# chairclr/PathTracing

Measured on AMD Instinct MI355X. Metric: Mrays/s, higher is better.
Workload: dtype f32

## Files before the change

include/ptrt.h:

```cpp
#ifndef PTRT_H
#define PTRT_H
#include <stddef.h>
#include <stdint.h>
#ifdef __cplusplus
extern "C" {
#endif

#define PTRT_ABI_VERSION 2

typedef int32_t pt_status;
enum {
    PT_OK = 0,
    PT_ERR_INVALID_ARGUMENT = 1,
    PT_ERR_NO_DEVICE = 2,
    PT_ERR_HIP = 3,
    PT_ERR_OUT_OF_MEMORY = 4,
    PT_ERR_NOT_COMMITTED = 5,
    PT_ERR_UNSUPPORTED = 6,
    PT_ERR_INTERNAL = 7
};

typedef struct pt_context pt_context;
typedef struct pt_scene pt_scene;

// ... 9 lines not shown
    PT_FLAG_EXTEND_SIMPLE = 8u,
    PT_FLAG_BUCKET_SPECULAR = 32u,
    PT_FLAG_SPLIT_KERNELS = 64u,
    PT_FLAG_EXTEND_POOL = 128u,
    PT_FLAG_ACCUMULATE = 16u,
    PT_FLAG_NEXT_EVENT = 256u,
    PT_FLAG_NEXT_EVENT_SPHERES = 512u
};
enum {
    PT_BVH_WIDTH_DEFAULT = 0,
    PT_BVH_WIDTH_2 = 2,
    PT_BVH_WIDTH_4 = 4,
    PT_BVH_WIDTH_4Q = 68,
    PT_BVH_WIDTH_8Q = 72,
    PT_BVH_WIDTH_8O = 73,
    PT_BVH_BUILD_LBVH = 0x100
};

typedef struct {
    int32_t device_ordinal;
    void *stream;
    uint32_t flags;
    uint32_t reserved;
} pt_device_desc;

typedef struct { uint32_t kind; float albedo[3]; float emission[3]; float roughness; float ior; uint32_t pad[3]; } pt_material;
#define PT_IOR_MIN 9.5367431640625e-07f
#define PT_IOR_MAX 1048576.0f

typedef struct { float origin[3], forward[3], right[3], up[3]; float scale, cx, cy; uint32_t jitter; } pt_camera;

typedef struct {
    uint32_t width, height;
    uint32_t spp;
    uint32_t max_depth;
    uint32_t rr_start;
    uint32_t seed;
    uint32_t sample_offset;
    uint32_t mode;
    float ray_eps;
    uint32_t rank, nranks;
    uint32_t tile_size;
    uint32_t flags;
    uint32_t streams;
    uint32_t pad[2];
} pt_render_params;

typedef struct {
    uint64_t rays;
    uint64_t paths;
    uint64_t node_visits, tri_tests, sphere_tests;
    uint32_t iterations;
    uint32_t extend_launches;
    double gpu_ms;
    double extend_ms;
    double shade_ms;
    double other_ms;
    uint64_t reserved[4];
} pt_stats;

typedef struct {
    uint32_t width;
    uint32_t n_nodes;
    uint32_t n_tris;
    uint32_t max_depth;
    uint64_t node_bytes;
    uint64_t tri_bytes;
    double build_ms;
    float sah_cost;
    uint32_t stack_need;
} pt_bvh_info;

typedef struct {
    uint32_t bounces;
    uint32_t loops;
    uint32_t finish_below;
    uint32_t packed_chunk;
    float compact_below;
    float sparse_below;
    uint32_t sticky_samples;
    uint32_t lag;
    uint32_t extend_kernel;
    uint32_t readback;
} pt_tuning;

pt_status pt_context_create(const pt_device_desc *desc, pt_context **out);
void pt_context_destroy(pt_context *ctx);
const char *pt_last_error(const pt_context *ctx);
pt_status pt_context_get_tuning(const pt_context *ctx, pt_tuning *out);
pt_status pt_context_set_tuning(pt_context *ctx, const pt_tuning *tuning);
uint32_t pt_abi_version(void);

pt_status pt_scene_create(pt_context *ctx, pt_scene **out);
void pt_scene_destroy(pt_scene *scene);
pt_status pt_scene_set_triangles(pt_scene *s, const float *verts9, const uint32_t *material_ids, uint64_t count);
pt_status pt_scene_set_spheres(pt_scene *s, const float *cxyzr, const uint32_t *material_ids, uint64_t count);
pt_status pt_scene_set_materials(pt_scene *s, const pt_material *mats, uint64_t count);
pt_status pt_scene_set_camera(pt_scene *s, const pt_camera *cam);
pt_status pt_scene_set_sky(pt_scene *s, const float rgb[3]);
pt_status pt_scene_set_environment(pt_scene *s, const float *rgb, uint32_t n);
typedef struct pt_environment_info { uint32_t n, lit; uint64_t device_bytes; double total; } pt_environment_info;
pt_status pt_scene_environment_info(const pt_scene *s, pt_environment_info *out);
pt_status pt_scene_environment_read(const pt_scene *s, float *texels4, float *mcdf, float *ccdf, uint64_t n_texels);
typedef struct pt_lens {
    float radius;
    float focus_distance;
    uint32_t flags;
    uint32_t pad[5];
} pt_lens;
pt_status pt_scene_set_lens(pt_scene *s, const pt_lens *lens);
pt_status pt_scene_get_lens(const pt_scene *s, pt_lens *out);
#define PT_MAX_TEXTURES 64u
#define PT_NO_TEXTURE 0xFFFFFFFFu
enum { PT_TEXTURE_NEAREST = 1u };
pt_status pt_scene_set_triangle_uvs(pt_scene *s, const float *uv6, uint64_t count);
pt_status pt_scene_set_texture(pt_scene *s, uint32_t index, const float *rgb, uint32_t width, uint32_t height, uint32_t flags);
pt_status pt_scene_set_material_textures(pt_scene *s, const uint32_t *texture_of_material, uint64_t count);
typedef struct pt_texture_info { uint32_t width, height, flags, materials; uint64_t device_bytes; } pt_texture_info;
pt_status pt_scene_texture_info(const pt_scene *s, uint32_t index, pt_texture_info *out);
pt_status pt_scene_commit(pt_scene *s, uint32_t bvh_width);
pt_status pt_scene_bvh_info(const pt_scene *s, pt_bvh_info *out);
pt_status pt_scene_bvh_read(const pt_scene *s, void *nodes, uint64_t node_bytes, void *tris48, uint64_t tri_bytes);

pt_status pt_render(pt_context *ctx, const pt_scene *scene, const pt_render_params *params, pt_stats *stats);

enum {
    PT_TRACE_OCCLUSION = 1u,
    PT_TRACE_COUNT_VISITS = 2u,
    PT_TRACE_HOST_MEMORY = 4u
};
pt_status pt_trace_rays(pt_context *ctx, const pt_scene *scene, const void *rays, void *hits, uint64_t n_rays,
                        uint32_t flags, pt_stats *stats);

enum { PT_GATHER_HOST_MEMORY = 1u };
typedef struct pt_gather_params {
    uint32_t samples;
    uint32_t seed;
    uint32_t sample_offset;
    uint32_t point_offset;
    float max_distance;
    float ray_eps;
    uint32_t flags;
    uint32_t pad;
} pt_gather_params;
pt_status pt_gather(pt_context *ctx, const pt_scene *scene, const void *points, void *out, uint64_t n_points,
                    const pt_gather_params *gp, pt_stats *stats);

enum {
    PT_GATHER_PATHS_NEXT_EVENT = 4u,
    PT_GATHER_PATHS_SPHERE_LIGHTS = 16u
};
typedef struct pt_gather_path_params {
    uint32_t max_depth;
    uint32_t rr_start;
    uint32_t flags;
    uint32_t pad[5];
} pt_gather_path_params;
pt_status pt_gather_paths(pt_context *ctx, const pt_scene *scene, const void *points, void *out, uint64_t n_points,
                          const pt_gather_params *gp, const pt_gather_path_params *pp, pt_stats *stats);

enum {
    PT_UPDATE_HOST_MEMORY = 1u
};
pt_status pt_scene_update_triangles(pt_scene *s, const void *verts9, uint64_t count, uint32_t flags, pt_stats *stats);
pt_status pt_scene_update_spheres(pt_scene *s, const float *cxyzr, uint64_t count);

// ... 99 lines not shown
```

pathtracing_amd/_native.py:

```python
import ctypes as C
import os

_HERE = os.path.dirname(os.path.abspath(__file__))
LIB_PATH = os.environ.get("PTRT_LIB") or os.path.join(_HERE, "libptrt.so")

if not os.path.exists(LIB_PATH):
    raise ImportError(
        f"{LIB_PATH} not found: build it with `make -C pathtracing_amd/csrc` (hipcc --offload-arch=gfx950) "
        "or `python -c 'import __graft_entry__ as g; g.build()'`. libptrt has no CPU fallback."
    )

try:
    import torch
except ImportError:
    torch = None

lib = C.CDLL(LIB_PATH)

PT_OK, PT_ERR_INVALID_ARGUMENT, PT_ERR_NO_DEVICE, PT_ERR_HIP, PT_ERR_OUT_OF_MEMORY, PT_ERR_NOT_COMMITTED, \
    PT_ERR_UNSUPPORTED, PT_ERR_INTERNAL = range(8)
PT_REFERENCE_SPHERE, PT_PATH_TRACE = 0, 1
PT_LAMBERT, PT_METAL, PT_DIELECTRIC = 0, 1, 2
PT_IOR_MIN, PT_IOR_MAX = 2.0 ** -20, 2.0 ** 20
PT_FLAG_PROFILE_KERNELS, PT_FLAG_COUNT_VISITS, PT_FLAG_EXTEND_PACKED, PT_FLAG_EXTEND_SIMPLE, PT_FLAG_ACCUMULATE, PT_FLAG_BUCKET_SPECULAR = 1, 2, 4, 8, 16, 32
PT_FLAG_SPLIT_KERNELS = 64
PT_FLAG_EXTEND_POOL = 128
PT_FLAG_NEXT_EVENT = 256
PT_FLAG_NEXT_EVENT_SPHERES = 512
PT_SCENE_CORNELL, PT_SCENE_CORNELL_GLASS, PT_SCENE_TRIANGLE_SOUP, PT_SCENE_CORNELL_TESS = 0, 1, 2, 3
PT_BVH_WIDTH_2, PT_BVH_WIDTH_4, PT_BVH_WIDTH_4Q, PT_BVH_WIDTH_8Q, PT_BVH_WIDTH_8O, PT_BVH_BUILD_LBVH = 2, 4, 68, 72, 73, 0x100
PT_COMM_FORCE_RCCL, PT_COMM_COPY_EXCHANGE = 1, 2
PT_TRACE_OCCLUSION, PT_TRACE_COUNT_VISITS, PT_TRACE_HOST_MEMORY = 1, 2, 4
PT_UPDATE_HOST_MEMORY = 1
PT_GATHER_HOST_MEMORY = 1
PT_MAX_TEXTURES, PT_NO_TEXTURE, PT_TEXTURE_NEAREST = 64, 0xFFFFFFFF, 1
PT_GATHER_PATHS_NEXT_EVENT = 4
PT_GATHER_PATHS_SPHERE_LIGHTS = 16
PT_DENOISE_GUIDES_ONLY, PT_DENOISE_NO_EDGE_STOPS = 1, 2
PT_TEMPORAL_RESET, PT_TEMPORAL_MATCH_IDS = 1, 2
PT_TEMPORAL_MOTION = 8
PT_DISPLAY_FRAME, PT_DISPLAY_DENOISED, PT_DISPLAY_TEMPORAL = 0, 1, 2
PT_TONE_CLAMP, PT_TONE_REINHARD, PT_TONE_ACES = 0, 1, 2
PT_DISPLAY_AUTO_EXPOSURE, PT_DISPLAY_LINEAR, PT_DISPLAY_RESET_ADAPTATION = 1, 2, 4


class pt_device_desc(C.Structure):
    _fields_ = [("device_ordinal", C.c_int32), ("stream", C.c_void_p), ("flags", C.c_uint32), ("reserved", C.c_uint32)]


class pt_material(C.Structure):
    _fields_ = [("kind", C.c_uint32), ("albedo", C.c_float * 3), ("emission", C.c_float * 3),
                ("roughness", C.c_float), ("ior", C.c_float), ("pad", C.c_uint32 * 3)]


class pt_camera(C.Structure):
    _fields_ = [("origin", C.c_float * 3), ("forward", C.c_float * 3), ("right", C.c_float * 3), ("up", C.c_float * 3),
                ("scale", C.c_float), ("cx", C.c_float), ("cy", C.c_float), ("jitter", C.c_uint32)]


class pt_render_params(C.Structure):
    _fields_ = [("width", C.c_uint32), ("height", C.c_uint32), ("spp", C.c_uint32), ("max_depth", C.c_uint32),
                ("rr_start", C.c_uint32), ("seed", C.c_uint32), ("sample_offset", C.c_uint32), ("mode", C.c_uint32),
                ("ray_eps", C.c_float), ("rank", C.c_uint32), ("nranks", C.c_uint32), ("tile_size", C.c_uint32),
                ("flags", C.c_uint32), ("streams", C.c_uint32), ("pad", C.c_uint32 * 2)]


class pt_stats(C.Structure):
    _fields_ = [("rays", C.c_uint64), ("paths", C.c_uint64), ("node_visits", C.c_uint64), ("tri_tests", C.c_uint64),
                ("sphere_tests", C.c_uint64), ("iterations", C.c_uint32), ("extend_launches", C.c_uint32),
                ("gpu_ms", C.c_double), ("extend_ms", C.c_double), ("shade_ms", C.c_double), ("other_ms", C.c_double),
                ("reserved", C.c_uint64 * 4)]


class pt_bvh_info(C.Structure):
    _fields_ = [("width", C.c_uint32), ("n_nodes", C.c_uint32), ("n_tris", C.c_uint32), ("max_depth", C.c_uint32),
                ("node_bytes", C.c_uint64), ("tri_bytes", C.c_uint64), ("build_ms", C.c_double),
                ("sah_cost", C.c_float), ("stack_need", C.c_uint32)]


class pt_tuning(C.Structure):
    _fields_ = [("bounces", C.c_uint32), ("loops", C.c_uint32), ("finish_below", C.c_uint32), ("packed_chunk", C.c_uint32),
                ("compact_below", C.c_float), ("sparse_below", C.c_float), ("sticky_samples", C.c_uint32), ("lag", C.c_uint32),
                ("extend_kernel", C.c_uint32), ("readback", C.c_uint32)]


class pt_tile_layout(C.Structure):
    _fields_ = [("tile_size", C.c_uint32), ("tiles_x", C.c_uint32), ("tiles_y", C.c_uint32), ("n_tiles", C.c_uint32),
                ("tiles_mine", C.c_uint32), ("tiles_per_rank", C.c_uint32), ("floats_per_tile", C.c_uint64)]


class pt_denoise_params(C.Structure):
    _fields_ = [("iterations", C.c_uint32), ("sigma_color", C.c_float), ("sigma_normal", C.c_float), ("sigma_depth", C.c_float),
                ("sigma_albedo", C.c_float), ("flags", C.c_uint32), ("pad", C.c_uint32 * 2)]


class pt_temporal_params(C.Structure):
    _fields_ = [("max_history", C.c_uint32), ("plane_tolerance", C.c_float), ("normal_min", C.c_float), ("flags", C.c_uint32),
                ("pad", C.c_uint32 * 4)]


class pt_display_params(C.Structure):
    _fields_ = [("source", C.c_uint32), ("curve", C.c_uint32), ("exposure", C.c_float), ("white", C.c_float), ("key", C.c_float),
                ("adapt", C.c_float), ("trim_low", C.c_uint32), ("trim_high", C.c_uint32), ("flags", C.c_uint32), ("pad", C.c_uint32)]


class pt_display_info(C.Structure):
    _fields_ = [("exposure", C.c_float), ("metered", C.c_float), ("log_average", C.c_float), ("adapted", C.c_uint32),
                ("counted", C.c_uint64), ("used", C.c_uint64)]


class pt_environment_info(C.Structure):
    _fields_ = [("n", C.c_uint32), ("lit", C.c_uint32), ("device_bytes", C.c_uint64), ("total", C.c_double)]


class pt_gather_params(C.Structure):
    _fields_ = [("samples", C.c_uint32), ("seed", C.c_uint32), ("sample_offset", C.c_uint32), ("point_offset", C.c_uint32),
                ("max_distance", C.c_float), ("ray_eps", C.c_float), ("flags", C.c_uint32), ("pad", C.c_uint32)]


class pt_gather_path_params(C.Structure):
    _fields_ = [("max_depth", C.c_uint32), ("rr_start", C.c_uint32), ("flags", C.c_uint32), ("pad", C.c_uint32 * 5)]


class pt_lens(C.Structure):
    _fields_ = [("radius", C.c_float), ("focus_distance", C.c_float), ("flags", C.c_uint32), ("pad", C.c_uint32 * 5)]


class pt_texture_info(C.Structure):
    _fields_ = [("width", C.c_uint32), ("height", C.c_uint32), ("flags", C.c_uint32), ("materials", C.c_uint32), ("device_bytes", C.c_uint64)]


class pt_scene_counts(C.Structure):
    _fields_ = [("n_tris", C.c_uint64), ("n_spheres", C.c_uint64), ("n_mats", C.c_uint64)]


assert C.sizeof(pt_material) == 48 and C.sizeof(pt_camera) == 64 and C.sizeof(pt_render_params) == 64 and C.sizeof(pt_tuning) == 40
assert C.sizeof(pt_denoise_params) == 32 and C.sizeof(pt_temporal_params) == 32
assert C.sizeof(pt_display_params) == 40 and C.sizeof(pt_display_info) == 32 and C.sizeof(pt_environment_info) == 24
assert C.sizeof(pt_gather_params) == 32 and C.sizeof(pt_lens) == 32 and C.sizeof(pt_texture_info) == 24

_vp, _u32, _u64, _st = C.c_void_p, C.c_uint32, C.c_uint64, C.c_int32
_P = C.POINTER

SYMBOLS = {
    "pt_abi_version": (_u32, []),
    "pt_context_create": (_st, [_P(pt_device_desc), _P(_vp)]),
    "pt_context_destroy": (None, [_vp]),
    "pt_last_error": (C.c_char_p, [_vp]),
    "pt_context_get_tuning": (_st, [_vp, _P(pt_tuning)]),
    "pt_context_set_tuning": (_st, [_vp, _P(pt_tuning)]),
    "pt_scene_create": (_st, [_vp, _P(_vp)]),
    "pt_scene_destroy": (None, [_vp]),
    "pt_scene_set_triangles": (_st, [_vp, _vp, _vp, _u64]),
    "pt_scene_set_spheres": (_st, [_vp, _vp, _vp, _u64]),
    "pt_scene_set_materials": (_st, [_vp, _vp, _u64]),
    "pt_scene_set_camera": (_st, [_vp, _P(pt_camera)]),
    "pt_scene_set_sky": (_st, [_vp, _P(C.c_float * 3)]),
    "pt_scene_set_environment": (_st, [_vp, _vp, _u32]),
    "pt_scene_environment_info": (_st, [_vp, _P(pt_environment_info)]),
    "pt_scene_environment_read": (_st, [_vp, _vp, _vp, _vp, _u64]),
    "pt_scene_set_lens": (_st, [_vp, _P(pt_lens)]),
    "pt_scene_get_lens": (_st, [_vp, _P(pt_lens)]),
    "pt_scene_set_triangle_uvs": (_st, [_vp, _vp, _u64]),
    "pt_scene_set_texture": (_st, [_vp, _u32, _vp, _u32, _u32, _u32]),
    "pt_scene_set_material_textures": (_st, [_vp, _vp, _u64]),
    "pt_scene_texture_info": (_st, [_vp, _u32, _P(pt_texture_info)]),
    "pt_scene_commit": (_st, [_vp, _u32]),
    "pt_scene_bvh_info": (_st, [_vp, _P(pt_bvh_info)]),
    "pt_scene_bvh_read": (_st, [_vp, _vp, _u64, _vp, _u64]),
    "pt_render": (_st, [_vp, _vp, _P(pt_render_params), _P(pt_stats)]),
    "pt_trace_rays": (_st, [_vp, _vp, _vp, _vp, _u64, _u32, _P(pt_stats)]),
    "pt_gather": (_st, [_vp, _vp, _vp, _vp, _u64, _P(pt_gather_params), _P(pt_stats)]),
    "pt_gather_paths": (_st, [_vp, _vp, _vp, _vp, _u64, _P(pt_gather_params), _P(pt_gather_path_params), _P(pt_stats)]),
    "pt_scene_update_triangles": (_st, [_vp, _vp, _u64, _u32, _P(pt_stats)]),
    "pt_scene_update_spheres": (_st, [_vp, _vp, _u64]),
    "pt_denoise": (_st, [_vp, _vp, _P(pt_denoise_params), _P(pt_stats)]),
    "pt_denoised_read": (_st, [_vp, _vp, _u64]),
    "pt_denoised_device_ptr": (_st, [_vp, _P(_vp), _P(_u64)]),
    "pt_guides_read": (_st, [_vp, _vp, _u64]),
    "pt_denoise_temporal": (_st, [_vp, _vp, _P(pt_temporal_params), _P(pt_denoise_params), _P(pt_stats)]),
    "pt_temporal_read": (_st, [_vp, _vp, _u64]),
    "pt_temporal_device_ptr": (_st, [_vp, _P(_vp), _P(_u64)]),
    "pt_temporal_history_read": (_st, [_vp, _vp, _u64]),
    "pt_display": (_st, [_vp, _P(pt_display_params), _P(pt_stats)]),
    "pt_display_read": (_st, [_vp, _vp, _u64]),
    "pt_display_device_ptr": (_st, [_vp, _P(_vp), _P(_u64)]),
    "pt_display_info_read": (_st, [_vp, _P(pt_display_info)]),
    "pt_display_histogram_read": (_st, [_vp, _vp, _u64]),
    "pt_framebuffer_read": (_st, [_vp, _vp, _u64]),
    "pt_framebuffer_read_rgba8": (_st, [_vp, _vp, _u64]),
    "pt_framebuffer_read_srgb8": (_st, [_vp, _vp, _u64]),
    "pt_framebuffer_device_ptr": (_st, [_vp, _P(_vp), _P(_u64)]),
    "pt_tile_layout_query": (_st, [_P(pt_render_params), _P(pt_tile_layout)]),
    "pt_tiles_device_ptr": (_st, [_vp, _P(_vp), _P(_u64)]),
    "pt_assemble_tiles": (_st, [_vp, _P(pt_render_params), _vp, _u64]),
    "pt_comm_create": (_st, [_P(_vp), _u32, _u32, _u32, _P(_vp)]),
    "pt_comm_destroy": (None, [_vp]),
    "pt_comm_render": (_st, [_vp, _P(_vp), _P(pt_render_params), _P(pt_stats)]),
    "pt_comm_stage_tiles": (_st, [_vp, _u32]),
    "pt_comm_assemble": (_st, [_vp, _P(pt_render_params)]),
    "pt_scenegen": (_st, [_u32, _u32, _u32, _u32, _u32, _P(pt_scene_counts), _vp, _vp, _vp, _vp, _vp, _P(pt_camera), _vp]),
}

for _name, (_res, _args) in SYMBOLS.items():
    _f = getattr(lib, _name)
    _f.restype = _res
    _f.argtypes = _args

INTERNAL_SYMBOLS = {
    "pt_internal_lbvh_binary": (_st, [_vp, _vp, _u64, _vp, _vp, _vp, _vp, _vp, _vp]),
}
for _name, (_res, _args) in INTERNAL_SYMBOLS.items():
    _f = getattr(lib, _name)
    _f.restype = _res
    _f.argtypes = _args

PTRT_ABI_VERSION = 2
if lib.pt_abi_version() != PTRT_ABI_VERSION:
    raise ImportError(f"{LIB_PATH} has ABI version {lib.pt_abi_version()}, this binding expects {PTRT_ABI_VERSION}: rebuild libptrt.so")
# ... 1 lines not shown
```

pathtracing_amd/csrc/api.cpp:

```cpp
#include "context.h"
#include <hip/hip_runtime.h>
#include <cmath>
#include <cstdarg>
#include <cstdio>
#include <cstring>
#include <new>
#include <string>

using namespace ptrt;

namespace {
thread_local std::string g_err;
}

namespace ptrt {
pt_status layout_of(const pt_render_params *p, pt_tile_layout *o)
{
    if (!p || !o) return PT_ERR_INVALID_ARGUMENT;
    if (p->width == 0 || p->height == 0 || p->width > 32768 || p->height > 32768) return PT_ERR_INVALID_ARGUMENT;
    if (p->tile_size != 0 && p->tile_size != kTile) return PT_ERR_UNSUPPORTED;
    const uint32_t nr = p->nranks ? p->nranks : 1u;
    if (p->rank >= nr) return PT_ERR_INVALID_ARGUMENT;
    o->tile_size = kTile;
    o->tiles_x = (p->width + kTile - 1) / kTile;
// ... 22 lines not shown
pt_status check_device_array(pt_context *c, const void *p, uint64_t bytes, const char *what, const char *who, const char *host_flag)
{
    hipPointerAttribute_t at;
    if (hipPointerGetAttributes(&at, p) != hipSuccess || (at.type != hipMemoryTypeDevice && !at.isManaged) || at.device != c->device) {
        (void)hipGetLastError();
        return fail(c, PT_ERR_INVALID_ARGUMENT, "%s: %s is not device memory of the context's device %d (host arrays: %s)", who, what, c->device, host_flag);
    }
    hipDeviceptr_t base = nullptr; size_t size = 0;
    if (hipMemGetAddressRange(&base, &size, (hipDeviceptr_t)p) != hipSuccess) { (void)hipGetLastError(); return PT_OK; }
    if ((const char *)p + bytes > (const char *)base + size)
        return fail(c, PT_ERR_INVALID_ARGUMENT, "%s: %s holds %llu bytes from the pointer on, the call needs %llu", who, what,
                    (unsigned long long)((const char *)base + size - (const char *)p), (unsigned long long)bytes);
    return PT_OK;
}
pt_status copy_out(pt_context *c, void *dst, const void *src, uint64_t need, size_t elem, uint64_t have, const char *unit)
{
    if (have < need) return fail(c, PT_ERR_INVALID_ARGUMENT, "buffer too small: need %llu %s", (unsigned long long)need, unit);
    HIP_TRY(c, hipSetDevice(c->device));
    HIP_TRY(c, hipMemcpyAsync(dst, src, need * elem, hipMemcpyDeviceToHost, c->stream));
    HIP_TRY(c, hipStreamSynchronize(c->stream));
    return PT_OK;
}
}

extern "C" {

uint32_t pt_abi_version(void) { return PTRT_ABI_VERSION; }

const char *pt_last_error(const pt_context *ctx) { return ctx ? ctx->err.c_str() : g_err.c_str(); }

pt_status pt_context_create(const pt_device_desc *desc, pt_context **out)
{
    if (!out) return fail(nullptr, PT_ERR_INVALID_ARGUMENT, "pt_context_create: out is NULL");
    *out = nullptr;
    const int dev = desc ? desc->device_ordinal : 0;
    int ndev = 0;
    hipError_t e = hipGetDeviceCount(&ndev);
    if (e != hipSuccess || ndev <= 0)
        return fail(nullptr, PT_ERR_NO_DEVICE, "no HIP device visible (%s); libptrt has no CPU backend",
                    e == hipSuccess ? "device count 0" : hipGetErrorString(e));
    if (dev < 0 || dev >= ndev) return fail(nullptr, PT_ERR_INVALID_ARGUMENT, "device ordinal %d out of range [0,%d)", dev, ndev);
    hipDeviceProp_t prop;
    HIP_TRY(nullptr, hipGetDeviceProperties(&prop, dev));
    if (std::strncmp(prop.gcnArchName, "gfx950", 6) != 0)
        return fail(nullptr, PT_ERR_NO_DEVICE, "device %d is %s; libptrt ships gfx950 (MI355X) code objects only", dev, prop.gcnArchName);
    HIP_TRY(nullptr, hipSetDevice(dev));
    pt_context *c = new (std::nothrow) pt_context();
    if (!c) return fail(nullptr, PT_ERR_OUT_OF_MEMORY, "host allocation failed");
    c->device = dev;
    if (desc && desc->stream) c->stream.borrow((hipStream_t)desc->stream);
    else if ((e = c->stream.create()) != hipSuccess) { delete c; return fail(nullptr, PT_ERR_HIP, "hipStreamCreate: %s", hipGetErrorString(e)); }
    bool ok = c->sizes.alloc() == hipSuccess;
    if (ok && !c->sizes.can_map()) c->tuning.readback = 1u;
    for (uint32_t g = 0; ok && g < kMaxGroups; ++g) ok = c->group_stream[g].create() == hipSuccess && c->ev_join[g].create(false) == hipSuccess;
    ok = ok && c->ev_fork.create(false) == hipSuccess && c->ev_start.create() == hipSuccess && c->ev_stop.create() == hipSuccess;
    ok = ok && c->sizes.create_events() == hipSuccess;
    for (auto &ev : c->ev_probe) ok = ok && ev.create() == hipSuccess;
    for (auto &ev : c->query.ev) ok = ok && ev.create() == hipSuccess;
    ok = ok && c->counters.ensure(kCntTotalWords) == hipSuccess;
    if (!ok) { delete c; return fail(nullptr, PT_ERR_HIP, "context resource creation failed"); }
    *out = c;
    return PT_OK;
}

pt_status pt_context_get_tuning(const pt_context *c, pt_tuning *o)
{
    if (!c || !o) return fail(nullptr, PT_ERR_INVALID_ARGUMENT, "pt_context_get_tuning: NULL argument");
    *o = c->tuning;
    return PT_OK;
}

pt_status pt_context_set_tuning(pt_context *c, const pt_tuning *t)
{
    if (!c || !t) return fail(c, PT_ERR_INVALID_ARGUMENT, "pt_context_set_tuning: NULL argument");
    if (t->bounces > 64) return fail(c, PT_ERR_INVALID_ARGUMENT, "tuning: bounces must be 0 (default) or 1..64");
    if (t->loops != 0 && t->loops != 1 && t->loops != 2 && t->loops != 4) return fail(c, PT_ERR_INVALID_ARGUMENT, "tuning: loops must be 0 (default), 1, 2 or 4");
    if (t->packed_chunk != 0 && (t->packed_chunk < 64 || t->packed_chunk > (1u << 20))) return fail(c, PT_ERR_INVALID_ARGUMENT, "tuning: packed_chunk must be 0 (default) or 64..2^20");
    if (t->lag != 0 && (t->lag < 2 || t->lag > kLag)) return fail(c, PT_ERR_INVALID_ARGUMENT, "tuning: lag must be 0 (default) or 2..%u", kLag);
    if (!(t->compact_below >= 0.f && t->compact_below <= 2.f) || !(t->sparse_below >= 0.f && t->sparse_below <= 1.f))
        return fail(c, PT_ERR_INVALID_ARGUMENT, "tuning: compact_below must be in [0,2], sparse_below in [0,1]");
    if (t->extend_kernel > kExtendKernelLast) return fail(c, PT_ERR_INVALID_ARGUMENT, "tuning: extend_kernel must be 0 (probed), 1 (one ray per lane), 2 (lane-packing) or 3 (pooled)");
    if (t->readback > 1) return fail(c, PT_ERR_INVALID_ARGUMENT, "tuning: readback must be 0 (mapped store) or 1 (copy per launch)");
    if (t->readback == 0 && !c->sizes.can_map()) return fail(c, PT_ERR_UNSUPPORTED, "tuning: readback 0 needs host-mapped pinned memory, which this platform did not provide");
    c->tuning = *t;
    return PT_OK;
}

void pt_context_destroy(pt_context *c)
{
    if (!c) return;
    (void)hipSetDevice(c->device);
    context_drain(c);
    delete c;
}

pt_status pt_tile_layout_query(const pt_render_params *p, pt_tile_layout *o)
{
    pt_status st = layout_of(p, o);
    if (st != PT_OK) return fail(nullptr, st, "invalid render params for tile layout");
    return PT_OK;
}

pt_status pt_framebuffer_read(pt_context *c, float *rgba, uint64_t n_floats)
{
    if (!c || !rgba) return fail(c, PT_ERR_INVALID_ARGUMENT, "NULL argument");
    if (!c->out.readable()) return fail(c, PT_ERR_NOT_COMMITTED, "no assembled frame (render with nranks == 1 or call pt_assemble_tiles)");
    return copy_out(c, rgba, c->out.fb.p, c->out.pixels() * 4, sizeof(float), n_floats, "floats");
}

pt_status pt_framebuffer_read_rgba8(pt_context *c, uint8_t *rgba8, uint64_t n_bytes)
{
    if (!c || !rgba8) return fail(c, PT_ERR_INVALID_ARGUMENT, "NULL argument");
    if (!c->out.readable()) return fail(c, PT_ERR_NOT_COMMITTED, "no assembled frame");
    return copy_out(c, rgba8, c->out.fb8.p, c->out.pixels() * 4, 1, n_bytes, "bytes");
}

pt_status pt_framebuffer_read_srgb8(pt_context *c, uint8_t *rgba8, uint64_t n_bytes)
{
    pt_status st = pt_framebuffer_read_rgba8(c, rgba8, n_bytes);
    if (st != PT_OK) return st;
    uint8_t lut[256];
    for (int q = 0; q < 256; ++q) {
        const double l = q / 255.0, e = l <= 0.0031308 ? 12.92 * l : 1.055 * std::pow(l, 1.0 / 2.4) - 0.055;
        lut[q] = (uint8_t)std::floor(255.0 * e + 0.5);
    }
    const uint64_t n = c->out.pixels() * 4;
    for (uint64_t i = 0; i < n; ++i) if ((i & 3u) != 3u) rgba8[i] = lut[rgba8[i]];
    return PT_OK;
}

pt_status pt_framebuffer_device_ptr(pt_context *c, void **dptr, uint64_t *n_floats)
{
    if (!c || !dptr) return fail(c, PT_ERR_INVALID_ARGUMENT, "NULL argument");
    if (!c->out.readable()) return fail(c, PT_ERR_NOT_COMMITTED, "no assembled frame");
    *dptr = c->out.fb.p;
    if (n_floats) *n_floats = c->out.pixels() * 4;
    return PT_OK;
}

pt_status pt_tiles_device_ptr(pt_context *c, void **dptr, uint64_t *n_floats)
{
    if (!c || !dptr) return fail(c, PT_ERR_INVALID_ARGUMENT, "NULL argument");
    if (!c->out.tile_slots()) return fail(c, PT_ERR_NOT_COMMITTED, "no path-traced frame yet");
    *dptr = c->out.tiles.p;
    if (n_floats) *n_floats = (uint64_t)c->out.tile_slots() * 4;
    return PT_OK;
}

pt_status pt_assemble_tiles(pt_context *c, const pt_render_params *p, const void *gathered, uint64_t n_floats)
{
    if (!c || !p || !gathered) return fail(c, PT_ERR_INVALID_ARGUMENT, "NULL argument");
    pt_tile_layout lay;
    pt_status st = layout_of(p, &lay);
    if (st != PT_OK) return fail(c, st, "pt_assemble_tiles: bad params");
    if (p->spp == 0) return fail(c, PT_ERR_INVALID_ARGUMENT, "spp == 0");
    const uint32_t nranks = p->nranks ? p->nranks : 1u;
    const uint64_t per_rank = (uint64_t)lay.tiles_per_rank * kTilePixels;
    if (n_floats < per_rank * nranks * 4) return fail(c, PT_ERR_INVALID_ARGUMENT, "gathered buffer too small: need %llu floats", (unsigned long long)(per_rank * nranks * 4));
    HIP_TRY(c, hipSetDevice(c->device));
    c->out.replace();
    HIP_TRY(c, c->out.resize(p->width, p->height));
    HIP_TRY(c, launch_assemble(c->stream, (const float4 *)gathered, nranks, (uint32_t)per_rank, p->width, p->height, lay.tiles_x, lay.n_tiles,
                               1.0f / (float)(((p->flags & PT_FLAG_ACCUMULATE) ? (uint64_t)p->sample_offset : 0u) + p->spp), c->out.fb.p, c->out.fb8.p));
    HIP_TRY(c, hipStreamSynchronize(c->stream));
    c->out.complete(FrameOutputs::Holds::path_traced);
    return PT_OK;
// ... 4 lines not shown
```

pathtracing_amd/csrc/context.h:

```cpp
#pragma once
#include "ptrt_internal.h"
#include "device_owner.h"
#include <algorithm>
#include <cstring>
#include <string>
#include <vector>

namespace ptrt {

pt_status fail(pt_context *ctx, pt_status code, const char *fmt, ...);
#define HIP_TRY(ctx, expr)                                                                          \
    do { hipError_t _e = (expr);                                                                    \
         if (_e != hipSuccess)                                                                      \
             return fail(ctx, _e == hipErrorOutOfMemory ? PT_ERR_OUT_OF_MEMORY : PT_ERR_HIP,        \
                         "%s failed: %s (%s:%d)", #expr, hipGetErrorString(_e), __FILE__, __LINE__); \
    } while (0)

void context_drain(pt_context *c);

template <typename Call> pt_status drained_on_failure(pt_context *c, Call call)
{
    const pt_status st = call();
    if (st != PT_OK && c) { (void)hipSetDevice(context_device(c)); context_drain(c); }
    return st;
// ... 141 lines not shown
    bool valid_ = false;
};

class Accumulation {
public:
    struct Key { uint32_t w, h, rank, nranks, streams, seed; bool nee; bool spheres = false; };
    enum class Refusal { none, other_frame, other_estimator, other_light_set, wrong_offset };
    Refusal continues(const Key &k, uint32_t sample_offset) const
    {
        if (spp == 0 || key.w != k.w || key.h != k.h || key.rank != k.rank || key.nranks != k.nranks || key.streams != k.streams || key.seed != k.seed)
            return Refusal::other_frame;
        if (key.nee != k.nee) return Refusal::other_estimator;
        if (key.spheres != k.spheres) return Refusal::other_light_set;
        return sample_offset != spp ? Refusal::wrong_offset : Refusal::none;
    }
    uint64_t samples() const { return spp; }
    bool next_event() const { return key.nee; }
    bool sphere_lights() const { return key.spheres; }
    void begin() { spp = 0; }
    void complete(const Key &k, uint64_t total_spp) { key = k; spp = total_spp; }

private:
    Key key{};
    uint64_t spp = 0;
};

class QueueSizes {
public:
    struct Sizes { uint32_t longest; uint64_t alive, traced; };
    hipError_t alloc()
    {
        const hipError_t e = h_counts.alloc(kTemplateOffset + kRingWords);
        if (e == hipSuccess && h_ring.alloc(kLag * kShards, true) == hipSuccess) std::memset(h_ring.p, 0, sizeof(uint4) * kLag * kShards);
        else if (e == hipSuccess) (void)hipGetLastError();
        return e;
    }
    hipError_t create_events()
    {
        for (auto &row : ev_lag) for (auto &ev : row) if (const hipError_t e = ev.create(false)) return e;
        return hipSuccess;
    }
    bool can_map() const { return h_ring.d != nullptr; }
    uint4 *begin(bool mapped) { mapped_ = mapped; return mapped ? h_ring.d : nullptr; }
    uint32_t *frame_end() const { return h_counts.p + kFinalOffset; }
    uint32_t *template_sizes() const { return h_counts.p + kTemplateOffset; }

    hipError_t post(hipStream_t stream, uint32_t g, uint32_t it, const uint32_t *lines, uint32_t n_shards)
    {
        const uint32_t ring = it % kLag;
        if (!mapped_) {
            const hipError_t e = hipMemcpyAsync(copied(g, ring), lines, sizeof(uint32_t) * n_shards * kCounterStride, hipMemcpyDeviceToHost, stream);
            if (e != hipSuccess) return e;
        }
        return hipEventRecord(ev_lag[g][ring], stream);
    }
    hipError_t wait(uint32_t g, uint32_t old_it, uint32_t first_shard, uint32_t n_shards, Sizes &out)
    {
        const hipError_t e = hipEventSynchronize(ev_lag[g][(mapped_ ? old_it + 1u : old_it) % kLag]);
        if (e != hipSuccess) return e;
        const volatile uint32_t *h_old = mapped_ ? (const volatile uint32_t *)(h_ring.p + (size_t)(old_it % kLag) * kShards + first_shard)
                                                 : copied(g, old_it % kLag);
        const uint32_t line = mapped_ ? 4u : kCounterStride;
        out = Sizes{ 0u, 0u, 0u };
        for (uint32_t sh = 0; sh < n_shards; ++sh) {
            out.longest = std::max(out.longest, (uint32_t)h_old[sh * line]);
            out.alive += h_old[sh * line + 1];
            out.traced += (uint64_t)h_old[sh * line + 2] | ((uint64_t)h_old[sh * line + 3] << 32);
        }
        return hipSuccess;
    }

private:
    static constexpr size_t kFinalOffset = (size_t)kMaxGroups * kLag * kRingWords;
    static constexpr size_t kTemplateOffset = kFinalOffset + kCntTotalWords;
    uint32_t *copied(uint32_t g, uint32_t ring) const { return h_counts.p + ((size_t)g * kLag + ring) * kRingWords; }
    Pinned<uint32_t> h_counts;
    Pinned<uint4> h_ring;
    Event ev_lag[kMaxGroups][kLag];
    bool mapped_ = false;
};

class FrameTemplate {
public:
    struct Key { uint32_t w, h, rank, nranks, streams, first_spp, offset, n_slots, shard_cap, pad; const void *q, *acc;
                 bool operator==(const Key &o) const { return std::memcmp(this, &o, sizeof *this) == 0; } };
    hipError_t reserve(size_t q_entries)
    {
        const hipError_t e = q_init.ensure(q_entries);
        return e != hipSuccess ? e : cnt_init.ensure(kCntTotalWords);
    }
    pt_status build_if_differs(pt_context *c, hipStream_t q, Key key, const Pipeline &pipe, const DeviceScene &ds, const PathState &ps,
                               const FrameParams &fp, const QueueSizes &sizes);
    void frame_ran(bool accumulate_or_full_state) { if (accumulate_or_full_state && key_.first_spp < key_.streams) valid = false; }
    const uint32_t *counters() const { return cnt_init.p; }
    uint32_t *first_queue() const { return q_init.p; }
    uint32_t first_bound() const { return bound; }

private:
    DevBuf<uint32_t> q_init, cnt_init;
    Key key_{};
    bool valid = false;
    uint32_t bound = 0;
};

class Queries {
public:
    DevBuf<float4> rays, hits;
    Event ev[2];
    struct Counts { uint32_t error; uint64_t node_visits, tri_tests, sphere_tests; };
    pt_status setup(pt_context *c, uint32_t overflow, uint64_t n_rays, PathState &ps);
    pt_status launch(pt_context *c, const DeviceScene &ds, const PathState &ps, const float4 *rays, float4 *hits, uint64_t n_rays, bool occlusion, bool count);
    pt_status finish(pt_context *c, Counts &out);

private:
    DevBuf<uint32_t> cnt;
    DevBuf<int32_t> ovf;
};

}

struct pt_context {
    int device = 0;
    ptrt::Stream stream;
    std::string err;
    ptrt::DevBuf<float4> ray_o, ray_d, thr, acc;
    ptrt::DevBuf<float4> nee_ext, nee_rad;
    ptrt::DevBuf<float2> hit;
    ptrt::DevBuf<uint32_t> sd, q_ext0, q_ext1, q_metal, q_dielectric, counters;
    ptrt::DevBuf<int32_t> stack_ovf;
    ptrt::Accumulation sums;
    ptrt::FrameTemplate start;
    ptrt::QueueSizes sizes;
    ptrt::Stream group_stream[ptrt::kMaxGroups];
    ptrt::Event ev_fork, ev_join[ptrt::kMaxGroups];
    pt_tuning tuning = {
        0,
        0,
        4096,
        0,
        0.9f,
        0.f,
        32,
        0,
        0,
        0,
    };
    ptrt::Event ev_start, ev_stop;
    ptrt::Event ev_probe[4];
    std::vector<ptrt::Event> ev_pool;
    ptrt::FrameOutputs out;
    ptrt::TemporalHistory history;
    ptrt::DisplayAdaptation adaptation;
    ptrt::Queries query;
};
```

pathtracing_amd/csrc/frame.cpp:

```cpp
#include "scene.h"
#include <hip/hip_runtime.h>
#include <algorithm>
#include <cmath>
#include <cstdio>
#include <cstdlib>
#include <cstring>
#include <vector>

using namespace ptrt;

namespace {

uint32_t host_pcg(uint32_t x)
{
    uint32_t s = x * 747796405u + 2891336453u;
    uint32_t w = ((s >> ((s >> 28) + 4u)) ^ s) * 277803737u;
    return (w >> 22) ^ w;
}

uint32_t faster(double rate_simple, double rate_packed) { return rate_packed > 1.10 * rate_simple ? EXT_PACKED : EXT_SIMPLE; }
struct ExtendFrame {
    ExtendChoice &mem;
    bool undecided;
    uint32_t frame_kernel, kernel;
    bool mixed = false;
    uint64_t probe_n[2] = { 0, 0 };
    ExtendFrame(ExtendChoice &m, const Pipeline &p) : mem(m),
        undecided(p.forced == 0u && m.kernel == 0u && !p.instrumented()),
        frame_kernel((undecided && m.rate_simple > 0.0 && m.rate_packed == 0.0) ? EXT_PACKED : EXT_SIMPLE),
        kernel(p.forced ? p.forced : m.kernel ? m.kernel : (undecided && frame_kernel == EXT_SIMPLE) ? 0u : frame_kernel) {}
    bool probing(uint32_t g, uint32_t it) const { return g == 0u && kernel == 0u && (it == 2u || it == 3u); }
    uint32_t bounces(uint32_t g, uint32_t it, int k, uint32_t simple) const { return k != EXT_PACKED ? simple : probing(g, it) ? 8u : 64u; }
    hipError_t observe(uint32_t g, uint32_t it, uint64_t traced, uint32_t loop_slots, const Event *ev)
    {
        if (!probing(g, it)) return hipSuccess;
        probe_n[it - 2u] = traced;
        if (it == 2u) return hipSuccess;
        float ms_simple = 0.f, ms_packed = 0.f; hipError_t e = hipEventElapsedTime(&ms_simple, ev[0], ev[1]);
        if (e != hipSuccess || (e = hipEventElapsedTime(&ms_packed, ev[2], ev[3])) != hipSuccess) return e;
        const uint64_t enough = (uint64_t)loop_slots / 8u;
        if (probe_n[0] < enough || probe_n[1] < enough) {
            kernel = EXT_SIMPLE; mixed = probe_n[1] >= enough / 8u;
        } else kernel = mem.kernel = faster(probe_n[0] / std::max((double)ms_simple, 1e-6), probe_n[1] / std::max((double)ms_packed, 1e-6));
        return hipSuccess;
    }
    void frame_done(uint64_t rays, double gpu_ms, bool cold)
    {
        if (!undecided || mem.kernel != 0u || cold) return;
        if (mixed || rays < (1u << 20) || !(gpu_ms > 0.0)) { if (++mem.misses >= 3u) mem.kernel = EXT_SIMPLE; return; }
        (frame_kernel == EXT_PACKED ? mem.rate_packed : mem.rate_simple) = (double)rays / gpu_ms;
        if (mem.rate_simple > 0.0 && mem.rate_packed > 0.0) mem.kernel = faster(mem.rate_simple, mem.rate_packed);
    }
};

hipEvent_t pool_event(pt_context *c, size_t i)
{
    while (c->ev_pool.size() <= i) {
        Event e;
        if (e.create() != hipSuccess) return nullptr;
        c->ev_pool.push_back(std::move(e));
    }
    return c->ev_pool[i];
}

bool scene_pixels(const pt_scene *s, const pt_camera &cam, uint32_t W, uint32_t H, FrameParams &fp)
{
    fp.scene_x0 = fp.scene_y0 = 0u; fp.scene_x1 = fp.scene_y1 = ~0u;
    Box tb;
    if (!s->tree.root_bound(tb)) return false;
    double lo[3], hi[3], o[3], big = 0.0;
    for (int k = 0; k < 3; ++k) { lo[k] = tb.lo[k]; hi[k] = tb.hi[k]; o[k] = cam.origin[k]; big = std::max(big, std::fabs(o[k])); }
    for (size_t i = 0; i < s->sph_mat.size(); ++i) {
        const float *sp = &s->spheres[i * 4];
        const double r = sp[3], dx = sp[0] - o[0], dy = sp[1] - o[1], dz = sp[2] - o[2], reach = std::sqrt(dx * dx + dy * dy + dz * dz) + r;
        const double rr = std::sqrt(r * r + std::ldexp(reach * reach, -16));
        for (int k = 0; k < 3; ++k) { lo[k] = std::min(lo[k], sp[k] - rr); hi[k] = std::max(hi[k], sp[k] + rr); }
    }
    if (!(lo[0] <= hi[0])) { fp.scene_x0 = fp.scene_x1 = fp.scene_y0 = fp.scene_y1 = ~0u; return true; }
    for (int k = 0; k < 3; ++k) big = std::max(big, std::max(std::fabs(lo[k]), std::fabs(hi[k])));
    if (!(big < 1e15)) return false;
    for (int k = 0; k < 3; ++k) { lo[k] -= 1e-4 * big; hi[k] += 1e-4 * big; }
    const double R[3] = { cam.right[0], cam.right[1], cam.right[2] }, U[3] = { cam.up[0], cam.up[1], cam.up[2] }, F[3] = { cam.forward[0], cam.forward[1], cam.forward[2] };
    auto cross = [](const double *a, const double *b, double *c) { c[0] = a[1] * b[2] - a[2] * b[1]; c[1] = a[2] * b[0] - a[0] * b[2]; c[2] = a[0] * b[1] - a[1] * b[0]; };
    auto dot = [](const double *a, const double *b) { return a[0] * b[0] + a[1] * b[1] + a[2] * b[2]; };
    double UF[3], FR[3], RU[3];
    cross(U, F, UF); cross(F, R, FR); cross(R, U, RU);
    const double det = dot(R, UF), scale = cam.scale;
    if (!(std::fabs(det) > 1e-6 * std::sqrt(dot(R, R) * dot(U, U) * dot(F, F))) || !(scale > 0.0) || !std::isfinite(scale)) return false;
    double x0 = INFINITY, x1 = -INFINITY, y0 = INFINITY, y1 = -INFINITY;
    for (int i = 0; i < 8; ++i) {
        const double v[3] = { ((i & 1) ? hi[0] : lo[0]) - o[0], ((i & 2) ? hi[1] : lo[1]) - o[1], ((i & 4) ? hi[2] : lo[2]) - o[2] };
        const double a = dot(v, UF) / det, b = dot(v, FR) / det, c = dot(v, RU) / det;
        if (!(c > 1e-4 * (std::fabs(a) + std::fabs(b) + std::fabs(c)))) return false;
        const double px = (a / c + cam.cx) / scale, py = (b / c + cam.cy) / scale;
        x0 = std::min(x0, px); x1 = std::max(x1, px); y0 = std::min(y0, py); y1 = std::max(y1, py);
    }
    const double mx = 1.0 + 1e-4 * ((double)W + std::fabs(cam.cx / scale)), my = 1.0 + 1e-4 * ((double)H + std::fabs(cam.cy / scale));
    x0 -= mx; x1 += mx; y0 -= my; y1 += my;
    if (!std::isfinite(x0) || !std::isfinite(x1) || !std::isfinite(y0) || !std::isfinite(y1)) return false;
    auto px_of = [](double v, uint32_t n) { return (uint32_t)std::min(std::max(v, 0.0), (double)n); };
    fp.scene_x0 = px_of(std::floor(x0), W); fp.scene_x1 = px_of(std::ceil(x1), W);
    fp.scene_y0 = px_of(std::floor(y0), H); fp.scene_y1 = px_of(std::ceil(y1), H);
    if (fp.scene_x0 == 0u && fp.scene_x1 >= W && fp.scene_y0 == 0u && fp.scene_y1 >= H) { fp.scene_x1 = fp.scene_y1 = ~0u; return false; }
    return true;
}

uint64_t scene_pixels_code(const FrameParams &fp)
{
    if (fp.scene_x0 >= fp.scene_x1 || fp.scene_y0 >= fp.scene_y1) return ~0ull;
    if (fp.width > 0xFFFFu || fp.height > 0xFFFFu) return 0ull;
    return (uint64_t)fp.scene_x0 | (uint64_t)fp.scene_x1 << 16 | (uint64_t)fp.scene_y0 << 32 | (uint64_t)fp.scene_y1 << 48;
}

bool lens_basis(const pt_camera &cam, const pt_lens &lens, LensArgs &out)
{
    auto dot = [](const float *a) { return std::fma(a[2], a[2], std::fma(a[1], a[1], a[0] * a[0])); };
    const float dr = dot(cam.right), du = dot(cam.up);
    if (dr == 0.0f || du == 0.0f) return false;
    const float ru = lens.radius * (1.0f / std::sqrt(dr)), rv = lens.radius * (1.0f / std::sqrt(du));
    for (int k = 0; k < 3; ++k) {
        out.u[k] = cam.right[k] * ru; out.v[k] = cam.up[k] * rv;
        if (!std::isfinite(out.u[k]) || !std::isfinite(out.v[k])) return false;
    }
    out.focus = lens.focus_distance; out.pad = 0u;
    return true;
}

bool lens_in_domain(const pt_camera &cam, const pt_lens &lens, uint32_t W, uint32_t H)
{
    const double r[3] = { cam.right[0], cam.right[1], cam.right[2] }, u[3] = { cam.up[0], cam.up[1], cam.up[2] }, f[3] = { cam.forward[0], cam.forward[1], cam.forward[2] };
    auto dot = [](const double *a, const double *b) { return a[0] * b[0] + a[1] * b[1] + a[2] * b[2]; };
    const double n[3] = { r[1] * u[2] - r[2] * u[1], r[2] * u[0] - r[0] * u[2], r[0] * u[1] - r[1] * u[0] };
    const double nn = std::sqrt(dot(n, n)), lr = std::sqrt(dot(r, r)), lu = std::sqrt(dot(u, u)), F = lens.focus_distance, R = lens.radius;
    if (!(nn > 0x1p-6 * lr * lu)) return false;
    const double scale = cam.scale, cx = cam.cx, cy = cam.cy, tw = (double)W * std::fabs(scale) + std::fabs(cx), th = (double)H * std::fabs(scale) + std::fabs(cy);
    const double ax = -cx, bx = (double)W * scale - cx, ay = -cy, by = (double)H * scale - cy;
    const double sxs[2] = { std::min(ax, bx) - std::ldexp(tw, -22), std::max(ax, bx) + std::ldexp(tw, -22) };
    const double sys[2] = { std::min(ay, by) - std::ldexp(th, -22), std::max(ay, by) + std::ldexp(th, -22) };
    double vmax = 0.0;
    for (int i = 0; i < 4; ++i) {
        const double sx = sxs[i & 1], sy = sys[i >> 1];
        const double v[3] = { f[0] + sx * r[0] + sy * u[0], f[1] + sx * r[1] + sy * u[1], f[2] + sx * r[2] + sy * u[2] };
        const double len = std::sqrt(dot(v, v));
        if (!std::isfinite(len)) return false;
        vmax = std::max(vmax, len);
    }
    const double hi = F * vmax + R * std::sqrt(1.0 + std::fabs(dot(r, u)) / (lr * lu));
    const double S = std::sqrt(dot(f, f)) + (std::max(std::fabs(ax), std::fabs(bx)) + tw) * lr + (std::max(std::fabs(ay), std::fabs(by)) + th) * lu;
    const double lo = F * (std::fabs(dot(f, n)) / nn - std::ldexp(S, -11));
    return lo >= 0x1p-60 && hi * hi <= 0x1p127;
}

struct Frame {
    uint32_t nranks, streams, pixel_slots, n_slots, shard_cap, samples_per_stream, lag, n_loops, packed_chunk, default_bounces;
    Pipeline pipe;
    bool accumulate, mapped, compact;
    NeeArgs nee_args; EnvArgs env_args; LensArgs lens_args;
    SphArgs sph_args;
    TexArgs tex_args;
    bool sky;
    Accumulation::Key sums_key;
    size_t q_entries; uint64_t total_spp, allocs_before;
    PathState ps; FrameParams fp;
    uint32_t iters; uint64_t slot_launches; size_t n_events;
    std::vector<uint64_t> trace_alive, trace_rays;
};

}

pt_status FrameTemplate::build_if_differs(pt_context *c, hipStream_t q, Key key, const Pipeline &pipe, const DeviceScene &ds, const PathState &ps,
                                          const FrameParams &fp, const QueueSizes &sizes)
{
    key.q = q_init.p;
    if (valid && key == key_) return PT_OK;
    valid = false; HIP_TRY(c, hipMemsetAsync(cnt_init.p, 0, sizeof(uint32_t) * kCntTotalWords, q));
    PathState pt = ps; pt.counters = cnt_init.p; pt.q_ext[0] = q_init.p;
    const bool dense = key.first_spp < key.streams;
    HIP_TRY(c, launch_generate(q, ds, pt, fp, pipe.generate_mode(dense)));
    bound = key.shard_cap;
    if (dense) {
        uint32_t *h = sizes.template_sizes();
        HIP_TRY(c, hipMemcpyAsync(h, cnt_init.p, sizeof(uint32_t) * kShards * kCounterStride, hipMemcpyDeviceToHost, q));
        HIP_TRY(c, hipStreamSynchronize(q));
        bound = 0;
        for (uint32_t sh = 0; sh < kShards; ++sh) bound = std::max(bound, h[cnt_ext_index(0, sh)]);
    }
    key_ = key; valid = true;
    return PT_OK;
}

static PipelineDecode decode_frame(const pt_context *c, const pt_scene *s, const pt_render_params *p)
{
    return decode_pipeline(p->flags, c->tuning.extend_kernel, s->env.present(), s->has_specular, s->lens.radius > 0.f, s->n_sph_lights != 0u, s->textures.textured());
}
static Accumulation::Key sums_key_of(const pt_render_params *p)
{
    return Accumulation::Key{ p->width, p->height, p->rank, p->nranks ? p->nranks : 1u, p->streams ? p->streams : 1u, p->seed,
                              (p->flags & PT_FLAG_NEXT_EVENT) != 0, (p->flags & PT_FLAG_NEXT_EVENT_SPHERES) != 0 };
}
static pt_status other_light_set(pt_context *c)
{
    return fail(c, PT_ERR_INVALID_ARGUMENT, "PT_FLAG_ACCUMULATE: the sums so far were made %s PT_FLAG_NEXT_EVENT_SPHERES", c->sums.sphere_lights() ? "with" : "without");
}

static pt_status plan_frame(pt_context *c, const pt_scene *s, const pt_render_params *p, const pt_tile_layout &lay, Frame &f)
{
    if (!s) return fail(c, PT_ERR_INVALID_ARGUMENT, "pt_render: scene is NULL");
    if (s->ctx != c) return fail(c, PT_ERR_INVALID_ARGUMENT, "scene belongs to another context");
    if (!s->committed) return fail(c, PT_ERR_NOT_COMMITTED, "scene not committed");
    if (p->spp == 0 || p->spp >= (1u << 24)) return fail(c, PT_ERR_INVALID_ARGUMENT, "spp must be in [1, 2^24)");
    if (p->max_depth == 0 || p->max_depth > 255) return fail(c, PT_ERR_INVALID_ARGUMENT, "max_depth must be in [1,255]");
    if (!std::isfinite(p->ray_eps) || p->ray_eps < 0.f) return fail(c, PT_ERR_INVALID_ARGUMENT, "ray_eps must be finite and >= 0");
    if (p->streams > 64) return fail(c, PT_ERR_INVALID_ARGUMENT, "streams must be in [0,64]");
    const pt_tuning &t = c->tuning;
    f.nranks = p->nranks ? p->nranks : 1u; f.streams = p->streams ? p->streams : 1u;
    f.pixel_slots = lay.tiles_per_rank * kTilePixels;
    const uint64_t slots64 = (uint64_t)f.pixel_slots * f.streams;
    if (slots64 >= (1ull << 28)) return fail(c, PT_ERR_UNSUPPORTED, "frame too large: %llu slots (pixels of this rank x streams), limit 2^28", (unsigned long long)slots64);
    f.n_slots = (uint32_t)slots64;
    const uint32_t groups = (f.n_slots + (1u << kShardGroupShift) - 1u) >> kShardGroupShift, shard_cap = ((groups + kShards - 1) / kShards) << kShardGroupShift;
    f.shard_cap = shard_cap; f.q_entries = (size_t)kShards * shard_cap;
    f.samples_per_stream = (p->spp + f.streams - 1u) / f.streams;
    const PipelineDecode d = decode_frame(c, s, p);
    if (d.status != PT_OK) return fail(c, d.status, "%s", d.message);
    const Pipeline &pipe = f.pipe = d.pipeline;
    if (pipe.lens && !lens_basis(s->ds.cam, s->lens, f.lens_args))
        return fail(c, PT_ERR_INVALID_ARGUMENT, "pt_render through a lens: the camera's right or up has length 0, or the aperture's axes are not finite");
    f.mapped = t.readback == 0u;
    f.packed_chunk = t.packed_chunk >= 64u ? t.packed_chunk : (f.streams >= 4u ? 256u : 128u);
    const uint32_t v34 = p->max_depth * 3u / 4u; f.default_bounces = std::min(12u, std::max(4u, v34 > 2u ? v34 - 2u : 0u));
    if (pipe.nee) f.default_bounces *= 2u;
    f.lag = t.lag ? t.lag : (f.samples_per_stream <= 2u ? 2u : 3u) + (f.mapped ? 1u : 0u);
    f.accumulate = (p->flags & PT_FLAG_ACCUMULATE) != 0;
    f.sums_key = sums_key_of(p);
    if (f.accumulate)
        switch (c->sums.continues(f.sums_key, p->sample_offset)) {
        case Accumulation::Refusal::other_frame:
            return fail(c, PT_ERR_INVALID_ARGUMENT, "PT_FLAG_ACCUMULATE needs a previous frame with the same size, rank, nranks, streams and seed");
        case Accumulation::Refusal::other_estimator:
            return fail(c, PT_ERR_INVALID_ARGUMENT, "PT_FLAG_ACCUMULATE: the sums so far were made %s PT_FLAG_NEXT_EVENT", c->sums.next_event() ? "with" : "without");
        case Accumulation::Refusal::other_light_set: return other_light_set(c);
        case Accumulation::Refusal::wrong_offset:
            return fail(c, PT_ERR_INVALID_ARGUMENT, "PT_FLAG_ACCUMULATE: sample_offset must be %llu (samples so far)", (unsigned long long)c->sums.samples());
        case Accumulation::Refusal::none: break;
        }
    f.total_spp = (f.accumulate ? c->sums.samples() : 0u) + p->spp; c->sums.begin();
    f.allocs_before = g_device_allocs;
    HIP_TRY(c, c->ray_o.ensure(f.n_slots)); HIP_TRY(c, c->ray_d.ensure(f.n_slots)); HIP_TRY(c, c->thr.ensure(f.n_slots));
    HIP_TRY(c, c->acc.ensure(f.n_slots)); HIP_TRY(c, c->out.tiles.ensure(f.pixel_slots)); HIP_TRY(c, c->sd.ensure(f.n_slots));
    HIP_TRY(c, c->q_ext0.ensure(f.q_entries)); HIP_TRY(c, c->q_ext1.ensure(f.q_entries));
    if (pipe.split) { HIP_TRY(c, c->hit.ensure(f.n_slots)); HIP_TRY(c, c->q_metal.ensure(f.q_entries)); HIP_TRY(c, c->q_dielectric.ensure(f.q_entries)); }
    if (!pipe.full_state()) HIP_TRY(c, c->start.reserve(f.q_entries));
    const uint32_t ovf = s->tree.stack_overflow();
    if (ovf) HIP_TRY(c, c->stack_ovf.ensure((size_t)ovf * f.q_entries));
    if (pipe.nee) {
        HIP_TRY(c, c->nee_ext.ensure(f.n_slots)); HIP_TRY(c, c->nee_rad.ensure(f.n_slots));
        f.nee_args = NeeArgs{ s->d_lights.p, s->d_cdf.p, s->d_pa.p, s->n_lights, c->nee_ext.p, c->nee_rad.p };
        if (pipe.sph) {
            f.nee_args = NeeArgs{ s->d_jlights.p, s->d_jcdf.p, s->d_jpa.p, s->n_lights + s->n_sph_lights, c->nee_ext.p, c->nee_rad.p };
            f.sph_args = SphArgs{ s->d_sph_pmf.p, s->n_lights, 0u };
        }
    }
    if (pipe.env) f.env_args = s->env.args(pipe.nee && s->env.lit() && (s->n_lights || pipe.sph) ? 0.5f : 1.0f);
    if (pipe.tex) f.tex_args = s->textures.args();
    if (f.nranks == 1) HIP_TRY(c, c->out.resize(p->width, p->height));
    PathState &ps = f.ps;
    ps.ray_o = c->ray_o.p; ps.ray_d = c->ray_d.p; ps.thr = c->thr.p; ps.sd = c->sd.p; ps.acc = c->acc.p; ps.q_ext[0] = c->q_ext0.p; ps.q_ext[1] = c->q_ext1.p;
    if (pipe.split) { ps.hit = c->hit.p; ps.q_bucket[B_METAL] = c->q_metal.p; ps.q_bucket[B_DIELECTRIC] = c->q_dielectric.p; }
    ps.counters = c->counters.p; ps.stack_ovf = c->stack_ovf.p; ps.stack_ovf_entries = ovf; ps.n_slots = f.n_slots; ps.shard_cap = f.shard_cap;
    ps.shard_base = 0; ps.shard_count = kShards; ps.compact_below = t.compact_below; ps.finish_below = t.finish_below; ps.sparse_below = t.sparse_below;
    ps.repack_sticky = (f.samples_per_stream <= t.sticky_samples && t.compact_below > 0.f) ? 1u : 0u;
    ps.host_ring = c->sizes.begin(f.mapped); ps.ring_slots = kLag;
    f.compact = pipe.forces_compact(ps.repack_sticky != 0u, f.samples_per_stream);
    FrameParams &fp = f.fp;
    fp.width = p->width; fp.height = p->height; fp.spp = p->spp; fp.max_depth = p->max_depth; fp.rr_start = p->rr_start;
    fp.seed_hashed = host_pcg(p->seed); fp.sample_offset = p->sample_offset; fp.ray_eps = p->ray_eps;
    fp.rank = p->rank; fp.nranks = f.nranks; fp.tiles_x = lay.tiles_x; fp.n_tiles = lay.n_tiles; fp.streams = f.streams; fp.slots_per_stream = f.pixel_slots;
    div_magic(f.streams, fp.streams_magic, fp.streams_shift); div_magic(lay.tiles_x, fp.tiles_x_magic, fp.tiles_x_shift);
    fp.offset_mod = p->sample_offset % f.streams; fp.accumulate = f.accumulate ? 1u : 0u;
    fp.scene_x0 = fp.scene_y0 = 0u; fp.scene_x1 = fp.scene_y1 = ~0u;
    f.sky = pipe.resolves_sky() && scene_pixels(s, s->ds.cam, p->width, p->height, fp);
    return PT_OK;
}

static pt_status start_frame(pt_context *c, const pt_scene *s, const pt_render_params *p, const Frame &f)
{
    hipStream_t q = c->stream; const bool full_state = f.pipe.full_state();
    if (full_state) {
        HIP_TRY(c, hipMemsetAsync(c->counters.p, 0, sizeof(uint32_t) * kCntTotalWords, q));
        HIP_TRY(c, hipEventRecord(c->ev_start, q));
        HIP_TRY(c, launch_generate(q, s->ds, f.ps, f.fp, f.pipe.generate_mode(false)));
    } else {
        HIP_TRY(c, hipEventRecord(c->ev_start, q));
        FrameTemplate::Key key{};
        key.w = p->width; key.h = p->height; key.rank = p->rank; key.nranks = f.nranks; key.streams = f.streams; key.first_spp = std::min(p->spp, f.streams);
        key.offset = f.fp.offset_mod; key.n_slots = f.n_slots; key.shard_cap = f.shard_cap; key.acc = c->acc.p;
        const pt_status st = c->start.build_if_differs(c, q, key, f.pipe, s->ds, f.ps, f.fp, c->sizes);
        if (st != PT_OK) return st;
        HIP_TRY(c, hipMemcpyAsync(c->counters.p, c->start.counters(), sizeof(uint32_t) * kCntTotalWords, hipMemcpyDeviceToDevice, q));
        if (f.sky) HIP_TRY(c, launch_sky_pixels(q, s->ds, f.ps, f.fp));
    }
    c->start.frame_ran(f.accumulate || full_state);
    return PT_OK;
}

static pt_status run_loops(pt_context *c, const pt_scene *s, const pt_render_params *p, Frame &f, ExtendFrame &x)
{
    hipStream_t q = c->stream; const Pipeline &pipe = f.pipe; const bool full_state = pipe.full_state();
    const uint32_t n_loops = f.n_loops, per_group = kShards / n_loops;
    struct Loop { hipStream_t stream; uint32_t base, bound, iters; bool done; } loops[kMaxGroups];
    HIP_TRY(c, hipEventRecord(c->ev_fork, q));
    for (uint32_t g = 0; g < n_loops; ++g) {
        loops[g] = Loop{ n_loops == 1 ? q : c->group_stream[g], g * per_group, full_state ? f.shard_cap : c->start.first_bound(), 0u, false };
        if (loops[g].stream != q) HIP_TRY(c, hipStreamWaitEvent(loops[g].stream, c->ev_fork, 0));
    }
    const uint64_t max_iters = (uint64_t)p->spp * p->max_depth * (pipe.nee ? 2u : 1u) + kLag + 2;
    const bool trace = pipe.profile && getenv("PTRT_TRACE") != nullptr;
    for (uint32_t live = n_loops; live > 0;) {
        for (uint32_t g = 0; g < n_loops; ++g) {
            Loop &L = loops[g];
            if (L.done) continue;
            if (L.iters >= max_iters) return fail(c, PT_ERR_INTERNAL, "wavefront loop did not drain after %u iterations", L.iters);
            const uint32_t it = L.iters; PathState pg = f.ps; pg.shard_base = L.base; pg.shard_count = per_group;
            if (it == 0u && !full_state) pg.q_ext[0] = c->start.first_queue();
            if (x.kernel == 0u) pg.finish_below = 0u;
            hipEvent_t e0 = nullptr, e1 = nullptr, e2 = nullptr;
            if (pipe.profile) {
                e0 = pool_event(c, f.n_events++); e1 = pool_event(c, f.n_events++); e2 = pool_event(c, f.n_events++);
                if (!e0 || !e1 || !e2) return fail(c, PT_ERR_HIP, "hipEventCreate failed");
                HIP_TRY(c, hipEventRecord(e0, L.stream));
            }
            const bool probing = x.probing(g, it); const ExtendKernel kernel = pipe.kernel_for(x.kernel, probing ? it : 0u);
            if (probing) HIP_TRY(c, hipEventRecord(c->ev_probe[(it - 2u) * 2u], L.stream));
            const ExtendLaunch launch{ it, L.bound, kernel, pipe.fuse(), pipe.count, f.compact, f.packed_chunk,
                                       c->tuning.bounces ? c->tuning.bounces : x.bounces(g, it, kernel, f.default_bounces),
                                       pipe.nee ? &f.nee_args : nullptr, pipe.env ? &f.env_args : nullptr, pipe.lens ? &f.lens_args : nullptr,
                                       pipe.sph ? &f.sph_args : nullptr, pipe.tex ? &f.tex_args : nullptr };
            HIP_TRY(c, launch_extend(L.stream, s->ds, pg, f.fp, launch));
            if (pipe.profile) HIP_TRY(c, hipEventRecord(e1, L.stream));
            if (pipe.bucket) {
                HIP_TRY(c, launch_shade(L.stream, s->ds, pg, f.fp, it, L.bound, SHADE_QUEUE, true));
                HIP_TRY(c, launch_shade(L.stream, s->ds, pg, f.fp, it, L.bound, SHADE_BUCKETS, true));
            } else if (pipe.split) HIP_TRY(c, launch_shade(L.stream, s->ds, pg, f.fp, it, L.bound, pipe.shade, f.compact));
            if (probing) HIP_TRY(c, hipEventRecord(c->ev_probe[(it - 2u) * 2u + 1u], L.stream));
            if (pipe.profile) HIP_TRY(c, hipEventRecord(e2, L.stream));
            HIP_TRY(c, c->sizes.post(L.stream, g, it, c->counters.p + cnt_ext_index((it + 1u) % 3u, L.base), per_group));
            f.iters = std::max(f.iters, ++L.iters);
            if (L.iters < f.lag) continue;
            const uint32_t old_iter = L.iters - f.lag;
            QueueSizes::Sizes left;
            HIP_TRY(c, c->sizes.wait(g, old_iter, L.base, per_group, left));
            const uint64_t total = left.alive, traced = left.traced;
            L.bound = left.longest;
            if (trace) {
                f.trace_alive.resize(std::max<size_t>(f.trace_alive.size(), old_iter + 1), 0); f.trace_rays.resize(f.trace_alive.size(), 0);
                f.trace_alive[old_iter] += total; f.trace_rays[old_iter] += traced;
            }
            f.slot_launches += total;
            if (total == 0) { L.done = true; --live; }
            HIP_TRY(c, x.observe(g, old_iter, traced, f.n_slots / n_loops, c->ev_probe));
        }
    }
    for (uint32_t g = 0; g < n_loops; ++g)
        if (loops[g].stream != q) { HIP_TRY(c, hipEventRecord(c->ev_join[g], loops[g].stream)); HIP_TRY(c, hipStreamWaitEvent(q, c->ev_join[g], 0)); }
    return PT_OK;
}

static pt_status finish_frame(pt_context *c, const pt_render_params *p, const Frame &f, ExtendFrame &x, pt_stats *stats)
{
    hipStream_t q = c->stream; const FrameParams &fp = f.fp;
    HIP_TRY(c, launch_reduce_streams(q, c->acc.p, c->out.tiles.p, f.pixel_slots, f.streams));
    if (f.nranks == 1)
        HIP_TRY(c, launch_assemble(q, c->out.tiles.p, 1, f.pixel_slots, p->width, p->height, fp.tiles_x, fp.n_tiles, 1.0f / (float)f.total_spp, c->out.fb.p, c->out.fb8.p));
    HIP_TRY(c, hipEventRecord(c->ev_stop, q));
    HIP_TRY(c, hipMemcpyAsync(c->sizes.frame_end(), c->counters.p, sizeof(uint32_t) * kCntTotalWords, hipMemcpyDeviceToHost, q));
    HIP_TRY(c, hipStreamSynchronize(q));
    pt_stats out{}; const CounterView hc{ c->sizes.frame_end(), 0u };
    if (hc.error()) return fail(c, PT_ERR_INTERNAL, "device error flag 0x%x (1 = traversal stack overflow, 2 = step limit)", hc.error());
    for (uint32_t sh = 0; sh < kShards; ++sh) {
        if (hc.word(cnt_alive_index(0, sh)) || hc.word(cnt_alive_index(1, sh)) || hc.word(cnt_alive_index(2, sh))) return fail(c, PT_ERR_INTERNAL, "extend queue of shard %u not empty at frame end", sh);
        out.rays += hc.u64(cnt_rays_index(sh));
    }
    float ms = 0.f; HIP_TRY(c, hipEventElapsedTime(&ms, c->ev_start, c->ev_stop)); out.gpu_ms = ms;
    out.node_visits = hc.u64(kCntNodes); out.tri_tests = hc.u64(kCntTris); out.sphere_tests = hc.u64(kCntSph);
    out.reserved[3] = (hc.u64(kCntWaveNodeIters) & 0xFFFFFFFFFFull) | (hc.u64(kCntWaveNodeIters + 2) << 40);
    if (f.sky) out.reserved[3] = scene_pixels_code(fp);
    if (f.pipe.count && getenv("PTRT_TRACE")) {
        const double slots = 64.0 * (double)hc.u64(kCntWaveNodeIters), v = (double)out.node_visits, lf = (double)hc.u64(kCntIdleLeaf), dn = (double)hc.u64(kCntIdleDone);
        if (slots > 0) fprintf(stderr, "ptrt: node-loop lane-slots %.3g: visiting %.1f %%, waiting at a leaf %.1f %%, ray finished %.1f %%, no ray %.1f %%\n", slots,
                               100 * v / slots, 100 * lf / slots, 100 * dn / slots, 100 * (slots - v - lf - dn) / slots);
    }
    out.iterations = f.iters; out.extend_launches = f.iters;
    x.frame_done(out.rays, out.gpu_ms, g_device_allocs != f.allocs_before);
    out.reserved[0] = x.kernel ? x.kernel : (uint32_t)EXT_SIMPLE;
    out.reserved[1] = hc.word(kCntCompactions);
    uint64_t px = 0, scene_px = 0;
    for (uint32_t t = p->rank; t < fp.n_tiles; t += f.nranks) {
        const uint32_t tx = t % fp.tiles_x, ty = t / fp.tiles_x;
        const uint32_t xa = tx * kTile, ya = ty * kTile, xb = xa + std::min(kTile, p->width - xa), yb = ya + std::min(kTile, p->height - ya);
        px += (uint64_t)(xb - xa) * (yb - ya);
        const int64_t ix = (int64_t)std::min(xb, fp.scene_x1) - (int64_t)std::max(xa, fp.scene_x0), iy = (int64_t)std::min(yb, fp.scene_y1) - (int64_t)std::max(ya, fp.scene_y0);
        scene_px += (uint64_t)(std::max<int64_t>(ix, 0) * std::max<int64_t>(iy, 0));
    }
    out.paths = px * p->spp;
    out.rays += (px - scene_px) * p->spp;
    out.reserved[2] = f.slot_launches + px * std::min(f.streams, p->spp);
    if (f.pipe.profile) {
        const bool trace = getenv("PTRT_TRACE") != nullptr;
        for (size_t i = 0; i + 2 < f.n_events; i += 3) {
            float a = 0.f, b = 0.f; HIP_TRY(c, hipEventElapsedTime(&a, c->ev_pool[i], c->ev_pool[i + 1]));
            HIP_TRY(c, hipEventElapsedTime(&b, c->ev_pool[i + 1], c->ev_pool[i + 2]));
            out.extend_ms += a; out.shade_ms += b;
            if (trace) fprintf(stderr, "ptrt: iteration %3zu  rays %10llu  alive after %10llu  extend %8.3f ms  shade %8.3f ms\n", i / 3,
                               (unsigned long long)(i / 3 < f.trace_rays.size() ? f.trace_rays[i / 3] : 0),
                               (unsigned long long)(i / 3 < f.trace_alive.size() ? f.trace_alive[i / 3] : 0), a, b);
        }
        out.other_ms = out.gpu_ms - out.extend_ms - out.shade_ms;
        if (trace && f.sky) fprintf(stderr, "ptrt: sky pixels x [%u, %u) y [%u, %u) excepted: %llu of %llu pixels, %llu rays resolved at frame start\n", fp.scene_x0,
                                    fp.scene_x1, fp.scene_y0, fp.scene_y1, (unsigned long long)(px - scene_px), (unsigned long long)px, (unsigned long long)((px - scene_px) * p->spp));
    }
    c->out.tiles_hold(f.pixel_slots); c->sums.complete(f.sums_key, f.total_spp);
    if (f.nranks == 1) c->out.complete(FrameOutputs::Holds::path_traced);
    if (stats) *stats = out;
    return PT_OK;
}

static pt_status render_frame(pt_context *c, const pt_scene *s, const pt_render_params *p, pt_stats *stats)
{
    if (!c || !p) return fail(c, PT_ERR_INVALID_ARGUMENT, "pt_render: NULL argument");
    pt_tile_layout lay; pt_status st = layout_of(p, &lay);
    if (st != PT_OK) return fail(c, st, "pt_render: bad width/height/rank/nranks/tile_size");
    HIP_TRY(c, hipSetDevice(c->device));
    c->out.replace();
    if (p->mode == PT_REFERENCE_SPHERE) {
        HIP_TRY(c, c->out.resize(p->width, p->height));
        HIP_TRY(c, hipEventRecord(c->ev_start, c->stream));
        HIP_TRY(c, launch_reference_sphere(c->stream, p->width, p->height, c->out.fb.p, c->out.fb8.p));
        HIP_TRY(c, hipEventRecord(c->ev_stop, c->stream));
        HIP_TRY(c, hipStreamSynchronize(c->stream));
        float ms = 0.f; HIP_TRY(c, hipEventElapsedTime(&ms, c->ev_start, c->ev_stop));
        pt_stats out{};
        out.gpu_ms = ms; out.other_ms = ms; out.rays = out.paths = (uint64_t)p->width * p->height; out.iterations = 1;
        c->out.complete(FrameOutputs::Holds::reference_sphere); if (stats) *stats = out;
        return PT_OK;
    }
    if (p->mode != PT_PATH_TRACE) return fail(c, PT_ERR_INVALID_ARGUMENT, "unknown mode %u", p->mode);
    Frame f{};
    if ((st = plan_frame(c, s, p, lay, f)) != PT_OK) return st;
    ExtendFrame x(s->cache.ext, f.pipe);
    f.n_loops = f.pipe.single_loop(x.kernel == 0u) ? 1u : c->tuning.loops ? c->tuning.loops : 2u;
    if ((st = start_frame(c, s, p, f)) != PT_OK || (st = run_loops(c, s, p, f, x)) != PT_OK) return st;
    return finish_frame(c, p, f, x, stats);
}

extern "C" pt_status pt_render(pt_context *c, const pt_scene *s, const pt_render_params *p, pt_stats *stats)
{
    if (c && s && p && p->mode == PT_PATH_TRACE && s->ctx == c && s->committed && s->lens.radius > 0.f && !lens_in_domain(s->ds.cam, s->lens, p->width, p->height))
        return fail(c, PT_ERR_INVALID_ARGUMENT, "pt_render through a lens: the lens (radius %g, focus_distance %g) is outside its domain for this camera and a %u x %u image "
                    "(docs/SPEC.md 3.1: focus_distance * |v| + radius too large, focus_distance * forward's part off the plane of right and up too small, or no such plane)",
                    (double)s->lens.radius, (double)s->lens.focus_distance, p->width, p->height);
    if (c && s && p && p->mode == PT_PATH_TRACE && s->ctx == c && s->committed) {
        if (p->flags & PT_FLAG_NEXT_EVENT_SPHERES) {
            const PipelineDecode d = decode_frame(c, s, p);
            if (d.status != PT_OK) return fail(c, d.status, "%s", d.message);
        }
        if ((p->flags & PT_FLAG_ACCUMULATE) && c->sums.continues(sums_key_of(p), p->sample_offset) == Accumulation::Refusal::other_light_set) return other_light_set(c);
    }
    const pt_status st = drained_on_failure(c, [&] { return render_frame(c, s, p, stats); });
    if (st != PT_OK && c) { c->sums.begin(); c->out.lost(); }
    return st;
}
```

pathtracing_amd/csrc/kernels.hip:

```cpp
#include "ptrt_internal.h"
#include "pt_device.h"
#include "texture_device.h"
#include <algorithm>
#include <cstdlib>
#include <type_traits>

using namespace ptd;

namespace ptrt {

PT_DEV uint32_t lane_prefix(uint64_t m) { return __builtin_amdgcn_mbcnt_hi((uint32_t)(m >> 32), __builtin_amdgcn_mbcnt_lo((uint32_t)m, 0u)); }
PT_DEV uint32_t lane_id() { return lane_prefix(~0ull); }

typedef const float4 __attribute__((address_space(4))) *uniform_f4;
PT_DEV uniform_f4 as_uniform(const float4 *p) { return (uniform_f4)(uintptr_t)p; }
PT_DEV float4 uniform_load(uniform_f4 p, uint32_t i) { return make_float4(p[i].x, p[i].y, p[i].z, p[i].w); }
PT_DEV uint32_t spheres_test(const float4 *spheres, uint32_t n_spheres, uint32_t first_id, V3 o, V3 d, Hit &h)
{
    const uniform_f4 sp = as_uniform(spheres);
    for (uint32_t j = 0; j < n_spheres; j += 4u) {
        const float4 s0 = uniform_load(sp, j), s1 = uniform_load(sp, j + 1u), s2 = uniform_load(sp, j + 2u), s3 = uniform_load(sp, j + 3u);
        sphere_test(s0, first_id + j, o, d, h);
        if (j + 1u < n_spheres) sphere_test(s1, first_id + j + 1u, o, d, h);
        if (j + 2u < n_spheres) sphere_test(s2, first_id + j + 2u, o, d, h);
        if (j + 3u < n_spheres) sphere_test(s3, first_id + j + 3u, o, d, h);
    }
    return n_spheres;
}
struct HotScene {
    const float4 *__restrict__ nodes, *__restrict__ tris, *__restrict__ spheres;
    uint32_t n_spheres, n_tris, n_nodes;
};
PT_DEV HotScene hot_scene(const DeviceScene &sc) { return HotScene{ sc.nodes, sc.tris, sc.spheres, sc.n_spheres, sc.n_tris, sc.n_nodes }; }
PT_DEV uint32_t spheres_test(const HotScene &g, V3 o, V3 d, Hit &h) { return spheres_test(g.spheres, g.n_spheres, g.n_tris, o, d, h); }

PT_DEV void wave_push(uint32_t *counter, uint32_t *queue, bool pred, uint32_t value)
{
    const uint64_t m = __ballot(pred);
    if (m == 0) return;
    const uint32_t prefix = lane_prefix(m);
    const int leader = __ffsll((long long)m) - 1;
    uint32_t base = 0;
    if ((int)lane_id() == leader) base = atomicAdd(counter, (uint32_t)__popcll(m));
    base = __shfl(base, leader, 64);
    if (pred) queue[base + prefix] = value;
}

struct ExtArgs {
    DeviceScene sc; PathState ps; FrameParams fp;
    uint32_t it, compact, bounces, chunk;
};
template <typename T>
PT_DEV T &at(T *base, uint32_t i) { return *reinterpret_cast<T *>(reinterpret_cast<char *>(base) + (size_t)(i * (uint32_t)sizeof(T))); }

template <bool NEE, bool ENV> struct ExtArgsT { ExtArgs x; };
template <> struct ExtArgsT<true, false> { ExtArgs x; NeeArgs nee; };
template <> struct ExtArgsT<false, true> { ExtArgs x; EnvArgs env; };
template <> struct ExtArgsT<true, true> { ExtArgs x; NeeArgs nee; EnvArgs env; };
static_assert(sizeof(ExtArgsT<false, false>) == sizeof(ExtArgs) && __builtin_offsetof(ExtArgsT<true, false>, nee) == sizeof(ExtArgs) &&
              __builtin_offsetof(ExtArgsT<false, true>, env) == sizeof(ExtArgs) && __builtin_offsetof(ExtArgsT<true, true>, nee) == sizeof(ExtArgs) &&
              __builtin_offsetof(ExtArgsT<true, true>, env) == sizeof(ExtArgs) + sizeof(NeeArgs), "each block directly behind the one before it");
template <bool NEE, bool ENV>
PT_DEV const ExtArgsT<NEE, ENV> &kernargs()
{
    auto p = __builtin_amdgcn_kernarg_segment_ptr();
    asm volatile("" : "+s"(p));
    return *(const ExtArgsT<NEE, ENV> *)p;
}
PT_DEV const ExtArgs &cold() { return kernargs<false, false>().x; }
template <bool NEE, bool ENV> struct ExtLensArgsT { ExtArgsT<NEE, ENV> a; LensArgs lens; };
static_assert(__builtin_offsetof(ExtLensArgsT<false, false>, lens) == sizeof(ExtArgsT<false, false>) && __builtin_offsetof(ExtLensArgsT<true, false>, lens) == sizeof(ExtArgsT<true, false>) &&
              __builtin_offsetof(ExtLensArgsT<false, true>, lens) == sizeof(ExtArgsT<false, true>) && __builtin_offsetof(ExtLensArgsT<true, true>, lens) == sizeof(ExtArgsT<true, true>) &&
              __builtin_offsetof(ExtLensArgsT<true, true>, a) == 0, "the lens block directly behind the others, which stay where every instantiation reads them");
template <bool NEE, bool ENV>
PT_DEV const LensArgs &lens_args()
{
    auto p = __builtin_amdgcn_kernarg_segment_ptr();
    asm volatile("" : "+s"(p));
    return ((const ExtLensArgsT<NEE, ENV> *)p)->lens;
}
template <bool NEE, bool ENV> PT_DEV const ExtArgs &ext_of(const ExtArgsT<NEE, ENV> &t) { return t.x; }
template <bool NEE, bool ENV> PT_DEV const ExtArgs &ext_of(const ExtLensArgsT<NEE, ENV> &t) { return t.a.x; }
template <bool ENV, bool LENS> struct ExtSphArgsT { std::conditional_t<LENS, ExtLensArgsT<true, ENV>, ExtArgsT<true, ENV>> a; SphArgs sph; };
static_assert(__builtin_offsetof(ExtSphArgsT<false, false>, sph) == sizeof(ExtArgsT<true, false>) && __builtin_offsetof(ExtSphArgsT<true, false>, sph) == sizeof(ExtArgsT<true, true>) &&
              __builtin_offsetof(ExtSphArgsT<false, true>, sph) == sizeof(ExtLensArgsT<true, false>) && __builtin_offsetof(ExtSphArgsT<true, true>, sph) == sizeof(ExtLensArgsT<true, true>) &&
              __builtin_offsetof(ExtSphArgsT<true, true>, a) == 0, "the sphere block directly behind the others, which stay where every instantiation reads them");
template <bool ENV, bool LENS>
PT_DEV const SphArgs &sph_args()
{
    auto p = __builtin_amdgcn_kernarg_segment_ptr();
    asm volatile("" : "+s"(p));
    return ((const ExtSphArgsT<ENV, LENS> *)p)->sph;
}
template <bool ENV, bool LENS> PT_DEV const ExtArgs &ext_of(const ExtSphArgsT<ENV, LENS> &t) { return ext_of(t.a); }
template <bool NEE, bool ENV> struct ExtTexArgsT { ExtArgsT<NEE, ENV> a; TexArgs tex; };
static_assert(__builtin_offsetof(ExtTexArgsT<false, false>, tex) == sizeof(ExtArgsT<false, false>) && __builtin_offsetof(ExtTexArgsT<true, false>, tex) == sizeof(ExtArgsT<true, false>) &&
              __builtin_offsetof(ExtTexArgsT<false, true>, tex) == sizeof(ExtArgsT<false, true>) && __builtin_offsetof(ExtTexArgsT<true, true>, tex) == sizeof(ExtArgsT<true, true>) &&
              __builtin_offsetof(ExtTexArgsT<true, true>, a) == 0, "the texture block directly behind the others, which stay where every instantiation reads them");
template <bool NEE, bool ENV>
PT_DEV const TexArgs &tex_args()
{
    auto p = __builtin_amdgcn_kernarg_segment_ptr();
    asm volatile("" : "+s"(p));
    return ((const ExtTexArgsT<NEE, ENV> *)p)->tex;
}
template <bool NEE, bool ENV> PT_DEV const ExtArgs &ext_of(const ExtTexArgsT<NEE, ENV> &t) { return t.a.x; }

PT_DEV uint32_t slot_stream(uint32_t slot, const FrameParams &fp)
{
    const uint32_t g = slot >> 6;
    return g - div_by(g, fp.streams_magic, fp.streams_shift) * fp.streams;
}
PT_DEV uint32_t slot_pixel_slot(uint32_t slot, const FrameParams &fp)
{
    return (div_by(slot >> 6, fp.streams_magic, fp.streams_shift) << 6) | (slot & 63u);
}
PT_DEV size_t slot_of(uint32_t pixel_slot, uint32_t stream, uint32_t streams)
{
    return (((size_t)(pixel_slot >> 6) * streams + stream) << 6) | (pixel_slot & 63u);
}

PT_DEV void block_pos(const PathState &ps, uint32_t &shard, uint32_t &bx, uint32_t &nbx)
{
    const uint32_t sh = 31u - (uint32_t)__builtin_clz(ps.shard_count);
    shard = (blockIdx.x & (ps.shard_count - 1u)) + ps.shard_base; bx = blockIdx.x >> sh; nbx = gridDim.x >> sh;
}
static inline dim3 shard_grid(uint32_t blocks, uint32_t shard_count) { return dim3(blocks * shard_count); }

PT_DEV bool slot_pixel(uint32_t slot_all, const FrameParams &fp, uint32_t &x, uint32_t &y)
{
    const uint32_t slot = slot_pixel_slot(slot_all, fp);
    const uint32_t tl = slot >> (2 * kTileShift), inner = slot & (kTilePixels - 1);
    const uint32_t tile = fp.rank + fp.nranks * tl;
    if (tile >= fp.n_tiles) return false;
    const uint32_t ty = div_by(tile, fp.tiles_x_magic, fp.tiles_x_shift), tx = tile - ty * fp.tiles_x;
    const uint32_t blk = inner >> 6, ln = inner & 63u;
    x = (tx << kTileShift) + ((blk & 7u) << 3) + (ln & 7u);
    y = (ty << kTileShift) + ((blk >> 3) << 3) + (ln >> 3);
    return x < fp.width && y < fp.height;
}

PT_DEV Camera camera_of(const pt_camera &c)
{
    Camera k;
    k.origin[0] = c.origin[0]; k.origin[1] = c.origin[1]; k.origin[2] = c.origin[2];
    k.forward[0] = c.forward[0]; k.forward[1] = c.forward[1]; k.forward[2] = c.forward[2];
    k.right[0] = c.right[0]; k.right[1] = c.right[1]; k.right[2] = c.right[2];
    k.up[0] = c.up[0]; k.up[1] = c.up[1]; k.up[2] = c.up[2];
    k.scale = c.scale; k.cx = c.cx; k.cy = c.cy; k.jitter = c.jitter;
    return k;
}
PT_DEV void camera_ray_of(const pt_camera &c, uint32_t x, uint32_t y, uint32_t key, V3 &o, V3 &d) { camera_ray(camera_of(c), x, y, key, o, d); }
PT_DEV V3 camera_vec_of(const pt_camera &c, uint32_t x, uint32_t y, float jx, float jy) { return camera_vec(camera_of(c), x, y, jx, jy); }
PT_DEV void lens_ray_of(const pt_camera &c, const LensArgs &l, uint32_t x, uint32_t y, uint32_t key, V3 &o, V3 &d)
{
    lens_ray(camera_of(c), v3(l.u[0], l.u[1], l.u[2]), v3(l.v[0], l.v[1], l.v[2]), l.focus, x, y, key, o, d);
}

__global__ void __launch_bounds__(kBlock) k_reference_sphere(uint32_t w, uint32_t h, float4 *out_f, uint32_t *out8)
{
    const uint32_t x = blockIdx.x * 64u + threadIdx.x, y = blockIdx.y * 4u + threadIdx.y;
    if (x >= w || y >= h) return;
    const float4 c = ref_sphere_pixel(x, y);
    const size_t i = (size_t)y * w + x;
    out_f[i] = c;
    out8[i] = unorm8(c.x) | (unorm8(c.y) << 8) | (unorm8(c.z) << 16) | (unorm8(c.w) << 24);
}

template <int L>
PT_DEV constexpr int node_rows() { return (L == PT_BVH_WIDTH_4 || L == PT_BVH_WIDTH_8Q || L == PT_BVH_WIDTH_8O) ? 8 : 4; }
template <int L>
PT_DEV constexpr int fanout() { return L == PT_BVH_WIDTH_2 ? 2 : (L == PT_BVH_WIDTH_8Q || L == PT_BVH_WIDTH_8O) ? 8 : 4; }

template <int L, bool SLOT>
PT_DEV void visit_node_keys(const float4 *__restrict__ nd, float4 r0, float4 r1, float4 r2, float4 r3, const RaySetup &rs, float t_best,
                            uint32_t (&key)[fanout<L>()], int32_t (&ref)[fanout<L>()])
{
    constexpr int N = fanout<L>();
    if constexpr (L == PT_BVH_WIDTH_8Q) {
        const float4 r4 = nd[4], r5 = nd[5];
        const uint32_t eb = __float_as_uint(r0.w);
        const float sx = __uint_as_float((eb & 0xffu) << 23), sy = __uint_as_float(((eb >> 8) & 0xffu) << 23),
                    sz = __uint_as_float(((eb >> 16) & 0xffu) << 23);
        const uint32_t q[6][2] = { { __float_as_uint(r3.x), __float_as_uint(r3.y) }, { __float_as_uint(r3.z), __float_as_uint(r3.w) },
                                   { __float_as_uint(r4.x), __float_as_uint(r4.y) }, { __float_as_uint(r4.z), __float_as_uint(r4.w) },
                                   { __float_as_uint(r5.x), __float_as_uint(r5.y) }, { __float_as_uint(r5.z), __float_as_uint(r5.w) } };
        ref[0] = __float_as_int(r1.x); ref[1] = __float_as_int(r1.y); ref[2] = __float_as_int(r1.z); ref[3] = __float_as_int(r1.w);
        ref[4] = __float_as_int(r2.x); ref[5] = __float_as_int(r2.y); ref[6] = __float_as_int(r2.z); ref[7] = __float_as_int(r2.w);
        const bool ng[3] = { rs.inv.x < 0.f, rs.inv.y < 0.f, rs.inv.z < 0.f };
        const float qa[3] = { sx * rs.inv.x, sy * rs.inv.y, sz * rs.inv.z };
        const float qb[3] = { fma_(r0.x, rs.inv.x, rs.noi.x), fma_(r0.y, rs.inv.y, rs.noi.y), fma_(r0.z, rs.inv.z, rs.noi.z) };
        uint32_t qn[3][2], qf[3][2];
#pragma unroll
        for (int k = 0; k < 3; ++k)
#pragma unroll
            for (int w = 0; w < 2; ++w) { qn[k][w] = ng[k] ? q[3 + k][w] : q[k][w]; qf[k][w] = ng[k] ? q[k][w] : q[3 + k][w]; }
#pragma unroll
        for (int c = 0; c < 8; ++c) {
            const int w = c >> 2, sh = 8 * (c & 3);
            float tnk[3], tfk[3];
#pragma unroll
            for (int k = 0; k < 3; ++k) {
                tnk[k] = fma_((float)((qn[k][w] >> sh) & 0xffu), qa[k], qb[k]);
                tfk[k] = fma_((float)((qf[k][w] >> sh) & 0xffu), qa[k], qb[k]);
            }
            const float tn = fmax_(fmax_(tnk[0], tnk[1]), fmax_(tnk[2], 0.0f));
            const float tf = fmin_(fmin_(tfk[0], tfk[1]), fmin_(tfk[2], t_best)) * 1.0000004f;
            const bool hb = tn <= tf && ref[c] != PT_BVH_EMPTY;
            key[c] = hb ? ((__float_as_uint(tn) & ~7u) | (uint32_t)c) : 0xFFFFFFFFu;
        }
    } else if constexpr (L == PT_BVH_WIDTH_4Q) {
        const uint32_t eb = __float_as_uint(r0.w);
        const float sx = __uint_as_float((eb & 0xffu) << 23), sy = __uint_as_float(((eb >> 8) & 0xffu) << 23),
                    sz = __uint_as_float(((eb >> 16) & 0xffu) << 23);
        const uint32_t qlx = __float_as_uint(r2.x), qly = __float_as_uint(r2.y), qlz = __float_as_uint(r2.z),
                       qhx = __float_as_uint(r2.w), qhy = __float_as_uint(r3.x), qhz = __float_as_uint(r3.y);
        ref[0] = __float_as_int(r1.x); ref[1] = __float_as_int(r1.y); ref[2] = __float_as_int(r1.z); ref[3] = __float_as_int(r1.w);
        const bool ng[3] = { rs.inv.x < 0.f, rs.inv.y < 0.f, rs.inv.z < 0.f };
        const float qa[3] = { sx * rs.inv.x, sy * rs.inv.y, sz * rs.inv.z };
        const float qb[3] = { fma_(r0.x, rs.inv.x, rs.noi.x), fma_(r0.y, rs.inv.y, rs.noi.y), fma_(r0.z, rs.inv.z, rs.noi.z) };
        const uint32_t ql[3] = { qlx, qly, qlz }, qh[3] = { qhx, qhy, qhz };
        uint32_t qn[3], qf[3];
// ... 126 lines not shown
};
PT_DEV PathRegs path_none() { return PathRegs{ v3(0.f, 0.f, 0.f), v3(0.f, 0.f, 1.f), v3(0.f, 0.f, 0.f), 0u, 0u, 0u }; }
PT_DEV void path_load(const PathState &ps, uint32_t slot, PathRegs &r)
{
    const float4 O = at(ps.ray_o, slot), D = at(ps.ray_d, slot), TK = at(ps.thr, slot);
    const uint32_t sdv = at(ps.sd, slot);
    r.o = xyz(O); r.d = xyz(D); r.T = xyz(TK);
    r.key = __float_as_uint(TK.w); r.sample = sdv >> 8; r.depth = sdv & 255u;
}

enum : uint32_t { NEE_PENDING = 1u, NEE_END = 2u };
constexpr uint32_t NEE_LAMP_SHIFT = 8u;
PT_DEV bool shadow_reached_lamp(uint32_t flags, uint32_t ref, uint32_t n_tris) { return (flags >> NEE_LAMP_SHIFT) != 0u && ref - n_tris + 1u == flags >> NEE_LAMP_SHIFT; }
struct NeeRegs {
    float aux;
    uint32_t flags;
};
template <bool NEE = false>
PT_DEV void path_store(const PathState &ps, uint32_t slot, const PathRegs &r, const NeeRegs *nr = nullptr)
{
    at(ps.ray_o, slot) = make_float4(r.o.x, r.o.y, r.o.z, NEE ? __uint_as_float(nr->flags) : 0.f);
    at(ps.ray_d, slot) = make_float4(r.d.x, r.d.y, r.d.z, NEE ? nr->aux : 0.f);
    at(ps.thr, slot) = make_float4(r.T.x, r.T.y, r.T.z, __uint_as_float(r.key));
    at(ps.sd, slot) = (r.sample << 8) | r.depth;
}
constexpr float kInvPi = 0.318309873f;
PT_DEV float nan_to_zero(float w) { return w >= 0.0f ? w : 0.0f; }
PT_DEV float mis_weight(float q) { return nan_to_zero(1.0f / fma_(q, q, 1.0f)); }
PT_DEV float mis_weight_times_q(float q) { return nan_to_zero(q / fma_(q, q, 1.0f)); }
PT_DEV uint32_t pick_light(const float *cdf, uint32_t n, float u)
{
    uint32_t lo = 0, hi = n - 1u;
    while (lo < hi) {
        const uint32_t mid = (lo + hi) >> 1;
        if (u < cdf[mid]) hi = mid; else lo = mid + 1u;
    }
    return lo;
}
constexpr float kTwoPi = 6.28318548f;
struct SphCone { V3 oc; float d2, r2, omc; };
PT_DEV bool sphere_cone(V3 c, float r, V3 o, SphCone &k)
{
    k.oc = c - o; k.d2 = dot(k.oc, k.oc); k.r2 = r * r;
    if (!(k.d2 > k.r2)) return false;
    const float sin2 = k.r2 / k.d2, cosm = __builtin_sqrtf(fmax_(0.0f, 1.0f - sin2));
    k.omc = sin2 / (1.0f + cosm);
    return true;
}
PT_DEV float sphere_cone_pdf(float pm, float omc) { return pm * (1.0f / (kTwoPi * omc)); }
PT_DEV V3 sphere_cone_dir(const SphCone &k, float u1, float u2, float &thit)
{
    const float z = u1 * k.omc, cos_t = 1.0f - z, s2 = z * (2.0f - z), sin_t = __builtin_sqrtf(s2);
    float sn, cs;
    sincos2pi(u2, sn, cs);
    const float dist = __builtin_sqrtf(k.d2), inv = 1.0f / dist;
    const V3 w = v3(k.oc.x * inv, k.oc.y * inv, k.oc.z * inv);
    V3 tx, ty;
    basis(w, tx, ty);
    thit = dist * cos_t - __builtin_sqrtf(fmax_(0.0f, k.r2 - k.d2 * s2));
    return to_world(v3(sin_t * cs, sin_t * sn, cos_t), tx, ty, w);
}
PT_DEV V3 env_decode(float u, float v)
{
    const float z = (1.0f - __builtin_fabsf(u)) - __builtin_fabsf(v);
    float x = u, y = v;
    if (z < 0.0f) { x = (1.0f - __builtin_fabsf(v)) * __builtin_copysignf(1.0f, u); y = (1.0f - __builtin_fabsf(u)) * __builtin_copysignf(1.0f, v); }
    return normalize(v3(x, y, z));
}
PT_DEV uint32_t env_cell(float u, float nf, uint32_t n)
{
    const int i = (int)__builtin_floorf(fma_(u, 0.5f, 0.5f) * nf);
    return (uint32_t)min(max(i, 0), (int)n - 1);
}
PT_DEV uint32_t env_texel(const EnvArgs &e, V3 d, float &s)
{
    s = (__builtin_fabsf(d.x) + __builtin_fabsf(d.y)) + __builtin_fabsf(d.z);
    const float is = 1.0f / s, px = d.x * is, py = d.y * is;
    float u = px, v = py;
    if (d.z < 0.0f) { u = (1.0f - __builtin_fabsf(py)) * __builtin_copysignf(1.0f, px); v = (1.0f - __builtin_fabsf(px)) * __builtin_copysignf(1.0f, py); }
    return env_cell(v, e.nf, e.n) * e.n + env_cell(u, e.nf, e.n);
}
PT_DEV float env_pdf(const EnvArgs &e, float4 tx, float s) { return e.psel * (tx.w / ((s * s) * s)); }

PT_DEV uint32_t first_sample(uint32_t slot, const FrameParams &fp)
{
    const uint32_t v = slot_stream(slot, fp) + fp.streams - fp.offset_mod;
    return v >= fp.streams ? v - fp.streams : v;
}
template <bool RAY = true, bool LENS = false>
PT_DEV void camera_sample(const DeviceScene &sc, const FrameParams &fp, uint32_t x, uint32_t y, PathRegs &r, uint32_t &depth, const LensArgs *lens = nullptr)
{
    static_assert(RAY || !LENS, "a lens ray's origin and direction are made together");
    r.key = path_key(fp.seed_hashed, y * fp.width + x, fp.sample_offset + r.sample);
    if constexpr (LENS) lens_ray_of(sc.cam, *lens, x, y, r.key, r.o, r.d);
    else if constexpr (RAY) camera_ray_of(sc.cam, x, y, r.key, r.o, r.d);
    else r.o = v3(sc.cam.origin[0], sc.cam.origin[1], sc.cam.origin[2]);
    r.T = v3(1.f, 1.f, 1.f); depth = 0;
}
template <bool LENS = false>
PT_DEV void path_init(const DeviceScene &sc, const FrameParams &fp, uint32_t slot, PathRegs &r, const LensArgs *lens = nullptr)
{
    uint32_t x = 0, y = 0;
    slot_pixel(slot, fp, x, y);
    r.sample = first_sample(slot, fp);
    camera_sample<true, LENS>(sc, fp, x, y, r, r.depth, lens);
}
template <bool NEE = false, bool LENS = false>
PT_DEV void path_begin(uint32_t it, uint32_t slot, PathRegs &r, NeeRegs *nr = nullptr, const LensArgs *lens = nullptr)
{
    if (it == 0u) {
        path_init<LENS>(cold().sc, cold().fp, slot, r, lens);
        if (!cold().fp.accumulate) at(cold().ps.acc, slot) = make_float4(0.f, 0.f, 0.f, 0.f);
    } else {
        const PathState &ps = cold().ps;
        path_load(ps, slot, r);
        if constexpr (NEE) { nr->flags = __float_as_uint(at(ps.ray_o, slot).w); nr->aux = at(ps.ray_d, slot).w; }
    }
}
PT_DEV uint32_t queued_slot(uint32_t it, uint32_t slot)
{
    if (it == 0u && slot != kInvalidSlot) {
        uint32_t x = 0, y = 0;
        slot_pixel(slot, cold().fp, x, y);
        if (sky_pixel(cold().fp, x, y)) slot = kInvalidSlot;
    }
    return slot;
}

__global__ void __launch_bounds__(kBlock) k_generate(DeviceScene sc, PathState ps, FrameParams fp, uint32_t full)
{
    uint32_t shard, bx, nbx;
    block_pos(ps, shard, bx, nbx);
    const uint32_t j = bx * kBlock + threadIdx.x;
    const uint32_t t = j >> kShardGroupShift, rot = (shard + kShards - t % kShards) % kShards;
    const uint32_t slot = ((t * kShards + rot) << kShardGroupShift) | (j & ((1u << kShardGroupShift) - 1u));
    uint32_t x = 0, y = 0;
    const bool in_range = j < ps.shard_cap && slot < ps.n_slots;
    const uint32_t first = first_sample(slot, fp);
    const bool valid = in_range && first < fp.spp && slot_pixel(slot, fp, x, y);
    if (in_range && !fp.accumulate) ps.acc[slot] = make_float4(0.f, 0.f, 0.f, 0.f);
    if (valid && full == 1u) {
        PathRegs r;
        path_init(sc, fp, slot, r);
        path_store(ps, slot, r);
    }
    if (full == 2u) wave_push(&ps.counters[cnt_ext_index(0, shard)], ps.q_ext[0] + (size_t)shard * ps.shard_cap, valid, slot);
    else if (j < ps.shard_cap) ps.q_ext[0][(size_t)shard * ps.shard_cap + j] = valid ? slot : kInvalidSlot;
    const uint32_t n_alive = (uint32_t)__syncthreads_count(valid);
    if (threadIdx.x == 0) {
        if (n_alive) atomicAdd(&ps.counters[cnt_alive_index(0, shard)], n_alive);
        if (bx == 0 && full != 2u) ps.counters[cnt_ext_index(0, shard)] = ps.shard_cap;
    }
}

__global__ void __launch_bounds__(kBlock) k_sky_pixels(DeviceScene sc, PathState ps, FrameParams fp)
{
    const uint32_t slot = blockIdx.x * kBlock + threadIdx.x;
    uint32_t x = 0, y = 0;
    if (slot >= ps.n_slots || !slot_pixel(slot, fp, x, y) || !sky_pixel(fp, x, y)) return;
    const uint32_t first = first_sample(slot, fp);
    if (first >= fp.spp) return;
    float4 A = fp.accumulate ? ps.acc[slot] : make_float4(0.f, 0.f, 0.f, 0.f);
    for (uint32_t s = first; s < fp.spp; s += fp.streams) {
        A.x = fma_(1.0f, sc.sky[0], A.x); A.y = fma_(1.0f, sc.sky[1], A.y); A.z = fma_(1.0f, sc.sky[2], A.z);
        A.w += 1.0f;
    }
    ps.acc[slot] = A;
}

template <bool LENS = false>
PT_DEV bool next_sample(const DeviceScene &sc, const FrameParams &fp, uint32_t slot, PathRegs &r, uint32_t &depth, const LensArgs *lens = nullptr)
{
    uint32_t x = 0, y = 0;
    r.sample += fp.streams;
    if (!(r.sample < fp.spp)) return false;
    slot_pixel(slot, fp, x, y);
    camera_sample<true, LENS>(sc, fp, x, y, r, depth, lens);
    return true;
}

PT_DEV bool roulette_ends(const FrameParams &fp, uint32_t key, uint32_t depth, uint32_t bb, V3 &T)
{
    if (!(fmax_(T.x, fmax_(T.y, T.z)) > 0.0f)) return true;
    if (depth >= fp.rr_start) {
        const float qrr = fmin_(fmax_(T.x, fmax_(T.y, T.z)), 0.95f);
        if (!(u01(key, 7u + 4u * bb) < qrr)) return true;
        const float iq = 1.0f / qrr; T = v3(T.x * iq, T.y * iq, T.z * iq);
    }
    return false;
}
template <int MODE, bool NEE = false, bool ENV = false, bool LENS = false, bool SPH = false, bool TEX = false>
PT_DEV bool shade_one(const DeviceScene &sc, const PathState &ps, const FrameParams &fp, uint32_t slot, PathRegs &r, float t, uint32_t ref,
                      uint32_t b, uint32_t &defer, NeeRegs *nr = nullptr)
{
    V3 &o = r.o, &d = r.d, &T = r.T;
    uint32_t &key = r.key, &sample = r.sample;
    uint32_t depth = r.depth + 1u;
    float4 A = at(ps.acc, slot);
    bool touched = false, term = false, alive = false;
    constexpr bool SHARED = !NEE && MODE != SHADE_INLINE;
    static_assert(!LENS || !SHARED, "the shared end makes pinhole rays only");
    static_assert(!SPH || (NEE && MODE == SHADE_INLINE), "sphere lights: NEE with all-kinds shading");
    static_assert(!TEX || (MODE == SHADE_INLINE && !LENS && !SPH), "textures: all-kinds shading, pinhole, no sphere lights");
    bool lambert = false, regen = false;
    auto add = [&](V3 L) {
        touched = true;
        A.x = fma_(T.x, L.x, A.x); A.y = fma_(T.y, L.y, A.y); A.z = fma_(T.z, L.z, A.z);
    };

    if (ref == PT_MISS) {
        if constexpr (ENV) {
            const EnvArgs &ea = kernargs<NEE, true>().env;
            float s;
            const float4 tx = ea.texels[env_texel(ea, d, s)];
            V3 e = xyz(tx);
            if constexpr (NEE)
                if (ea.lit && nr->aux > 0.0f) {
                    const float w = mis_weight(env_pdf(ea, tx, s) / nr->aux);
                    e = v3(tx.x * w, tx.y * w, tx.z * w);
                }
            add(e);
        } else
        add(v3(sc.sky[0], sc.sky[1], sc.sky[2]));
        term = true;
    } else {
        const V3 P = madd(t, d, o);
        V3 ng;
        uint32_t mat;
        V3 texel = v3(1.0f, 1.0f, 1.0f);
        if (ref < sc.n_tris) {
            const float4 ts = sc.tris[(size_t)ref * 4 + 3];
            ng = xyz(ts);
            mat = __float_as_uint(ts.w);
            if constexpr (TEX) {
                const float4 *tr = sc.tris + (size_t)ref * 4;
                float u, v;
                tri_uv(tr[0], tr[1], tr[2], o, d, u, v);
                texel = tex_of_hit(tex_args<NEE, ENV>(), ref, u, v);
            }
        } else {
            const uint32_t j = ref - sc.n_tris;
            const float4 s = sc.spheres[j];
            const uint2 mi = sc.sph_mat[j];
            const float ir = __uint_as_float(mi.y);
            ng = v3((P.x - s.x) * ir, (P.y - s.y) * ir, (P.z - s.z) * ir);
            mat = mi.x;
        }
        const bool front = dot(ng, d) < 0.0f;
        const V3 n = front ? ng : neg(ng);
        float4 m0 = sc.mats[(size_t)mat * 3], m1 = sc.mats[(size_t)mat * 3 + 1];
        const float4 m2 = sc.mats[(size_t)mat * 3 + 2];
        asm volatile("" : "+v"(m0.x), "+v"(m1.x));
        const V3 alb = TEX ? v3(m0.y * texel.x, m0.z * texel.y, m0.w * texel.z) : v3(m0.y, m0.z, m0.w), emi = xyz(m1);
        const uint32_t kind = __float_as_uint(m0.x);
        if (MODE == SHADE_QUEUE && kind != (uint32_t)PT_LAMBERT) { defer = 1u + kind; return false; }
        if (emi.x != 0.0f || emi.y != 0.0f || emi.z != 0.0f) {
            if constexpr (NEE) {
                V3 e = emi;
                if (nr->aux > 0.0f && ref < sc.n_tris && (!ENV || kernargs<true, ENV>().nee.n_lights)) {
                    float pa = kernargs<true, ENV>().nee.pa[ref];
                    if constexpr (ENV) pa = pa * kernargs<NEE, true>().env.psel;
                    if (pa > 0.0f) {
                        const float pl = (pa * (t * t)) / __builtin_fabsf(dot(ng, d)), w = mis_weight(pl / nr->aux);
                        e = v3(emi.x * w, emi.y * w, emi.z * w);
                    }
                }
                if constexpr (SPH)
                    if (nr->aux > 0.0f && ref >= sc.n_tris) {
                        float pm = sph_args<ENV, LENS>().pmf[ref - sc.n_tris];
                        if constexpr (ENV) pm = pm * kernargs<NEE, true>().env.psel;
                        const float4 s = sc.spheres[ref - sc.n_tris];
                        SphCone k;
                        if (pm > 0.0f && sphere_cone(xyz(s), s.w, o, k)) {
                            const float w = mis_weight(sphere_cone_pdf(pm, k.omc) / nr->aux);
                            e = v3(emi.x * w, emi.y * w, emi.z * w);
                        }
                    }
                add(e);
            } else add(emi);
        }
        if (depth >= fp.max_depth) term = true;
// ... 25 lines not shown
                        if constexpr (ENV) return na.n_lights || kernargs<NEE, true>().env.lit;
                        else return na.n_lights;
                    };
                    if (!term) nr->aux = (bk == B_LAMBERT && lights()) ? dot(n, wi) * kInvPi : 0.0f;
                    if (bk == B_LAMBERT && lights()) {
                        float uc = 0.0f;
                        bool to_env = false;
                        if constexpr (ENV) {
                            uc = u01(key, 1024u + 3u * bb);
                            to_env = kernargs<NEE, true>().env.lit != 0u;
                            if (to_env && na.n_lights) { to_env = uc < 0.5f; uc = to_env ? uc * 2.0f : fma_(uc, 2.0f, -1.0f); }
                        }
                        if (ENV && to_env) {
                            const EnvArgs &ea = kernargs<NEE, true>().env;
                            const uint32_t j = pick_light(ea.mcdf, ea.n, uc), i = pick_light(ea.ccdf + (size_t)j * ea.n, ea.n, u01(key, 1025u + 3u * bb));
                            const float u = fma_((float)i + u01(key, 1026u + 3u * bb), ea.step, -1.0f), v = fma_((float)j + u01(key, 2048u + bb), ea.step, -1.0f);
                            const V3 wl = env_decode(u, v);
                            float s;
                            const float4 tx = ea.texels[env_texel(ea, wl, s)];
                            const float cs = dot(n, wl), pl = env_pdf(ea, tx, s);
                            if (cs > 0.0f && pl > 0.0f) {
                                const float f = mis_weight_times_q((cs * kInvPi) / pl);
                                at(na.rad, slot) = make_float4((ta.x * f) * tx.x, (ta.y * f) * tx.y, (ta.z * f) * tx.z, 0.0f);
                                if (!term) at(na.ext, slot) = make_float4(d.x, d.y, d.z, nr->aux);
                                nr->flags = NEE_PENDING | (term ? NEE_END : 0u);
                                nr->aux = __builtin_inff();
                                o = madd(fp.ray_eps, n, P); d = wl;
                                term = false;
                            }
                        } else {
                        const float4 *lr = na.lights + (size_t)pick_light(na.cdf, na.n_lights, ENV ? uc : u01(key, 1024u + 3u * bb)) * 4;
                        const float4 l0 = lr[0], l1 = lr[1], l2 = lr[2];
                        if (SPH && lr >= na.lights + (size_t)sph_args<ENV, LENS>().n_tri * 4) {
                            const V3 so = madd(fp.ray_eps, n, P);
                            SphCone k;
                            if (sphere_cone(xyz(l0), l1.x, so, k)) {
                                float thit, pm = l0.w;
                                const V3 sd = sphere_cone_dir(k, u01(key, 1025u + 3u * bb), u01(key, 1026u + 3u * bb), thit);
                                if constexpr (ENV) pm = pm * kernargs<NEE, true>().env.psel;
                                const float cs = dot(n, sd), pl = sphere_cone_pdf(pm, k.omc);
                                if (cs > 0.0f && pl > 0.0f) {
                                    const float4 l3 = lr[3];
                                    const float f = mis_weight_times_q((cs * kInvPi) / pl);
                                    at(na.rad, slot) = make_float4((ta.x * f) * l1.w, (ta.y * f) * l2.w, (ta.z * f) * l3.w, 0.0f);
                                    if (!term) at(na.ext, slot) = make_float4(d.x, d.y, d.z, nr->aux);
                                    nr->flags = NEE_PENDING | (term ? NEE_END : 0u) | (__float_as_uint(l1.y) << NEE_LAMP_SHIFT);
                                    nr->aux = thit * 0.9999f;
                                    o = so; d = sd;
                                    term = false;
                                }
                            }
                        } else {
                        const float su = __builtin_sqrtf(u01(key, 1025u + 3u * bb)), b1 = 1.0f - su, b2 = u01(key, 1026u + 3u * bb) * su;
                        const V3 x = v3(fma_(b2, l2.x, fma_(b1, l1.x, l0.x)), fma_(b2, l2.y, fma_(b1, l1.y, l0.y)), fma_(b2, l2.z, fma_(b1, l1.z, l0.z)));
                        const V3 so = madd(fp.ray_eps, n, P);
                        const V3 dl = x - so;
                        const float dist2 = dot(dl, dl), dist = __builtin_sqrtf(dist2), inv = 1.0f / dist;
                        const V3 sd = v3(dl.x * inv, dl.y * inv, dl.z * inv);
                        const float4 l3 = lr[3];
                        const float cs = dot(n, sd), cl = __builtin_fabsf(dot(xyz(l3), sd));
                        if (cs > 0.0f && cl > 0.0f) {
                            float pa = l0.w;
                            if constexpr (ENV) pa = pa * kernargs<NEE, true>().env.psel;
                            const float pl = (pa * dist2) / cl, f = mis_weight_times_q((cs * kInvPi) / pl);
                            at(na.rad, slot) = make_float4((ta.x * f) * l1.w, (ta.y * f) * l2.w, (ta.z * f) * l3.w, 0.0f);
                            if (!term) at(na.ext, slot) = make_float4(d.x, d.y, d.z, nr->aux);
                            nr->flags = NEE_PENDING | (term ? NEE_END : 0u);
                            nr->aux = dist * 0.9999f;
                            o = so; d = sd;
                            term = false;
                        }
                        }
                        }
                    }
                }
            }
        }
    }

    uint32_t x = 0, y = 0;
    if (term) {
        touched = true;
        A.w += 1.0f;
        sample += fp.streams;
        if (sample < fp.spp) {
            slot_pixel(slot, fp, x, y);
            if constexpr (LENS) camera_sample<true, true>(sc, fp, x, y, r, depth, &lens_args<NEE, ENV>());
            else
            camera_sample<!SHARED>(sc, fp, x, y, r, depth);
            regen = SHARED; alive = true;
        }
        if constexpr (NEE) nr->aux = 0.0f;
    } else alive = true;
    if (lambert || regen) {
        const uint32_t dim = regen ? 0u : 4u * depth;
        float u1 = u01(key, dim), u2 = u01(key, dim + 1u);
        V3 v;
        if (regen) {
            if (!sc.cam.jitter) u1 = u2 = 0.5f;
            v = camera_vec_of(sc.cam, x, y, u1, u2);
        } else v = lambert_vec(d, u1, u2);
        d = normalize(v);
    }
    if (touched) at(ps.acc, slot) = A;
    r.depth = depth;
    return alive;
}

template <bool LENS = false>
PT_DEV bool resolve_shadow(const DeviceScene &sc, const PathState &ps, const FrameParams &fp, const NeeArgs &na, uint32_t slot, PathRegs &r,
                           NeeRegs &nr, bool visible, const LensArgs *lens = nullptr)
{
    const bool end = (nr.flags & NEE_END) != 0u;
    bool alive = true;
    if (visible || end) {
        float4 A = at(ps.acc, slot);
        if (visible) { const float4 L = at(na.rad, slot); A.x = A.x + L.x; A.y = A.y + L.y; A.z = A.z + L.z; }
        if (end) { A.w += 1.0f; alive = next_sample<LENS>(sc, fp, slot, r, r.depth, lens); nr.aux = 0.0f; }
        at(ps.acc, slot) = A;
    }
    if (!end) { const float4 e = at(na.ext, slot); r.d = xyz(e); nr.aux = e.w; }
    nr.flags = 0u;
    return alive;
}

PT_DEV unsigned long long *traced_counter(const PathState &ps, uint32_t c, uint32_t shard)
{
    return reinterpret_cast<unsigned long long *>(ps.counters + cnt_traced_index(c, shard));
}
PT_DEV void fold_traced(const PathState &ps, uint32_t shard, uint32_t it, uint32_t n, uint32_t n_alive)
{
    *traced_counter(ps, (it + 2u) % 3u, shard) = 0ull;
    const unsigned long long traced = *traced_counter(ps, it % 3u, shard);
    *reinterpret_cast<unsigned long long *>(ps.counters + cnt_rays_index(shard)) += traced;
    if (ps.host_ring && it) ps.host_ring[((it - 1u) % ps.ring_slots) * kShards + shard] = make_uint4(n, n_alive, (uint32_t)traced, (uint32_t)(traced >> 32));
}

PT_DEV bool want_compact(const PathState &ps, uint32_t len, uint32_t n_alive, uint32_t prev_alive, bool sticky, bool forced)
{
    const uint32_t deaths = prev_alive > n_alive ? prev_alive - n_alive : 0u;
    const uint32_t predicted = n_alive > deaths ? n_alive - deaths : 0u;
    return forced || (sticky && len < ps.shard_cap) || (float)predicted < ps.compact_below * (float)len;
}

PT_DEV void queue_next(const PathState &ps, uint32_t shard, uint32_t cnext, uint32_t *q_next, uint32_t gid, uint32_t total, bool alive,
                       uint32_t slot, bool compact)
{
    if (compact) wave_push(&ps.counters[cnt_ext_index(cnext, shard)], q_next, alive, slot);
    else {
        if (gid < total) at(q_next, gid) = alive ? slot : kInvalidSlot;
        if (gid == 0) ps.counters[cnt_ext_index(cnext, shard)] = total;
    }
    const uint64_t m = __ballot(alive);
    if (m && lane_id() == 0u) atomicAdd(&ps.counters[cnt_alive_index(cnext, shard)], (uint32_t)__popcll(m));
}

#ifndef PT_EXT_WAVES
#define PT_EXT_WAVES(L, FUSE) (((L) == PT_BVH_WIDTH_4Q || (L) == PT_BVH_WIDTH_2) && (FUSE) != SHADE_INLINE ? 8 : 7)
#endif
#ifndef PT_EXT_WAVES_NEE
#define PT_EXT_WAVES_NEE(L, FUSE) ((FUSE) == SHADE_QUEUE && (L) != PT_BVH_WIDTH_8Q && (L) != PT_BVH_WIDTH_8O ? 7 : 6)
#endif
#define PT_EXT_WAVES_OF(L, FUSE, NEE) ((NEE) ? PT_EXT_WAVES_NEE(L, FUSE) : PT_EXT_WAVES(L, FUSE))
#ifndef PT_EXT_WAVES_ENV
#define PT_EXT_WAVES_ENV(L, NEE) ((NEE) ? 5 : (L) == PT_BVH_WIDTH_8O ? 6 : 7)
#endif
#define PT_EXT_WAVES_FOR(L, FUSE, NEE, ENV) ((ENV) ? PT_EXT_WAVES_ENV(L, NEE) : PT_EXT_WAVES_OF(L, FUSE, NEE))
#ifndef PT_EXT_WAVES_LENS
#define PT_EXT_WAVES_LENS(L, NEE, ENV) (!(NEE) && ((L) == PT_BVH_WIDTH_8Q || (L) == PT_BVH_WIDTH_8O) ? 6 : PT_EXT_WAVES_FOR(L, SHADE_INLINE, NEE, ENV))
#endif
#ifndef PT_EXT_WAVES_SPH
#define PT_EXT_WAVES_SPH(L, FUSE, ENV) ((FUSE) == 5  && (L) == PT_BVH_WIDTH_8O && !(ENV) ? 5 : PT_EXT_WAVES_FOR(L, SHADE_INLINE, true, ENV))
#endif
#ifndef PT_EXT_WAVES_TEX
#define PT_EXT_WAVES_TEX(L, NEE, ENV) (!(NEE) && !(ENV) && (L) == PT_BVH_WIDTH_8O ? 6 : PT_EXT_WAVES_FOR(L, SHADE_INLINE, NEE, ENV))
#endif
#define PT_EXT_WAVES_K(L, FUSE, NEE, ENV) ((FUSE) == 6  ? PT_EXT_WAVES_TEX(L, NEE, ENV) : (FUSE) >= 4  ? PT_EXT_WAVES_SPH(L, FUSE, ENV) : (FUSE) == 3  ? PT_EXT_WAVES_LENS(L, NEE, ENV) : PT_EXT_WAVES_FOR(L, FUSE, NEE, ENV))
struct StackCtx { int32_t *lds; uint32_t stride, tid, col; };
PT_DEV void push_slow(const StackCtx &k, uint32_t &sp, int32_t v)
{
    if (sp < kStackLds) k.lds[sp * k.stride + k.tid] = v;
    else {
        const PathState &ps = cold().ps;
        const uint32_t e = sp - kStackLds;
        if (e < ps.stack_ovf_entries) ps.stack_ovf[(size_t)e * ((size_t)kShards * ps.shard_cap) + k.col] = v;
        else { atomicOr(&ps.counters[kCntError], 1u); return; }
    }
    ++sp;
}
PT_DEV int32_t pop_slow(const StackCtx &k, uint32_t &sp)
{
    if (sp == 0) return PT_BVH_EMPTY;
    --sp;
    if (sp < kStackLds) return k.lds[sp * k.stride + k.tid];
    const PathState &ps = cold().ps;
    return ps.stack_ovf[(size_t)(sp - kStackLds) * ((size_t)kShards * ps.shard_cap) + k.col];
}
PT_DEV int32_t pop_lds(const StackCtx &k, uint32_t &sp)
{
    if (sp == 0) return PT_BVH_EMPTY;
    --sp;
    return k.lds[sp * k.stride + k.tid];
// ... 154 lines not shown
};
PT_DEV void flush_visit_counters(const PathState &ps, const VisitCounts &v)
{
    auto add = [&](uint32_t i, unsigned long long x) { atomicAdd(reinterpret_cast<unsigned long long *>(ps.counters + i), x); };
    if (v.wave_iters) add(kCntWaveNodeIters, v.wave_iters);
    if (v.wave_iters_late) add(kCntWaveNodeIters + 2, v.wave_iters_late);
    if (v.idle_leaf) add(kCntIdleLeaf, v.idle_leaf);
    if (v.idle_done) add(kCntIdleDone, v.idle_done);
    add(kCntNodes, v.nodes);
    add(kCntTris, v.tris);
    add(kCntSph, v.sph);
}

template <int L, bool COUNT, bool DIAG, bool ANY>
PT_DEV Hit trace_ray(const HotScene &g, const StackCtx &stk, V3 o, V3 d, Hit h, VisitCounts &vc, int32_t *s_state)
{
    constexpr VisitOrder ORD = visit_order<L, COUNT>();
    { const uint32_t ns = spheres_test(g, o, d, h); if (COUNT) vc.sph += ns; }

    const RaySetup rs = ray_setup(o, d);
    int32_t cur = PT_BVH_EMPTY;
    uint32_t sp = 0, steps = 0;
    if (g.n_nodes && !(ANY && h.id != PT_MISS)) {
        ++steps;
        if (COUNT) vc.nodes++;
        if (DIAG && lane_id() == (uint32_t)(__ffsll((long long)__ballot(1)) - 1)) vc.wave_iters++;
        const uniform_f4 root = as_uniform(g.nodes);
        node_visit_rows<L, ORD>(g.nodes, uniform_load(root, 0), uniform_load(root, 1), uniform_load(root, 2), uniform_load(root, 3), stk, rs, h.t, cur, sp);
        if (DIAG) s_state[stk.tid & 63u] = cur;
    }

    if constexpr (!COUNT) {
        constexpr uint32_t kMaxSteps = 1u << 22;
        for (;;) {
            bool go = (uint32_t)cur < (uint32_t)PT_BVH_EMPTY && steps < kMaxSteps;
            if (__builtin_amdgcn_ballot_w64(go) != 0) do {
                if (go) { ++steps; node_step<L, ORD>(g.nodes, stk, rs, h.t, cur, sp); }
                go = (uint32_t)cur < (uint32_t)PT_BVH_EMPTY && steps < kMaxSteps;
            } while (__builtin_amdgcn_ballot_w64(go) != 0);
            if ((uint32_t)cur < (uint32_t)PT_BVH_EMPTY) { atomicOr(&cold().ps.counters[kCntError], 2u); cur = PT_BVH_EMPTY; }
            if (!__any((int)(cur != PT_BVH_EMPTY))) break;
            if (cur != PT_BVH_EMPTY) {
                if (ANY) leaf_step_any(g.tris, stk, o, d, h, cur, sp);
                else leaf_step(g.tris, stk, o, d, h, cur, sp);
            }
        }
        return h;
    }
    bool late_cycle = false;
    for (;;) {
        while ((uint32_t)cur < (uint32_t)PT_BVH_EMPTY) {
            if (++steps > (1u << 22)) { atomicOr(&cold().ps.counters[kCntError], 2u); cur = PT_BVH_EMPTY; break; }
            if (COUNT) vc.nodes++;
            if (DIAG && lane_id() == (uint32_t)(__ffsll((long long)__ballot(1)) - 1)) {
                vc.wave_iters++; if (late_cycle) vc.wave_iters_late++;
                uint32_t n_leaf = 0, n_done = 0;
                for (uint32_t l = 0; l < 64u; ++l) { const int32_t c2 = s_state[l]; n_leaf += c2 < 0 ? 1u : 0u; n_done += c2 == PT_BVH_EMPTY ? 1u : 0u; }
                vc.idle_leaf += n_leaf; vc.idle_done += n_done;
            }
            node_step<L, ORD>(g.nodes, stk, rs, h.t, cur, sp);
            if (DIAG) s_state[stk.tid & 63u] = cur;
        }
        if (cur == PT_BVH_EMPTY) break;
        if (DIAG) late_cycle = true;
        if (ANY) leaf_step_any(g.tris, stk, o, d, h, cur, sp);
        else { const uint32_t nt = leaf_step(g.tris, stk, o, d, h, cur, sp); if (COUNT) vc.tris += nt; }
        if (DIAG) s_state[stk.tid & 63u] = cur;
    }
    return h;
}

constexpr int FUSE_LENS = 3, FUSE_SPH = 4, FUSE_SPH_LENS = 5, FUSE_TEX = 6;
template <int FUSE_, bool NEE, bool ENV>
using ExtendArgsOf = std::conditional_t<FUSE_ == FUSE_TEX, ExtTexArgsT<NEE, ENV>, std::conditional_t<FUSE_ == FUSE_SPH, ExtSphArgsT<ENV, false>, std::conditional_t<FUSE_ == FUSE_SPH_LENS, ExtSphArgsT<ENV, true>,
                     std::conditional_t<FUSE_ == FUSE_LENS, ExtLensArgsT<NEE, ENV>, ExtArgsT<NEE, ENV>>>>>;
template <int L, bool COUNT, int FUSE_, bool NEE = false, bool ENV = false>
__global__ void __launch_bounds__(kExtBlock) __attribute__((amdgpu_waves_per_eu(PT_EXT_WAVES_K(L, FUSE_, NEE, ENV), PT_EXT_WAVES_K(L, FUSE_, NEE, ENV))))
k_extend(ExtendArgsOf<FUSE_, NEE, ENV> args)
{
    constexpr bool SPH = FUSE_ == FUSE_SPH || FUSE_ == FUSE_SPH_LENS;
    constexpr bool LENS = FUSE_ == FUSE_LENS || FUSE_ == FUSE_SPH_LENS;
    constexpr bool TEX = FUSE_ == FUSE_TEX;
    constexpr int FUSE = (LENS || SPH || TEX) ? (int)SHADE_INLINE : FUSE_;
    const ExtArgs &a = ext_of(args);
    static_assert(!SPH || (NEE && !COUNT), "SPH: NEE's, all-kinds fused shading, no visit counters");
    static_assert(!NEE || (FUSE != SHADE_NONE && !COUNT), "NEE: fused shading, no visit counters");
    static_assert(!ENV || (FUSE == SHADE_INLINE && !COUNT), "ENV: all-kinds fused shading, no visit counters");
    static_assert(!LENS || (FUSE == SHADE_INLINE && !COUNT), "LENS: all-kinds fused shading, no visit counters");
    static_assert(!TEX || !COUNT, "TEX: all-kinds fused shading, no visit counters");
    const HotScene g = hot_scene(a.sc);
    const uint32_t it = a.it;
    __shared__ int32_t s_stack[kStackLds * kExtBlock];
    __shared__ uint32_t s_stash[(FUSE != SHADE_NONE ? (NEE ? 7 : 5) : 1) * kExtBlock];
    const uint32_t tid = threadIdx.x;
    ExtHead hd;
    uint32_t gid, qbase, slot = kInvalidSlot, n_bounces;
    {
        const PathState &ps = cold().ps;
        hd = extend_head<FUSE>(a, ps, kExtBlock, tid, true, false);
        gid = hd.bx * kExtBlock + tid;
        if (hd.idle) return;
        qbase = hd.shard * ps.shard_cap;
        if (gid < hd.n) slot = at(ps.q_ext[hd.parity], qbase + gid);
        if (FUSE != SHADE_NONE) slot = queued_slot(it, slot);
        const bool sparse = hd.do_compact && (float)hd.n_alive < ps.sparse_below * (float)hd.n;
        n_bounces = FUSE == SHADE_NONE ? 1u : (hd.n_alive <= ps.finish_below ? kFinishVertices : sparse ? 1u : a.bounces);
    }
    const uint32_t shard = hd.shard, parity = hd.parity, n = hd.n;
    const bool active = slot != kInvalidSlot;
    const StackCtx stk{ s_stack, kExtBlock, tid, qbase + gid };

    VisitCounts vc;
    __shared__ int32_t s_state[COUNT ? 64 : 1];
    PathRegs r = path_none();
    NeeRegs nr{ 0.0f, 0u };
    if (active) {
        if (FUSE == SHADE_NONE) { const PathState &ps = cold().ps; r.o = xyz(at(ps.ray_o, slot)); r.d = xyz(at(ps.ray_d, slot)); }
        else if constexpr (LENS) path_begin<NEE, true>(it, slot, r, &nr, &lens_args<NEE, ENV>());
        else path_begin<NEE>(it, slot, r, &nr);
    }
    bool alive = active;
    uint32_t wave_rays = 0;
    for (uint32_t bounce = 0; bounce < n_bounces; ++bounce) {
        const uint64_t alive_mask = __ballot(alive);
        if (alive_mask == 0) break;
        wave_rays += (uint32_t)__popcll(alive_mask);
        if (COUNT && kExtBlock == 64u) { s_state[tid] = alive ? 0 : 1; __syncthreads(); }
        if (alive) {
            const V3 o = r.o, d = r.d;
            Hit h{ (NEE && (nr.flags & NEE_PENDING)) ? nr.aux : __builtin_inff(), PT_MISS, PT_MISS };
            if (FUSE != SHADE_NONE) stash_park(s_stash, kExtBlock, tid, r);
            if constexpr (NEE) {
                s_stash[5 * kExtBlock + tid] = __float_as_uint(nr.aux); s_stash[6 * kExtBlock + tid] = nr.flags;
                asm volatile("" ::: "memory");
            }
            h = trace_ray<L, COUNT, COUNT, false>(g, stk, o, d, h, vc, s_state);
            if (FUSE == SHADE_NONE) at(cold().ps.hit, slot) = make_float2(h.t, __uint_as_float(h.ref));
            else {
                stash_restore(s_stash, kExtBlock, tid, r);
                uint32_t defer = 0u;
                const ExtArgs &c = cold();
                if constexpr (NEE) {
                    nr.aux = __uint_as_float(s_stash[5 * kExtBlock + tid]); nr.flags = s_stash[6 * kExtBlock + tid];
                    if (nr.flags & NEE_PENDING) {
                        if constexpr (SPH) { if (shadow_reached_lamp(nr.flags, h.ref, g.n_tris)) h.ref = PT_MISS; }
                        if constexpr (LENS) alive = resolve_shadow<true>(c.sc, c.ps, c.fp, kernargs<true, ENV>().nee, slot, r, nr, h.ref == PT_MISS, &lens_args<true, ENV>());
                        else alive = resolve_shadow(c.sc, c.ps, c.fp, kernargs<true, ENV>().nee, slot, r, nr, h.ref == PT_MISS);
                    } else alive = shade_one<FUSE, true, ENV, LENS, SPH, TEX>(c.sc, c.ps, c.fp, slot, r, h.t, h.ref, B_LAMBERT, defer, &nr);
                } else alive = shade_one<FUSE, false, ENV, LENS, false, TEX>(c.sc, c.ps, c.fp, slot, r, h.t, h.ref, B_LAMBERT, defer);
            }
        }
    }
    const PathState &ps = cold().ps;
    if (COUNT && active) flush_visit_counters(ps, vc);
    if (FUSE != SHADE_NONE) {
        if (alive) path_store<NEE>(ps, slot, r, &nr);
        queue_next(ps, shard, hd.cnext, &at(ps.q_ext[parity ^ 1u], qbase), gid, n, alive, slot, hd.do_compact);
        if (wave_rays && lane_id() == 0u) atomicAdd(traced_counter(ps, hd.cnext, shard), (unsigned long long)wave_rays);
    }
}

#ifndef PT_REFILL_IDLE
#define PT_REFILL_IDLE 16
#endif
constexpr uint32_t kRefillIdle = PT_REFILL_IDLE;

#ifndef PT_PACKED_WAVES
#define PT_PACKED_WAVES(FUSE) ((FUSE) == SHADE_INLINE ? 6 : 7)
#endif
template <int L, bool COUNT, int FUSE>
__global__ void __launch_bounds__(64) __attribute__((amdgpu_waves_per_eu(PT_PACKED_WAVES(FUSE), PT_PACKED_WAVES(FUSE))))
k_extend_packed(ExtArgs a)
{
    const float4 *__restrict__ nodes = a.sc.nodes, *__restrict__ tris = a.sc.tris, *__restrict__ spheres = a.sc.spheres;
    const uint32_t n_spheres = a.sc.n_spheres, n_tris = a.sc.n_tris, n_nodes = a.sc.n_nodes;
    const uint32_t it = a.it, chunk = a.chunk, bounces = a.bounces;
    __shared__ int32_t s_stack[kStackLds * 64];
    __shared__ uint32_t s_stash[(FUSE != SHADE_NONE ? 5 : 1) * 64];
    const uint32_t lane = threadIdx.x;
    const ExtHead hd = extend_head<FUSE>(a, cold().ps, chunk, lane, false, true);
    if (hd.idle) return;
    const uint32_t shard = hd.shard, n_alive = hd.n_alive;
    const bool do_compact = hd.do_compact;
    uint32_t next = hd.bx * chunk;
    const uint32_t end = min(hd.n, next + chunk);
    const uint32_t qbase = hd.shard * cold().ps.shard_cap;
    const uint32_t *queue = cold().ps.q_ext[hd.parity] + (size_t)qbase;
    uint32_t *q_next = cold().ps.q_ext[hd.parity ^ 1u] + (size_t)qbase;
    const StackCtx stk{ s_stack, 64u, lane, qbase + hd.bx * 64u + lane };
    const uint32_t budget0 = FUSE == SHADE_NONE ? 1u : (n_alive <= cold().ps.finish_below ? kFinishVertices : bounces);

    bool has = false;
    uint32_t slot = 0, pos = 0, budget = 0, sp = 0, steps = 0;
    int32_t cur = PT_BVH_EMPTY;
    PathRegs r = path_none();
    V3 &o = r.o, &d = r.d;
    RaySetup rs = ray_setup(o, d);
    Hit h{ __builtin_inff(), PT_MISS, PT_MISS };
    VisitCounts vc;
    uint32_t wave_rays = 0, wave_alive = 0;

    auto start_ray = [&]() {
        if (FUSE != SHADE_NONE) stash_park(s_stash, 64u, lane, r);
        h = Hit{ __builtin_inff(), PT_MISS, PT_MISS };
        { const uint32_t ns = spheres_test(spheres, n_spheres, n_tris, o, d, h); if (COUNT) vc.sph += ns; }
        rs = ray_setup(o, d);
        cur = n_nodes ? 0 : PT_BVH_EMPTY;
        sp = 0; steps = 0;
    };

    for (;;) {
        const bool fin = has && cur == PT_BVH_EMPTY;
        bool retired = false, retire_alive = false;
        if (fin) {
            if (FUSE == SHADE_NONE) {
                at(cold().ps.hit, slot) = make_float2(h.t, __uint_as_float(h.ref));
                has = false;
            } else {
                stash_restore(s_stash, 64u, lane, r);
                uint32_t defer = 0u;
                const bool alive = shade_one<FUSE>(cold().sc, cold().ps, cold().fp, slot, r, h.t, h.ref, B_LAMBERT, defer);
                --budget;
                if (alive && budget != 0u) start_ray();
                else {
                    if (alive) path_store(cold().ps, slot, r);
                    retired = true; retire_alive = alive; has = false;
                }
            }
        }
        if (FUSE != SHADE_NONE) {
            wave_rays += (uint32_t)__popcll(__ballot(fin && has));
            wave_alive += (uint32_t)__popcll(__ballot(retire_alive));
// ... 731 lines not shown
{
    constexpr bool SPEC = MODE == SHADE_BUCKETS;
    const uint32_t parity = it & 1u, ccur = it % 3u, cnext = (it + 1u) % 3u;
    uint32_t shard, bx, nbx;
    block_pos(ps, shard, bx, nbx);
    const size_t qbase = (size_t)shard * ps.shard_cap;
    uint32_t total, c0 = 0u;
    if (SPEC) {
        c0 = ps.counters[cnt_bucket_index(parity, B_METAL, shard)];
        total = c0 + ps.counters[cnt_bucket_index(parity, B_DIELECTRIC, shard)];
        if (bx == 0 && threadIdx.x < 2u)
            ps.counters[cnt_bucket_index(parity ^ 1u, B_METAL + threadIdx.x, shard)] = 0u;
    } else total = ps.counters[cnt_ext_index(ccur, shard)];
    const uint32_t n_alive = ps.counters[cnt_alive_index(ccur, shard)];
    const bool do_compact = SPEC || want_compact(ps, total, n_alive, 0u, false, compact != 0u);
    if (!SPEC && do_compact && n_alive && bx == 0 && threadIdx.x == 0) atomicAdd(&ps.counters[kCntCompactions], 1u);
    for (uint32_t base = bx * kBlock; base < total; base += nbx * kBlock) {
        const uint32_t gid = base + threadIdx.x;
        uint32_t b = B_LAMBERT, slot = kInvalidSlot;
        if (SPEC) {
            b = gid >= c0 ? B_DIELECTRIC : B_METAL;
            if (gid < total) slot = ps.q_bucket[b][qbase + (gid >= c0 ? gid - c0 : gid)];
        } else if (gid < total) slot = ps.q_ext[parity][qbase + gid];
        const bool active = slot != kInvalidSlot;
        bool alive = false;
        uint32_t defer = 0u;

        if (active) {
            const float2 hr = at(ps.hit, slot);
            PathRegs r;
            path_load(ps, slot, r);
            alive = shade_one<MODE>(sc, ps, fp, slot, r, hr.x, __float_as_uint(hr.y), b, defer);
            if (alive) path_store(ps, slot, r);
        }
        queue_next(ps, shard, cnext, ps.q_ext[parity ^ 1u] + qbase, gid, total, alive, slot, do_compact);
        if (MODE == SHADE_QUEUE) {
            wave_push(&ps.counters[cnt_bucket_index(parity, B_METAL, shard)], ps.q_bucket[B_METAL] + qbase, defer == B_METAL, slot);
            wave_push(&ps.counters[cnt_bucket_index(parity, B_DIELECTRIC, shard)], ps.q_bucket[B_DIELECTRIC] + qbase, defer == B_DIELECTRIC, slot);
        }
        if (!SPEC) break;
    }
}

__global__ void __launch_bounds__(kBlock) k_reduce_streams(const float4 *__restrict__ acc, float4 *__restrict__ tiles,
                                                           uint32_t slots_per_stream, uint32_t streams)
{
    const uint32_t slot = blockIdx.x * kBlock + threadIdx.x;
    if (slot >= slots_per_stream) return;
    float4 t = acc[slot_of(slot, 0u, streams)];
    for (uint32_t k = 1; k < streams; ++k) {
        const float4 a = acc[slot_of(slot, k, streams)];
        t.x = t.x + a.x; t.y = t.y + a.y; t.z = t.z + a.z; t.w = t.w + a.w;
    }
    tiles[slot] = t;
}

__global__ void __launch_bounds__(kBlock) k_assemble(const float4 *__restrict__ gathered, uint32_t nranks, uint32_t slots_per_rank,
                                                     uint32_t width, uint32_t height, uint32_t tiles_x, uint32_t n_tiles,
                                                     float inv_spp, float4 *__restrict__ fb, uint32_t *__restrict__ fb8)
{
    const uint32_t x = blockIdx.x * 64u + threadIdx.x, y = blockIdx.y * 4u + threadIdx.y;
    if (x >= width || y >= height) return;
    const uint32_t tile = (y >> kTileShift) * tiles_x + (x >> kTileShift);
    const uint32_t rank = tile % nranks, tl = tile / nranks;
    const uint32_t lx = x & (kTile - 1), ly = y & (kTile - 1);
    const uint32_t inner = ((((ly >> 3) << 3) + (lx >> 3)) << 6) | ((ly & 7u) << 3) | (lx & 7u);
    const float4 a = gathered[(size_t)rank * slots_per_rank + ((size_t)tl << (2 * kTileShift)) + inner];
    const float4 c = make_float4(a.x * inv_spp, a.y * inv_spp, a.z * inv_spp, a.w * inv_spp);
    const size_t i = (size_t)y * width + x;
    fb[i] = c;
    fb8[i] = unorm8(c.x) | (unorm8(c.y) << 8) | (unorm8(c.z) << 16) | (unorm8(c.w) << 24);
    (void)n_tiles;
}

static inline uint32_t blocks_for(uint32_t n) { return n ? (n + kBlock - 1) / kBlock : 1u; }

hipError_t launch_reference_sphere(hipStream_t s, uint32_t w, uint32_t h, float4 *out_f, uint32_t *out8)
{
    dim3 block(64, 4, 1), grid((w + 63) / 64, (h + 3) / 4, 1);
    hipLaunchKernelGGL(k_reference_sphere, grid, block, 0, s, w, h, out_f, out8);
    return hipGetLastError();
}

hipError_t launch_generate(hipStream_t s, const DeviceScene &sc, const PathState &ps, const FrameParams &fp, GenerateMode mode)
{
    hipLaunchKernelGGL(k_generate, shard_grid(blocks_for(ps.shard_cap), ps.shard_count), dim3(kBlock), 0, s, sc, ps, fp, (uint32_t)mode);
    return hipGetLastError();
}

hipError_t launch_sky_pixels(hipStream_t s, const DeviceScene &sc, const PathState &ps, const FrameParams &fp)
{
    hipLaunchKernelGGL(k_sky_pixels, dim3(blocks_for(ps.n_slots)), dim3(kBlock), 0, s, sc, ps, fp);
    return hipGetLastError();
}

template <typename F>
static bool with_layout(uint32_t width, F &&f)
{
    switch (width) {
    case PT_BVH_WIDTH_2: f(std::integral_constant<int, PT_BVH_WIDTH_2>{}); return true;
    case PT_BVH_WIDTH_4: f(std::integral_constant<int, PT_BVH_WIDTH_4>{}); return true;
    case PT_BVH_WIDTH_4Q: f(std::integral_constant<int, PT_BVH_WIDTH_4Q>{}); return true;
    case PT_BVH_WIDTH_8Q: f(std::integral_constant<int, PT_BVH_WIDTH_8Q>{}); return true;
    case PT_BVH_WIDTH_8O: f(std::integral_constant<int, PT_BVH_WIDTH_8O>{}); return true;
    default: return false;
    }
}
template <int... V, typename F>
static void with_value(int v, F &&f) { (void)((v == V && (f(std::integral_constant<int, V>{}), true)) || ...); }

template <int L, bool COUNT, int FUSE, bool NEE, bool ENV, bool LENS, bool SPH, bool TEX>
static void launch_k_extend(hipStream_t s, dim3 grid, const ExtArgs &a, const NeeArgs *nee, const EnvArgs *env, const LensArgs *lens, const SphArgs *sph, const TexArgs *tex)
{
    ExtArgsT<NEE, ENV> t; t.x = a; if constexpr (NEE) t.nee = *nee; if constexpr (ENV) t.env = *env;
    if constexpr (TEX) hipLaunchKernelGGL((k_extend<L, COUNT, FUSE_TEX, NEE, ENV>), grid, dim3(kExtBlock), 0, s, ExtTexArgsT<NEE, ENV>{ t, *tex });
    else if constexpr (SPH && LENS) hipLaunchKernelGGL((k_extend<L, COUNT, FUSE_SPH_LENS, true, ENV>), grid, dim3(kExtBlock), 0, s, ExtSphArgsT<ENV, true>{ { t, *lens }, *sph });
    else if constexpr (SPH) hipLaunchKernelGGL((k_extend<L, COUNT, FUSE_SPH, true, ENV>), grid, dim3(kExtBlock), 0, s, ExtSphArgsT<ENV, false>{ t, *sph });
    else if constexpr (LENS) hipLaunchKernelGGL((k_extend<L, COUNT, FUSE_LENS, NEE, ENV>), grid, dim3(kExtBlock), 0, s, ExtLensArgsT<NEE, ENV>{ t, *lens });
    else hipLaunchKernelGGL((k_extend<L, COUNT, FUSE, NEE, ENV>), grid, dim3(kExtBlock), 0, s, t);
}

hipError_t launch_extend(hipStream_t s, const DeviceScene &sc, const PathState &ps, const FrameParams &fp, const ExtendLaunch &x)
{
    const bool has_nee = x.nee != nullptr, has_env = x.env != nullptr, has_lens = x.lens != nullptr, has_sph = x.sph != nullptr, has_tex = x.tex != nullptr;
    if (!extend_instantiated(x.kernel, x.fuse, x.count, has_nee, has_env, has_lens, has_sph, has_tex)) return hipErrorInvalidValue;
    const uint32_t chunk = x.kernel == EXT_PACKED ? (x.packed_chunk >= 64u ? x.packed_chunk : 128u) : 0u;
    const uint32_t per_block = x.kernel == EXT_PACKED ? chunk : x.kernel == EXT_POOL ? kPool : kExtBlock;
    const dim3 grid = shard_grid(x.shard_bound ? (x.shard_bound + per_block - 1) / per_block : 1u, ps.shard_count);
    ExtArgs a;
    a.sc = sc; a.ps = ps; a.fp = fp; a.it = x.it; a.compact = x.compact ? 1u : 0u; a.bounces = x.bounces ? x.bounces : 1u; a.chunk = chunk;
    const bool known = with_layout(sc.bvh_width, [&](auto lc) { with_value<EXT_SIMPLE, EXT_PACKED, EXT_POOL>(x.kernel, [&](auto kc) {
        with_value<SHADE_NONE, SHADE_QUEUE, SHADE_INLINE>(x.fuse, [&](auto fc) { with_value<0, 1>(x.count, [&](auto cc) {
            with_value<0, 1>(has_nee, [&](auto nc) { with_value<0, 1>(has_env, [&](auto ec) { with_value<0, 1>(has_lens, [&](auto zc) { with_value<0, 1>(has_sph, [&](auto sc_) { with_value<0, 1>(has_tex, [&](auto tc) {
                constexpr int L = decltype(lc)::value, K = decltype(kc)::value, F = decltype(fc)::value;
                constexpr bool C = decltype(cc)::value != 0, N = decltype(nc)::value != 0, E = decltype(ec)::value != 0, Z = decltype(zc)::value != 0, S = decltype(sc_)::value != 0, T = decltype(tc)::value != 0;
                if constexpr (!extend_instantiated(K, F, C, N, E, Z, S, T)) return;
                else if constexpr (K == EXT_POOL) hipLaunchKernelGGL((k_extend_pool<L, C, F>), grid, dim3(64), 0, s, a);
                else if constexpr (K == EXT_PACKED) hipLaunchKernelGGL((k_extend_packed<L, C, F>), grid, dim3(64), 0, s, a);
                else launch_k_extend<L, C, F, N, E, Z, S, T>(s, grid, a, x.nee, x.env, x.lens, x.sph, x.tex);
            }); }); }); }); });
        }); });
    }); });
    return known ? hipGetLastError() : hipErrorInvalidValue;
}

uint32_t trace_blocks(uint32_t n) { return std::max(1u, std::min(kTraceBlocks, (n + kExtBlock - 1u) / kExtBlock)); }

hipError_t launch_trace(hipStream_t s, const DeviceScene &sc, const PathState &ps, const float4 *rays, float4 *hits, uint32_t n, bool occlusion, bool count)
{
    TraceArgs a{};
    a.sc = sc; a.ps = ps; a.rays = rays; a.hits = hits; a.n = n;
    const dim3 grid(trace_blocks(n));
    const bool known = with_layout(sc.bvh_width, [&](auto lc) {
        constexpr int L = decltype(lc)::value;
        if (occlusion) hipLaunchKernelGGL((k_trace<L, TRACE_OCCLUSION>), grid, dim3(kExtBlock), 0, s, a);
        else if (count) hipLaunchKernelGGL((k_trace<L, TRACE_COUNT>), grid, dim3(kExtBlock), 0, s, a);
        else hipLaunchKernelGGL((k_trace<L, TRACE_CLOSEST>), grid, dim3(kExtBlock), 0, s, a);
    });
    return known ? hipGetLastError() : hipErrorInvalidValue;
}

uint32_t gather_group_shift(uint32_t samples)
{
    uint32_t sh = 0;
    while (sh < 6u && (1u << sh) < samples) ++sh;
    return sh;
}
uint32_t gather_blocks(uint32_t n, uint32_t samples)
{
    const uint32_t per_wave = kExtBlock >> gather_group_shift(samples);
    return std::max(1u, std::min(kTraceBlocks, (uint32_t)(((uint64_t)n + per_wave - 1u) / per_wave)));
}

hipError_t launch_gather(hipStream_t s, const DeviceScene &sc, const PathState &ps, const float4 *points, float4 *out, uint32_t n, const GatherParams &gp,
                         const GatherPathParams *pp, const EnvArgs *env, const NeeArgs *nee, const SphArgs *sph)
{
    if ((nee && !pp) || (sph && !nee)) return hipErrorInvalidValue;
    GatherArgs a{};
    a.sc = sc; a.ps = ps; a.points = points; a.out = out; a.n = n;
    a.samples = gp.samples; a.gshift = gather_group_shift(gp.samples); a.seed = gp.seed;
    a.point_offset = gp.point_offset; a.sample_offset = gp.sample_offset; a.tmax = gp.tmax; a.ray_eps = gp.ray_eps;
    if (pp) { a.fp.max_depth = pp->max_depth; a.fp.rr_start = pp->rr_start; a.fp.ray_eps = gp.ray_eps; }
    const dim3 grid(gather_blocks(n, gp.samples));
    const bool known = with_layout(sc.bvh_width, [&](auto lc) { with_value<0, 1>(env != nullptr, [&](auto ec) { with_value<0, 1>(pp != nullptr, [&](auto pc) {
        constexpr int L = decltype(lc)::value;
        constexpr bool E = decltype(ec)::value != 0;
        GatherArgsT<E> t; t.x = a; if constexpr (E) t.env = *env;
        if constexpr (decltype(pc)::value != 0) {
            if (nee) {
                GatherNeeArgsT<E> tn; tn.x = a; tn.nee = *nee; if constexpr (E) tn.env = *env;
                if (sph) hipLaunchKernelGGL((k_gather_paths_nee<L | kGatherSph, E>), grid, dim3(kExtBlock), 0, s, GatherSphArgsT<E>{ tn, *sph });
                else
                hipLaunchKernelGGL((k_gather_paths_nee<L, E>), grid, dim3(kExtBlock), 0, s, tn);
            } else hipLaunchKernelGGL((k_gather_paths<L, E>), grid, dim3(kExtBlock), 0, s, t);
        }
        else hipLaunchKernelGGL((k_gather<L, E>), grid, dim3(kExtBlock), 0, s, t);
    }); }); });
    return known ? hipGetLastError() : hipErrorInvalidValue;
}

hipError_t launch_shade(hipStream_t s, const DeviceScene &sc, const PathState &ps, const FrameParams &fp, uint32_t it, uint32_t shard_bound, ShadeMode mode, bool compact)
{
    const uint32_t parity = it;
    const dim3 grid = shard_grid(blocks_for(shard_bound), ps.shard_count), block(kBlock);
    const dim3 sgrid = shard_grid(std::min(blocks_for(shard_bound), 16u), ps.shard_count);
    const uint32_t cm = compact ? 1u : 0u;
    if (mode == SHADE_BUCKETS) hipLaunchKernelGGL(k_shade<SHADE_BUCKETS>, sgrid, block, 0, s, sc, ps, fp, parity, 1u);
    else if (mode == SHADE_INLINE) hipLaunchKernelGGL(k_shade<SHADE_INLINE>, grid, block, 0, s, sc, ps, fp, parity, cm);
    else hipLaunchKernelGGL(k_shade<SHADE_QUEUE>, grid, block, 0, s, sc, ps, fp, parity, cm);
    return hipGetLastError();
}

hipError_t launch_reduce_streams(hipStream_t s, const float4 *acc, float4 *tiles, uint32_t slots_per_stream, uint32_t streams)
{
    hipLaunchKernelGGL(k_reduce_streams, dim3(blocks_for(slots_per_stream)), dim3(kBlock), 0, s, acc, tiles, slots_per_stream, streams);
    return hipGetLastError();
}

hipError_t launch_assemble(hipStream_t s, const float4 *gathered, uint32_t nranks, uint32_t slots_per_rank,
                           uint32_t width, uint32_t height, uint32_t tiles_x, uint32_t n_tiles, float inv_spp,
                           float4 *fb, uint32_t *fb8)
{
// ... 7 lines not shown
```

pathtracing_amd/csrc/pipeline.h:

```cpp
#pragma once
#include <stdint.h>
#include "../../include/ptrt.h"

namespace ptrt {

enum ExtendKernel : int { EXT_SIMPLE = 1, EXT_PACKED = 2, EXT_POOL = 3 };
constexpr uint32_t kExtendKernelFirst = EXT_SIMPLE, kExtendKernelLast = EXT_POOL;
enum ShadeMode { SHADE_NONE = -1, SHADE_QUEUE = 0, SHADE_BUCKETS = 1, SHADE_INLINE = 2 };
enum GenerateMode : uint32_t { GEN_QUEUE = 0, GEN_STATE = 1, GEN_DENSE = 2 };

constexpr bool extend_instantiated(int kernel, int fuse, bool count, bool nee, bool env, bool lens = false, bool sph = false, bool tex = false)
{
    if (kernel < EXT_SIMPLE || kernel > EXT_POOL || fuse == SHADE_BUCKETS || fuse < SHADE_NONE || fuse > SHADE_INLINE) return false;
    if (tex) return kernel == EXT_SIMPLE && !count && fuse == SHADE_INLINE && !lens && !sph;
    if (sph) return nee && kernel == EXT_SIMPLE && !count && fuse == SHADE_INLINE;
    if (lens) return kernel == EXT_SIMPLE && !count && fuse == SHADE_INLINE;
    if (env) return kernel == EXT_SIMPLE && !count && fuse == SHADE_INLINE;
    if (nee) return kernel == EXT_SIMPLE && !count && fuse != SHADE_NONE;
    return kernel != EXT_POOL || fuse != SHADE_NONE;
}

struct Pipeline {
    uint32_t forced;
    bool profile, count;
    bool split, bucket;
    bool nee;
    bool env;
    ShadeMode shade;
    bool lens;
    bool sph;
    bool tex;

    constexpr ShadeMode fuse() const { return split ? SHADE_NONE : shade; }
    constexpr bool full_state() const { return split || forced == (uint32_t)EXT_POOL; }
    constexpr GenerateMode generate_mode(bool dense) const { return full_state() ? GEN_STATE : dense ? GEN_DENSE : GEN_QUEUE; }
    constexpr bool forces_compact(bool repack_sticky, uint32_t samples_per_stream) const { return bucket || (repack_sticky && samples_per_stream <= 2u); }
    constexpr bool resolves_sky() const { return !full_state() && !count && !env && !lens; }
    constexpr bool instrumented() const { return count || profile; }
    constexpr bool single_loop(bool probing) const { return instrumented() || probing; }
    constexpr ExtendKernel kernel_for(uint32_t choice, uint32_t probe_iteration) const
    {
        return (choice == (uint32_t)EXT_PACKED || (choice == 0u && probe_iteration == 3u)) ? EXT_PACKED : (choice == (uint32_t)EXT_POOL && !split) ? EXT_POOL : EXT_SIMPLE;
    }
};

struct PipelineDecode { pt_status status; const char *message; Pipeline pipeline; };

constexpr PipelineDecode decode_pipeline(uint32_t flags, uint32_t tuned_kernel, bool has_env, bool has_specular, bool has_lens = false,
                                         bool has_sphere_light = false, bool has_textures = false)
{
    Pipeline p{};
    if ((flags & PT_FLAG_NEXT_EVENT_SPHERES) && !(flags & PT_FLAG_NEXT_EVENT))
        return { PT_ERR_INVALID_ARGUMENT, "PT_FLAG_NEXT_EVENT_SPHERES needs PT_FLAG_NEXT_EVENT", p };
    p.profile = (flags & PT_FLAG_PROFILE_KERNELS) != 0; p.count = (flags & PT_FLAG_COUNT_VISITS) != 0;
    p.bucket = (flags & PT_FLAG_BUCKET_SPECULAR) != 0; p.split = p.bucket || (flags & PT_FLAG_SPLIT_KERNELS) != 0;
    p.nee = (flags & PT_FLAG_NEXT_EVENT) != 0; p.env = has_env; p.lens = has_lens;
    p.sph = p.nee && (flags & PT_FLAG_NEXT_EVENT_SPHERES) != 0 && has_sphere_light;
    p.tex = has_textures;
    p.shade = (has_specular || has_env || has_lens || p.sph || p.tex) ? SHADE_INLINE : SHADE_QUEUE;
    p.forced = (flags & PT_FLAG_EXTEND_POOL) ? (uint32_t)EXT_POOL : (flags & PT_FLAG_EXTEND_PACKED) ? (uint32_t)EXT_PACKED
               : (flags & PT_FLAG_EXTEND_SIMPLE) ? (uint32_t)EXT_SIMPLE : tuned_kernel;
    const bool other_kernel = p.split || p.forced == (uint32_t)EXT_PACKED || p.forced == (uint32_t)EXT_POOL;
    if (p.tex && (other_kernel || p.count))
        return { PT_ERR_UNSUPPORTED, "a textured scene (docs/SPEC.md §13) renders on the one-ray-per-lane kernel only: not with PT_FLAG_EXTEND_PACKED, "
                                     "PT_FLAG_EXTEND_POOL, PT_FLAG_SPLIT_KERNELS, PT_FLAG_BUCKET_SPECULAR, PT_FLAG_COUNT_VISITS or pt_tuning.extend_kernel 2 / 3", p };
    if (p.tex && p.lens)
        return { PT_ERR_UNSUPPORTED, "a textured scene does not render through a lens (pt_scene_set_lens, radius > 0): remove the lens or the textures", p };
    if (p.tex && p.sph)
        return { PT_ERR_UNSUPPORTED, "a textured scene with a sphere light does not render with PT_FLAG_NEXT_EVENT_SPHERES", p };
    if (p.env && (other_kernel || p.count))
        return { PT_ERR_UNSUPPORTED, "a scene with an environment map renders on the one-ray-per-lane kernel only: not with PT_FLAG_EXTEND_PACKED, "
                                     "PT_FLAG_EXTEND_POOL, PT_FLAG_SPLIT_KERNELS, PT_FLAG_BUCKET_SPECULAR, PT_FLAG_COUNT_VISITS or pt_tuning.extend_kernel 2 / 3", p };
    if (p.lens && (other_kernel || p.count))
        return { PT_ERR_UNSUPPORTED, "a frame through a lens (pt_scene_set_lens, radius > 0) renders on the one-ray-per-lane kernel only: not with PT_FLAG_EXTEND_PACKED, "
                                     "PT_FLAG_EXTEND_POOL, PT_FLAG_SPLIT_KERNELS, PT_FLAG_BUCKET_SPECULAR, PT_FLAG_COUNT_VISITS or pt_tuning.extend_kernel 2 / 3", p };
    if (p.nee && other_kernel)
        return { PT_ERR_UNSUPPORTED, "PT_FLAG_NEXT_EVENT runs on the one-ray-per-lane kernel only: not with PT_FLAG_EXTEND_PACKED, "
                                     "PT_FLAG_EXTEND_POOL, PT_FLAG_SPLIT_KERNELS, PT_FLAG_BUCKET_SPECULAR or pt_tuning.extend_kernel 2 / 3", p };
    if (p.nee && p.count) return { PT_ERR_UNSUPPORTED, "PT_FLAG_NEXT_EVENT does not count visits (PT_FLAG_COUNT_VISITS)", p };
    if (p.env || p.nee || p.lens || p.tex) p.forced = EXT_SIMPLE;
    return { PT_OK, nullptr, p };
}

}
```

pathtracing_amd/csrc/ptrt_internal.h:

```cpp
#pragma once
#include <hip/hip_runtime_api.h>
#include <stdint.h>
#include "../../include/ptrt.h"
#include "pipeline.h"

namespace ptrt {

constexpr uint32_t kTileShift = 6;
constexpr uint32_t kTile = 1u << kTileShift;
constexpr uint32_t kTilePixels = kTile * kTile;
constexpr uint32_t kBlock = 256;
#ifndef PT_SHARD_GROUP_SHIFT
#define PT_SHARD_GROUP_SHIFT 6
#endif
constexpr uint32_t kShardGroupShift = PT_SHARD_GROUP_SHIFT;
#ifndef PT_STACK_LDS
#define PT_STACK_LDS 12
#endif
#ifndef PT_EXT_BLOCK
#define PT_EXT_BLOCK 64
#endif
constexpr uint32_t kStackLds = PT_STACK_LDS;
constexpr uint32_t kExtBlock = PT_EXT_BLOCK;
constexpr uint32_t kMaxSpheres = 64;
// ... 38 lines not shown
    const float4 *mats;
    uint32_t n_nodes, n_tris, n_spheres, n_mats;
    float sky[3];
    uint32_t bvh_width;
    pt_camera cam;
};

struct PathState {
    float4 *ray_o;
    float4 *ray_d;
    float2 *hit;
    float4 *thr;
    uint32_t *sd;
    float4 *acc;
    uint32_t *q_ext[2];
    uint32_t *q_bucket[B_COUNT];
    uint32_t *counters;
    int32_t *stack_ovf;
    uint32_t stack_ovf_entries;
    uint32_t n_slots;
    uint32_t shard_cap;
    uint32_t shard_base, shard_count;
    float compact_below;
    uint32_t repack_sticky;
    float sparse_below;
    uint32_t finish_below;
    uint4 *host_ring;
    uint32_t ring_slots;
};

struct NeeArgs {
    const float4 *lights;
    const float *cdf;
    const float *pa;
    uint32_t n_lights;
    float4 *ext;
    float4 *rad;
};

struct EnvArgs {
    const float4 *texels;
    const float *mcdf;
    const float *ccdf;
    uint32_t n;
    float nf, step;
    uint32_t lit;
    float psel;
};

struct LensArgs {
    float u[3], v[3];
    float focus;
    uint32_t pad;
};
static_assert(sizeof(LensArgs) == 32, "LensArgs is 32 bytes");

struct SphArgs {
    const float *pmf;
    uint32_t n_tri;
    uint32_t pad;
};
static_assert(sizeof(SphArgs) == 16, "SphArgs is 16 bytes");

struct TexArgs {
    const float4 *uv;
    const uint4 *desc;
    const float4 *texels;
    uint32_t n_desc;
    uint32_t pad;
};
static_assert(sizeof(TexArgs) == 32, "TexArgs is 32 bytes");

struct FrameParams {
    uint32_t width, height, spp, max_depth, rr_start, seed_hashed, sample_offset;
    float ray_eps;
    uint32_t rank, nranks, tiles_x, n_tiles;
    uint32_t streams;
    uint32_t slots_per_stream;
    uint32_t accumulate;
    uint32_t streams_magic, streams_shift, tiles_x_magic, tiles_x_shift;
    uint32_t offset_mod;
    uint32_t scene_x0, scene_x1, scene_y0, scene_y1;
};
inline __host__ __device__ bool sky_pixel(const FrameParams &fp, uint32_t x, uint32_t y)
{
    return x < fp.scene_x0 || x >= fp.scene_x1 || y < fp.scene_y0 || y >= fp.scene_y1;
}
inline void div_magic(uint32_t d, uint32_t &magic, uint32_t &shift)
{
    if (d <= 1u) { magic = 0u; shift = 0u; return; }
    uint32_t l = 0; while ((1ull << l) < d) ++l;
    magic = (uint32_t)(((1ull << (31u + l)) + d - 1u) / d); shift = l - 1u;
}
inline __host__ __device__ uint32_t div_by(uint32_t n, uint32_t magic, uint32_t shift)
{
    return magic ? (uint32_t)(((uint64_t)n * magic) >> 32) >> shift : n;
}

hipError_t launch_reference_sphere(hipStream_t s, uint32_t w, uint32_t h, float4 *out_f, uint32_t *out_rgba8);
hipError_t launch_generate(hipStream_t s, const DeviceScene &sc, const PathState &ps, const FrameParams &fp, GenerateMode mode);
hipError_t launch_sky_pixels(hipStream_t s, const DeviceScene &sc, const PathState &ps, const FrameParams &fp);
struct ExtendLaunch {
    uint32_t it, shard_bound;
    ExtendKernel kernel; ShadeMode fuse; bool count, compact;
    uint32_t packed_chunk;
    uint32_t bounces;
    const NeeArgs *nee;
    const EnvArgs *env;
    const LensArgs *lens;
    const SphArgs *sph = nullptr;
    const TexArgs *tex = nullptr;
};
hipError_t launch_extend(hipStream_t s, const DeviceScene &sc, const PathState &ps, const FrameParams &fp, const ExtendLaunch &x);
hipError_t launch_shade(hipStream_t s, const DeviceScene &sc, const PathState &ps, const FrameParams &fp, uint32_t it, uint32_t shard_bound, ShadeMode mode, bool compact);
uint32_t trace_blocks(uint32_t n);
hipError_t launch_trace(hipStream_t s, const DeviceScene &sc, const PathState &ps, const float4 *rays, float4 *hits, uint32_t n, bool occlusion, bool count);
struct GatherParams {
    uint32_t samples, seed, point_offset, sample_offset;
    float tmax, ray_eps;
};
struct GatherPathParams { uint32_t max_depth, rr_start; };
uint32_t gather_group_shift(uint32_t samples);
uint32_t gather_blocks(uint32_t n, uint32_t samples);
hipError_t launch_gather(hipStream_t s, const DeviceScene &sc, const PathState &ps, const float4 *points, float4 *out, uint32_t n, const GatherParams &gp,
                         const GatherPathParams *pp, const EnvArgs *env, const NeeArgs *nee = nullptr, const SphArgs *sph = nullptr);
hipError_t launch_reduce_streams(hipStream_t s, const float4 *acc, float4 *tiles, uint32_t slots_per_stream, uint32_t streams);
hipError_t launch_assemble(hipStream_t s, const float4 *gathered, uint32_t nranks, uint32_t slots_per_rank,
                           uint32_t width, uint32_t height, uint32_t tiles_x, uint32_t n_tiles, float inv_spp,
                           float4 *fb, uint32_t *fb8);

int context_device(const pt_context *c);
hipStream_t context_stream(const pt_context *c);
void context_set_error(pt_context *c, const char *msg);

struct BinaryBvh;
struct DeviceBlob4Q;
hipError_t build_lbvh_device(hipStream_t s, const float *verts9, uint32_t n_tris, BinaryBvh &out);
hipError_t build_lbvh_blob4q_device(hipStream_t s, const float *verts9, const uint32_t *mats, uint32_t n_tris, DeviceBlob4Q &out);

}
```

Measured before the change: 18510.

## Add lane grouping so each path slot walks several accumulation streams

Adds a LaneParams mapping in which each path slot serves several streams in turn (per_lane = streams/lanes), shrinking the number of live slots, and adds a 'lanes' tuning knob. With the default (default_lanes returns streams) the mapping is the identity, so the behaviour is meant to stay the same while the structure is added. It does add kernel-argument bytes, some magic-division index work, and a WALK template path that uses an LDS stash in the extend kernel.

```diff
diff --git a/include/ptrt.h b/include/ptrt.h
--- a/include/ptrt.h
+++ b/include/ptrt.h
@@ -115,6 +115,7 @@
     uint32_t lag;
     uint32_t extend_kernel;
     uint32_t readback;
+    uint32_t lanes;
 } pt_tuning;
 
 pt_status pt_context_create(const pt_device_desc *desc, pt_context **out);
diff --git a/pathtracing_amd/_native.py b/pathtracing_amd/_native.py
--- a/pathtracing_amd/_native.py
+++ b/pathtracing_amd/_native.py
@@ -81,7 +81,7 @@
 class pt_tuning(C.Structure):
     _fields_ = [("bounces", C.c_uint32), ("loops", C.c_uint32), ("finish_below", C.c_uint32), ("packed_chunk", C.c_uint32),
                 ("compact_below", C.c_float), ("sparse_below", C.c_float), ("sticky_samples", C.c_uint32), ("lag", C.c_uint32),
-                ("extend_kernel", C.c_uint32), ("readback", C.c_uint32)]
+                ("extend_kernel", C.c_uint32), ("readback", C.c_uint32), ("lanes", C.c_uint32)]
 
 
 class pt_tile_layout(C.Structure):
@@ -134,7 +134,7 @@
     _fields_ = [("n_tris", C.c_uint64), ("n_spheres", C.c_uint64), ("n_mats", C.c_uint64)]
 
 
-assert C.sizeof(pt_material) == 48 and C.sizeof(pt_camera) == 64 and C.sizeof(pt_render_params) == 64 and C.sizeof(pt_tuning) == 40
+assert C.sizeof(pt_material) == 48 and C.sizeof(pt_camera) == 64 and C.sizeof(pt_render_params) == 64 and C.sizeof(pt_tuning) == 44
 assert C.sizeof(pt_denoise_params) == 32 and C.sizeof(pt_temporal_params) == 32
 assert C.sizeof(pt_display_params) == 40 and C.sizeof(pt_display_info) == 32 and C.sizeof(pt_environment_info) == 24
 assert C.sizeof(pt_gather_params) == 32 and C.sizeof(pt_lens) == 32 and C.sizeof(pt_texture_info) == 24
diff --git a/pathtracing_amd/csrc/api.cpp b/pathtracing_amd/csrc/api.cpp
--- a/pathtracing_amd/csrc/api.cpp
+++ b/pathtracing_amd/csrc/api.cpp
@@ -128,6 +128,7 @@
     if (t->extend_kernel > kExtendKernelLast) return fail(c, PT_ERR_INVALID_ARGUMENT, "tuning: extend_kernel must be 0 (probed), 1 (one ray per lane), 2 (lane-packing) or 3 (pooled)");
     if (t->readback > 1) return fail(c, PT_ERR_INVALID_ARGUMENT, "tuning: readback must be 0 (mapped store) or 1 (copy per launch)");
     if (t->readback == 0 && !c->sizes.can_map()) return fail(c, PT_ERR_UNSUPPORTED, "tuning: readback 0 needs host-mapped pinned memory, which this platform did not provide");
+    if (t->lanes > 64) return fail(c, PT_ERR_INVALID_ARGUMENT, "tuning: lanes must be 0 (default) or a divisor of the frames' streams, at most 64");
     c->tuning = *t;
     return PT_OK;
 }
diff --git a/pathtracing_amd/csrc/context.h b/pathtracing_amd/csrc/context.h
--- a/pathtracing_amd/csrc/context.h
+++ b/pathtracing_amd/csrc/context.h
@@ -247,7 +247,7 @@
 
 class FrameTemplate {
 public:
-    struct Key { uint32_t w, h, rank, nranks, streams, first_spp, offset, n_slots, shard_cap, pad; const void *q, *acc;
+    struct Key { uint32_t w, h, rank, nranks, streams, first_spp, offset, n_slots, shard_cap, lanes; const void *q, *acc;
                  bool operator==(const Key &o) const { return std::memcmp(this, &o, sizeof *this) == 0; } };
     hipError_t reserve(size_t q_entries)
     {
@@ -255,7 +255,7 @@
         return e != hipSuccess ? e : cnt_init.ensure(kCntTotalWords);
     }
     pt_status build_if_differs(pt_context *c, hipStream_t q, Key key, const Pipeline &pipe, const DeviceScene &ds, const PathState &ps,
-                               const FrameParams &fp, const QueueSizes &sizes);
+                               const FrameParams &fp, const LaneParams &lp, const QueueSizes &sizes);
     void frame_ran(bool accumulate_or_full_state) { if (accumulate_or_full_state && key_.first_spp < key_.streams) valid = false; }
     const uint32_t *counters() const { return cnt_init.p; }
     uint32_t *first_queue() const { return q_init.p; }
@@ -309,6 +309,7 @@
         0,
         0,
         0,
+        0,
     };
     ptrt::Event ev_start, ev_stop;
     ptrt::Event ev_probe[4];
diff --git a/pathtracing_amd/csrc/frame.cpp b/pathtracing_amd/csrc/frame.cpp
--- a/pathtracing_amd/csrc/frame.cpp
+++ b/pathtracing_amd/csrc/frame.cpp
@@ -53,6 +53,12 @@
     }
 };
 
+uint32_t default_lanes(uint32_t pixel_slots, uint32_t streams, uint32_t spp)
+{
+    (void)pixel_slots; (void)spp;
+    return streams;
+}
+
 hipEvent_t pool_event(pt_context *c, size_t i)
 {
     while (c->ev_pool.size() <= i) {
@@ -152,7 +158,8 @@
 }
 
 struct Frame {
-    uint32_t nranks, streams, pixel_slots, n_slots, shard_cap, samples_per_stream, lag, n_loops, packed_chunk, default_bounces;
+    uint32_t nranks, streams, pixel_slots, n_slots, shard_cap, samples_per_slot, lag, n_loops, packed_chunk, default_bounces;
+    LaneParams lp;
     Pipeline pipe;
     bool accumulate, mapped, compact;
     NeeArgs nee_args; EnvArgs env_args; LensArgs lens_args;
@@ -169,14 +176,14 @@
 }
 
 pt_status FrameTemplate::build_if_differs(pt_context *c, hipStream_t q, Key key, const Pipeline &pipe, const DeviceScene &ds, const PathState &ps,
-                                          const FrameParams &fp, const QueueSizes &sizes)
+                                          const FrameParams &fp, const LaneParams &lp, const QueueSizes &sizes)
 {
     key.q = q_init.p;
     if (valid && key == key_) return PT_OK;
     valid = false; HIP_TRY(c, hipMemsetAsync(cnt_init.p, 0, sizeof(uint32_t) * kCntTotalWords, q));
     PathState pt = ps; pt.counters = cnt_init.p; pt.q_ext[0] = q_init.p;
     const bool dense = key.first_spp < key.streams;
-    HIP_TRY(c, launch_generate(q, ds, pt, fp, pipe.generate_mode(dense)));
+    HIP_TRY(c, launch_generate(q, ds, pt, fp, lp, pipe.generate_mode(dense)));
     bound = key.shard_cap;
     if (dense) {
         uint32_t *h = sizes.template_sizes();
@@ -214,23 +221,27 @@
     if (p->streams > 64) return fail(c, PT_ERR_INVALID_ARGUMENT, "streams must be in [0,64]");
     const pt_tuning &t = c->tuning;
     f.nranks = p->nranks ? p->nranks : 1u; f.streams = p->streams ? p->streams : 1u;
+    if (t.lanes && f.streams % t.lanes) return fail(c, PT_ERR_INVALID_ARGUMENT, "pt_tuning.lanes (%u) does not divide the frame's streams (%u)", t.lanes, f.streams);
     f.pixel_slots = lay.tiles_per_rank * kTilePixels;
     const uint64_t slots64 = (uint64_t)f.pixel_slots * f.streams;
     if (slots64 >= (1ull << 28)) return fail(c, PT_ERR_UNSUPPORTED, "frame too large: %llu slots (pixels of this rank x streams), limit 2^28", (unsigned long long)slots64);
-    f.n_slots = (uint32_t)slots64;
-    const uint32_t groups = (f.n_slots + (1u << kShardGroupShift) - 1u) >> kShardGroupShift, shard_cap = ((groups + kShards - 1) / kShards) << kShardGroupShift;
-    f.shard_cap = shard_cap; f.q_entries = (size_t)kShards * shard_cap;
-    f.samples_per_stream = (p->spp + f.streams - 1u) / f.streams;
     const PipelineDecode d = decode_frame(c, s, p);
     if (d.status != PT_OK) return fail(c, d.status, "%s", d.message);
     const Pipeline &pipe = f.pipe = d.pipeline;
+    const bool groups_ok = pipe.lane_groups(ExtendFrame(s->cache.ext, pipe).kernel, p->spp, f.streams);
+    const uint32_t lanes = !groups_ok ? f.streams : t.lanes ? t.lanes : default_lanes(f.pixel_slots, f.streams, p->spp);
+    f.lp = lane_params(f.streams, lanes);
+    f.n_slots = f.pixel_slots * lanes;
+    const uint32_t groups = (f.n_slots + (1u << kShardGroupShift) - 1u) >> kShardGroupShift, shard_cap = ((groups + kShards - 1) / kShards) << kShardGroupShift;
+    f.shard_cap = shard_cap; f.q_entries = (size_t)kShards * shard_cap;
+    f.samples_per_slot = (p->spp + lanes - 1u) / lanes;
     if (pipe.lens && !lens_basis(s->ds.cam, s->lens, f.lens_args))
         return fail(c, PT_ERR_INVALID_ARGUMENT, "pt_render through a lens: the camera's right or up has length 0, or the aperture's axes are not finite");
     f.mapped = t.readback == 0u;
     f.packed_chunk = t.packed_chunk >= 64u ? t.packed_chunk : (f.streams >= 4u ? 256u : 128u);
     const uint32_t v34 = p->max_depth * 3u / 4u; f.default_bounces = std::min(12u, std::max(4u, v34 > 2u ? v34 - 2u : 0u));
     if (pipe.nee) f.default_bounces *= 2u;
-    f.lag = t.lag ? t.lag : (f.samples_per_stream <= 2u ? 2u : 3u) + (f.mapped ? 1u : 0u);
+    f.lag = t.lag ? t.lag : (f.samples_per_slot <= 2u ? 2u : 3u) + (f.mapped ? 1u : 0u);
     f.accumulate = (p->flags & PT_FLAG_ACCUMULATE) != 0;
     f.sums_key = sums_key_of(p);
     if (f.accumulate)
@@ -247,7 +258,7 @@
     f.total_spp = (f.accumulate ? c->sums.samples() : 0u) + p->spp; c->sums.begin();
     f.allocs_before = g_device_allocs;
     HIP_TRY(c, c->ray_o.ensure(f.n_slots)); HIP_TRY(c, c->ray_d.ensure(f.n_slots)); HIP_TRY(c, c->thr.ensure(f.n_slots));
-    HIP_TRY(c, c->acc.ensure(f.n_slots)); HIP_TRY(c, c->out.tiles.ensure(f.pixel_slots)); HIP_TRY(c, c->sd.ensure(f.n_slots));
+    HIP_TRY(c, c->acc.ensure((size_t)slots64)); HIP_TRY(c, c->out.tiles.ensure(f.pixel_slots)); HIP_TRY(c, c->sd.ensure(f.n_slots));
     HIP_TRY(c, c->q_ext0.ensure(f.q_entries)); HIP_TRY(c, c->q_ext1.ensure(f.q_entries));
     if (pipe.split) { HIP_TRY(c, c->hit.ensure(f.n_slots)); HIP_TRY(c, c->q_metal.ensure(f.q_entries)); HIP_TRY(c, c->q_dielectric.ensure(f.q_entries)); }
     if (!pipe.full_state()) HIP_TRY(c, c->start.reserve(f.q_entries));
@@ -269,9 +280,9 @@
     if (pipe.split) { ps.hit = c->hit.p; ps.q_bucket[B_METAL] = c->q_metal.p; ps.q_bucket[B_DIELECTRIC] = c->q_dielectric.p; }
     ps.counters = c->counters.p; ps.stack_ovf = c->stack_ovf.p; ps.stack_ovf_entries = ovf; ps.n_slots = f.n_slots; ps.shard_cap = f.shard_cap;
     ps.shard_base = 0; ps.shard_count = kShards; ps.compact_below = t.compact_below; ps.finish_below = t.finish_below; ps.sparse_below = t.sparse_below;
-    ps.repack_sticky = (f.samples_per_stream <= t.sticky_samples && t.compact_below > 0.f) ? 1u : 0u;
+    ps.repack_sticky = (f.samples_per_slot <= t.sticky_samples && t.compact_below > 0.f) ? 1u : 0u;
     ps.host_ring = c->sizes.begin(f.mapped); ps.ring_slots = kLag;
-    f.compact = pipe.forces_compact(ps.repack_sticky != 0u, f.samples_per_stream);
+    f.compact = pipe.forces_compact(ps.repack_sticky != 0u, f.samples_per_slot);
     FrameParams &fp = f.fp;
     fp.width = p->width; fp.height = p->height; fp.spp = p->spp; fp.max_depth = p->max_depth; fp.rr_start = p->rr_start;
     fp.seed_hashed = host_pcg(p->seed); fp.sample_offset = p->sample_offset; fp.ray_eps = p->ray_eps;
@@ -289,13 +300,13 @@
     if (full_state) {
         HIP_TRY(c, hipMemsetAsync(c->counters.p, 0, sizeof(uint32_t) * kCntTotalWords, q));
         HIP_TRY(c, hipEventRecord(c->ev_start, q));
-        HIP_TRY(c, launch_generate(q, s->ds, f.ps, f.fp, f.pipe.generate_mode(false)));
+        HIP_TRY(c, launch_generate(q, s->ds, f.ps, f.fp, f.lp, f.pipe.generate_mode(false)));
     } else {
         HIP_TRY(c, hipEventRecord(c->ev_start, q));
         FrameTemplate::Key key{};
         key.w = p->width; key.h = p->height; key.rank = p->rank; key.nranks = f.nranks; key.streams = f.streams; key.first_spp = std::min(p->spp, f.streams);
-        key.offset = f.fp.offset_mod; key.n_slots = f.n_slots; key.shard_cap = f.shard_cap; key.acc = c->acc.p;
-        const pt_status st = c->start.build_if_differs(c, q, key, f.pipe, s->ds, f.ps, f.fp, c->sizes);
+        key.offset = f.fp.offset_mod; key.n_slots = f.n_slots; key.shard_cap = f.shard_cap; key.lanes = f.lp.lanes; key.acc = c->acc.p;
+        const pt_status st = c->start.build_if_differs(c, q, key, f.pipe, s->ds, f.ps, f.fp, f.lp, c->sizes);
         if (st != PT_OK) return st;
         HIP_TRY(c, hipMemcpyAsync(c->counters.p, c->start.counters(), sizeof(uint32_t) * kCntTotalWords, hipMemcpyDeviceToDevice, q));
         if (f.sky) HIP_TRY(c, launch_sky_pixels(q, s->ds, f.ps, f.fp));
@@ -335,7 +346,7 @@
             const ExtendLaunch launch{ it, L.bound, kernel, pipe.fuse(), pipe.count, f.compact, f.packed_chunk,
                                        c->tuning.bounces ? c->tuning.bounces : x.bounces(g, it, kernel, f.default_bounces),
                                        pipe.nee ? &f.nee_args : nullptr, pipe.env ? &f.env_args : nullptr, pipe.lens ? &f.lens_args : nullptr,
-                                       pipe.sph ? &f.sph_args : nullptr, pipe.tex ? &f.tex_args : nullptr };
+                                       pipe.sph ? &f.sph_args : nullptr, pipe.tex ? &f.tex_args : nullptr, &f.lp };
             HIP_TRY(c, launch_extend(L.stream, s->ds, pg, f.fp, launch));
             if (pipe.profile) HIP_TRY(c, hipEventRecord(e1, L.stream));
             if (pipe.bucket) {
@@ -404,7 +415,7 @@
     }
     out.paths = px * p->spp;
     out.rays += (px - scene_px) * p->spp;
-    out.reserved[2] = f.slot_launches + px * std::min(f.streams, p->spp);
+    out.reserved[2] = f.slot_launches + px * std::min(f.lp.lanes, p->spp);
     if (f.pipe.profile) {
         const bool trace = getenv("PTRT_TRACE") != nullptr;
         for (size_t i = 0; i + 2 < f.n_events; i += 3) {
diff --git a/pathtracing_amd/csrc/kernels.hip b/pathtracing_amd/csrc/kernels.hip
--- a/pathtracing_amd/csrc/kernels.hip
+++ b/pathtracing_amd/csrc/kernels.hip
@@ -53,13 +53,14 @@
 template <typename T>
 PT_DEV T &at(T *base, uint32_t i) { return *reinterpret_cast<T *>(reinterpret_cast<char *>(base) + (size_t)(i * (uint32_t)sizeof(T))); }
 
-template <bool NEE, bool ENV> struct ExtArgsT { ExtArgs x; };
-template <> struct ExtArgsT<true, false> { ExtArgs x; NeeArgs nee; };
-template <> struct ExtArgsT<false, true> { ExtArgs x; EnvArgs env; };
-template <> struct ExtArgsT<true, true> { ExtArgs x; NeeArgs nee; EnvArgs env; };
-static_assert(sizeof(ExtArgsT<false, false>) == sizeof(ExtArgs) && __builtin_offsetof(ExtArgsT<true, false>, nee) == sizeof(ExtArgs) &&
-              __builtin_offsetof(ExtArgsT<false, true>, env) == sizeof(ExtArgs) && __builtin_offsetof(ExtArgsT<true, true>, nee) == sizeof(ExtArgs) &&
-              __builtin_offsetof(ExtArgsT<true, true>, env) == sizeof(ExtArgs) + sizeof(NeeArgs), "each block directly behind the one before it");
+template <bool NEE, bool ENV> struct ExtArgsT { ExtArgs x; LaneParams lp; };
+template <> struct ExtArgsT<true, false> { ExtArgs x; LaneParams lp; NeeArgs nee; };
+template <> struct ExtArgsT<false, true> { ExtArgs x; LaneParams lp; EnvArgs env; };
+template <> struct ExtArgsT<true, true> { ExtArgs x; LaneParams lp; NeeArgs nee; EnvArgs env; };
+static_assert(sizeof(ExtArgsT<false, false>) == sizeof(ExtArgs) + sizeof(LaneParams) && __builtin_offsetof(ExtArgsT<true, false>, nee) == sizeof(ExtArgs) + sizeof(LaneParams) &&
+              __builtin_offsetof(ExtArgsT<false, true>, env) == sizeof(ExtArgs) + sizeof(LaneParams) && __builtin_offsetof(ExtArgsT<true, true>, nee) == sizeof(ExtArgs) + sizeof(LaneParams) &&
+              __builtin_offsetof(ExtArgsT<true, true>, lp) == sizeof(ExtArgs) && __builtin_offsetof(ExtArgsT<false, false>, lp) == sizeof(ExtArgs) &&
+              __builtin_offsetof(ExtArgsT<true, true>, env) == sizeof(ExtArgs) + sizeof(LaneParams) + sizeof(NeeArgs), "each block directly behind the one before it");
 template <bool NEE, bool ENV>
 PT_DEV const ExtArgsT<NEE, ENV> &kernargs()
 {
@@ -68,6 +69,7 @@
     return *(const ExtArgsT<NEE, ENV> *)p;
 }
 PT_DEV const ExtArgs &cold() { return kernargs<false, false>().x; }
+PT_DEV const LaneParams &lane_args() { return kernargs<false, false>().lp; }
 template <bool NEE, bool ENV> struct ExtLensArgsT { ExtArgsT<NEE, ENV> a; LensArgs lens; };
 static_assert(__builtin_offsetof(ExtLensArgsT<false, false>, lens) == sizeof(ExtArgsT<false, false>) && __builtin_offsetof(ExtLensArgsT<true, false>, lens) == sizeof(ExtArgsT<true, false>) &&
               __builtin_offsetof(ExtLensArgsT<false, true>, lens) == sizeof(ExtArgsT<false, true>) && __builtin_offsetof(ExtLensArgsT<true, true>, lens) == sizeof(ExtArgsT<true, true>) &&
@@ -119,6 +121,34 @@
 {
     return (((size_t)(pixel_slot >> 6) * streams + stream) << 6) | (pixel_slot & 63u);
 }
+PT_DEV uint32_t lane_pixel_slot(uint32_t slot, const LaneParams &lp)
+{
+    return (div_by(slot >> 6, lp.lanes_magic, lp.lanes_shift) << 6) | (slot & 63u);
+}
+PT_DEV uint32_t lane_first_stream(uint32_t slot, const LaneParams &lp)
+{
+    const uint32_t g = slot >> 6;
+    return (g - div_by(g, lp.lanes_magic, lp.lanes_shift) * lp.lanes) * lp.per_lane;
+}
+PT_DEV uint32_t lane_acc_first(uint32_t slot, const LaneParams &lp)
+{
+    return (((slot >> 6) * lp.per_lane) << 6) | (slot & 63u);
+}
+PT_DEV uint32_t lane_stream_index(uint32_t sample, const FrameParams &fp, const LaneParams &lp)
+{
+    const uint32_t v = fp.offset_mod + sample;
+    return v - div_by(v, lp.per_lane_magic, lp.per_lane_shift) * lp.per_lane;
+}
+PT_DEV uint32_t lane_acc(uint32_t slot, uint32_t sample, const FrameParams &fp, const LaneParams &lp)
+{
+    return lane_acc_first(slot, lp) + (lane_stream_index(sample, fp, lp) << 6);
+}
+PT_DEV uint32_t lane_next_stream(uint32_t sample, const FrameParams &fp, const LaneParams &lp)
+{
+    if (lane_stream_index(sample, fp, lp) + 1u >= lp.per_lane) return sample;
+    const uint32_t v = sample + 1u;
+    return v - div_by(v, fp.streams_magic, fp.streams_shift) * fp.streams;
+}
 
 PT_DEV void block_pos(const PathState &ps, uint32_t &shard, uint32_t &bx, uint32_t &nbx)
 {
@@ -127,9 +157,8 @@
 }
 static inline dim3 shard_grid(uint32_t blocks, uint32_t shard_count) { return dim3(blocks * shard_count); }
 
-PT_DEV bool slot_pixel(uint32_t slot_all, const FrameParams &fp, uint32_t &x, uint32_t &y)
-{
-    const uint32_t slot = slot_pixel_slot(slot_all, fp);
+PT_DEV bool pixel_of(uint32_t slot, const FrameParams &fp, uint32_t &x, uint32_t &y)
+{
     const uint32_t tl = slot >> (2 * kTileShift), inner = slot & (kTilePixels - 1);
     const uint32_t tile = fp.rank + fp.nranks * tl;
     if (tile >= fp.n_tiles) return false;
@@ -138,6 +167,14 @@
     x = (tx << kTileShift) + ((blk & 7u) << 3) + (ln & 7u);
     y = (ty << kTileShift) + ((blk >> 3) << 3) + (ln >> 3);
     return x < fp.width && y < fp.height;
+}
+PT_DEV bool slot_pixel(uint32_t slot_all, const FrameParams &fp, uint32_t &x, uint32_t &y)
+{
+    return pixel_of(slot_pixel_slot(slot_all, fp), fp, x, y);
+}
+PT_DEV bool lane_pixel(uint32_t slot, const FrameParams &fp, const LaneParams &lp, uint32_t &x, uint32_t &y)
+{
+    return pixel_of(lane_pixel_slot(slot, lp), fp, x, y);
 }
 
 PT_DEV Camera camera_of(const pt_camera &c)
@@ -430,10 +467,18 @@
 }
 PT_DEV float env_pdf(const EnvArgs &e, float4 tx, float s) { return e.psel * (tx.w / ((s * s) * s)); }
 
-PT_DEV uint32_t first_sample(uint32_t slot, const FrameParams &fp)
-{
-    const uint32_t v = slot_stream(slot, fp) + fp.streams - fp.offset_mod;
+PT_DEV uint32_t stream_first_sample(uint32_t stream, const FrameParams &fp)
+{
+    const uint32_t v = stream + fp.streams - fp.offset_mod;
     return v >= fp.streams ? v - fp.streams : v;
+}
+PT_DEV uint32_t first_sample(uint32_t slot, const FrameParams &fp) { return stream_first_sample(slot_stream(slot, fp), fp); }
+PT_DEV uint32_t lane_first_sample(uint32_t slot, const FrameParams &fp, const LaneParams &lp) { return stream_first_sample(lane_first_stream(slot, lp), fp); }
+template <bool WALK>
+PT_DEV bool slot_xy(uint32_t slot, const FrameParams &fp, uint32_t &x, uint32_t &y)
+{
+    if constexpr (WALK) return lane_pixel(slot, fp, lane_args(), x, y);
+    else return slot_pixel(slot, fp, x, y);
 }
 template <bool RAY = true, bool LENS = false>
 PT_DEV void camera_sample(const DeviceScene &sc, const FrameParams &fp, uint32_t x, uint32_t y, PathRegs &r, uint32_t &depth, const LensArgs *lens = nullptr)
@@ -445,19 +490,25 @@
     else r.o = v3(sc.cam.origin[0], sc.cam.origin[1], sc.cam.origin[2]);
     r.T = v3(1.f, 1.f, 1.f); depth = 0;
 }
-template <bool LENS = false>
+template <bool LENS = false, bool WALK = false>
 PT_DEV void path_init(const DeviceScene &sc, const FrameParams &fp, uint32_t slot, PathRegs &r, const LensArgs *lens = nullptr)
 {
     uint32_t x = 0, y = 0;
-    slot_pixel(slot, fp, x, y);
+    slot_xy<WALK>(slot, fp, x, y);
+    if constexpr (WALK) r.sample = lane_first_sample(slot, fp, lane_args());
+    else
     r.sample = first_sample(slot, fp);
     camera_sample<true, LENS>(sc, fp, x, y, r, r.depth, lens);
 }
-template <bool NEE = false, bool LENS = false>
+template <bool NEE = false, bool LENS = false, bool WALK = false>
 PT_DEV void path_begin(uint32_t it, uint32_t slot, PathRegs &r, NeeRegs *nr = nullptr, const LensArgs *lens = nullptr)
 {
     if (it == 0u) {
-        path_init<LENS>(cold().sc, cold().fp, slot, r, lens);
+        path_init<LENS, WALK>(cold().sc, cold().fp, slot, r, lens);
+        if constexpr (WALK) {
+            if (!cold().fp.accumulate)
+                for (uint32_t j = 0, e = lane_acc_first(slot, lane_args()); j < lane_args().per_lane; ++j, e += 64u) at(cold().ps.acc, e) = make_float4(0.f, 0.f, 0.f, 0.f);
+        } else
         if (!cold().fp.accumulate) at(cold().ps.acc, slot) = make_float4(0.f, 0.f, 0.f, 0.f);
     } else {
         const PathState &ps = cold().ps;
@@ -465,17 +516,18 @@
         if constexpr (NEE) { nr->flags = __float_as_uint(at(ps.ray_o, slot).w); nr->aux = at(ps.ray_d, slot).w; }
     }
 }
+template <bool WALK = false>
 PT_DEV uint32_t queued_slot(uint32_t it, uint32_t slot)
 {
     if (it == 0u && slot != kInvalidSlot) {
         uint32_t x = 0, y = 0;
-        slot_pixel(slot, cold().fp, x, y);
+        slot_xy<WALK>(slot, cold().fp, x, y);
         if (sky_pixel(cold().fp, x, y)) slot = kInvalidSlot;
     }
     return slot;
 }
 
-__global__ void __launch_bounds__(kBlock) k_generate(DeviceScene sc, PathState ps, FrameParams fp, uint32_t full)
+__global__ void __launch_bounds__(kBlock) k_generate(DeviceScene sc, PathState ps, FrameParams fp, LaneParams lp, uint32_t full)
 {
     uint32_t shard, bx, nbx;
     block_pos(ps, shard, bx, nbx);
@@ -484,9 +536,10 @@
     const uint32_t slot = ((t * kShards + rot) << kShardGroupShift) | (j & ((1u << kShardGroupShift) - 1u));
     uint32_t x = 0, y = 0;
     const bool in_range = j < ps.shard_cap && slot < ps.n_slots;
-    const uint32_t first = first_sample(slot, fp);
-    const bool valid = in_range && first < fp.spp && slot_pixel(slot, fp, x, y);
-    if (in_range && !fp.accumulate) ps.acc[slot] = make_float4(0.f, 0.f, 0.f, 0.f);
+    const uint32_t first = lane_first_sample(slot, fp, lp);
+    const bool valid = in_range && first < fp.spp && lane_pixel(slot, fp, lp, x, y);
+    if (in_range && !fp.accumulate)
+        for (uint32_t k = 0, e = lane_acc_first(slot, lp); k < lp.per_lane; ++k, e += 64u) ps.acc[e] = make_float4(0.f, 0.f, 0.f, 0.f);
     if (valid && full == 1u) {
         PathRegs r;
         path_init(sc, fp, slot, r);
@@ -505,7 +558,7 @@
 {
     const uint32_t slot = blockIdx.x * kBlock + threadIdx.x;
     uint32_t x = 0, y = 0;
-    if (slot >= ps.n_slots || !slot_pixel(slot, fp, x, y) || !sky_pixel(fp, x, y)) return;
+    if (slot >= fp.slots_per_stream * fp.streams || !slot_pixel(slot, fp, x, y) || !sky_pixel(fp, x, y)) return;
     const uint32_t first = first_sample(slot, fp);
     if (first >= fp.spp) return;
     float4 A = fp.accumulate ? ps.acc[slot] : make_float4(0.f, 0.f, 0.f, 0.f);
@@ -516,13 +569,25 @@
     ps.acc[slot] = A;
 }
 
-template <bool LENS = false>
-PT_DEV bool next_sample(const DeviceScene &sc, const FrameParams &fp, uint32_t slot, PathRegs &r, uint32_t &depth, const LensArgs *lens = nullptr)
+template <bool WALK>
+PT_DEV uint32_t sample_after(uint32_t sample, const FrameParams &fp, uint32_t *sum_cell)
+{
+    sample += fp.streams;
+    if constexpr (WALK)
+        if (!(sample < fp.spp)) {
+            const uint32_t first = lane_next_stream(sample, fp, lane_args());
+            if (first != sample) *sum_cell += 64u;
+            sample = first;
+        }
+    return sample;
+}
+template <bool LENS = false, bool WALK = false>
+PT_DEV bool next_sample(const DeviceScene &sc, const FrameParams &fp, uint32_t slot, PathRegs &r, uint32_t &depth, const LensArgs *lens = nullptr, uint32_t *sum_cell = nullptr)
 {
     uint32_t x = 0, y = 0;
-    r.sample += fp.streams;
+    r.sample = sample_after<WALK>(r.sample, fp, sum_cell);
     if (!(r.sample < fp.spp)) return false;
-    slot_pixel(slot, fp, x, y);
+    slot_xy<WALK>(slot, fp, x, y);
     camera_sample<true, LENS>(sc, fp, x, y, r, depth, lens);
     return true;
 }
@@ -537,14 +602,15 @@
     }
     return false;
 }
-template <int MODE, bool NEE = false, bool ENV = false, bool LENS = false, bool SPH = false, bool TEX = false>
+template <int MODE, bool NEE = false, bool ENV = false, bool LENS = false, bool SPH = false, bool TEX = false, bool WALK = false>
 PT_DEV bool shade_one(const DeviceScene &sc, const PathState &ps, const FrameParams &fp, uint32_t slot, PathRegs &r, float t, uint32_t ref,
-                      uint32_t b, uint32_t &defer, NeeRegs *nr = nullptr)
+                      uint32_t b, uint32_t &defer, NeeRegs *nr = nullptr, uint32_t *sum_cell = nullptr)
 {
     V3 &o = r.o, &d = r.d, &T = r.T;
     uint32_t &key = r.key, &sample = r.sample;
     uint32_t depth = r.depth + 1u;
-    float4 A = at(ps.acc, slot);
+    auto sum = [&]() { if constexpr (WALK) return *sum_cell; else return slot; };
+    float4 A = at(ps.acc, sum());
     bool touched = false, term = false, alive = false;
     constexpr bool SHARED = !NEE && MODE != SHADE_INLINE;
     static_assert(!LENS || !SHARED, "the shared end makes pinhole rays only");
@@ -736,9 +802,10 @@
     if (term) {
         touched = true;
         A.w += 1.0f;
-        sample += fp.streams;
+        if constexpr (WALK) { at(ps.acc, sum()) = A; touched = false; }
+        sample = sample_after<WALK>(sample, fp, sum_cell);
         if (sample < fp.spp) {
-            slot_pixel(slot, fp, x, y);
+            slot_xy<WALK>(slot, fp, x, y);
             if constexpr (LENS) camera_sample<true, true>(sc, fp, x, y, r, depth, &lens_args<NEE, ENV>());
             else
             camera_sample<!SHARED>(sc, fp, x, y, r, depth);
@@ -756,22 +823,23 @@
         } else v = lambert_vec(d, u1, u2);
         d = normalize(v);
     }
-    if (touched) at(ps.acc, slot) = A;
+    if (touched) at(ps.acc, sum()) = A;
     r.depth = depth;
     return alive;
 }
 
-template <bool LENS = false>
+template <bool LENS = false, bool WALK = false>
 PT_DEV bool resolve_shadow(const DeviceScene &sc, const PathState &ps, const FrameParams &fp, const NeeArgs &na, uint32_t slot, PathRegs &r,
-                           NeeRegs &nr, bool visible, const LensArgs *lens = nullptr)
+                           NeeRegs &nr, bool visible, const LensArgs *lens = nullptr, uint32_t *sum_cell = nullptr)
 {
     const bool end = (nr.flags & NEE_END) != 0u;
     bool alive = true;
     if (visible || end) {
-        float4 A = at(ps.acc, slot);
+        const uint32_t sum = WALK ? *sum_cell : slot;
+        float4 A = at(ps.acc, sum);
         if (visible) { const float4 L = at(na.rad, slot); A.x = A.x + L.x; A.y = A.y + L.y; A.z = A.z + L.z; }
-        if (end) { A.w += 1.0f; alive = next_sample<LENS>(sc, fp, slot, r, r.depth, lens); nr.aux = 0.0f; }
-        at(ps.acc, slot) = A;
+        if (end) { A.w += 1.0f; alive = next_sample<LENS, WALK>(sc, fp, slot, r, r.depth, lens, sum_cell); nr.aux = 0.0f; }
+        at(ps.acc, sum) = A;
     }
     if (!end) { const float4 e = at(na.ext, slot); r.d = xyz(e); nr.aux = e.w; }
     nr.flags = 0u;
@@ -1092,6 +1160,7 @@
     constexpr bool LENS = FUSE_ == FUSE_LENS || FUSE_ == FUSE_SPH_LENS;
     constexpr bool TEX = FUSE_ == FUSE_TEX;
     constexpr int FUSE = (LENS || SPH || TEX) ? (int)SHADE_INLINE : FUSE_;
+    constexpr bool WALK = FUSE != SHADE_NONE && !COUNT;
     const ExtArgs &a = ext_of(args);
     static_assert(!SPH || (NEE && !COUNT), "SPH: NEE's, all-kinds fused shading, no visit counters");
     static_assert(!NEE || (FUSE != SHADE_NONE && !COUNT), "NEE: fused shading, no visit counters");
@@ -1101,7 +1170,8 @@
     const HotScene g = hot_scene(a.sc);
     const uint32_t it = a.it;
     __shared__ int32_t s_stack[kStackLds * kExtBlock];
-    __shared__ uint32_t s_stash[(FUSE != SHADE_NONE ? (NEE ? 7 : 5) : 1) * kExtBlock];
+    constexpr uint32_t kSumRow = NEE ? 7 : 5;
+    __shared__ uint32_t s_stash[(FUSE != SHADE_NONE ? kSumRow + (WALK ? 1 : 0) : 1) * kExtBlock];
     const uint32_t tid = threadIdx.x;
     ExtHead hd;
     uint32_t gid, qbase, slot = kInvalidSlot, n_bounces;
@@ -1112,7 +1182,7 @@
         if (hd.idle) return;
         qbase = hd.shard * ps.shard_cap;
         if (gid < hd.n) slot = at(ps.q_ext[hd.parity], qbase + gid);
-        if (FUSE != SHADE_NONE) slot = queued_slot(it, slot);
+        if (FUSE != SHADE_NONE) slot = queued_slot<WALK>(it, slot);
         const bool sparse = hd.do_compact && (float)hd.n_alive < ps.sparse_below * (float)hd.n;
         n_bounces = FUSE == SHADE_NONE ? 1u : (hd.n_alive <= ps.finish_below ? kFinishVertices : sparse ? 1u : a.bounces);
     }
@@ -1126,8 +1196,9 @@
     NeeRegs nr{ 0.0f, 0u };
     if (active) {
         if (FUSE == SHADE_NONE) { const PathState &ps = cold().ps; r.o = xyz(at(ps.ray_o, slot)); r.d = xyz(at(ps.ray_d, slot)); }
-        else if constexpr (LENS) path_begin<NEE, true>(it, slot, r, &nr, &lens_args<NEE, ENV>());
-        else path_begin<NEE>(it, slot, r, &nr);
+        else if constexpr (LENS) path_begin<NEE, true, WALK>(it, slot, r, &nr, &lens_args<NEE, ENV>());
+        else path_begin<NEE, false, WALK>(it, slot, r, &nr);
+        if constexpr (WALK) s_stash[kSumRow * kExtBlock + tid] = lane_acc(slot, r.sample, cold().fp, lane_args());
     }
     bool alive = active;
     uint32_t wave_rays = 0;
@@ -1154,10 +1225,10 @@
                     nr.aux = __uint_as_float(s_stash[5 * kExtBlock + tid]); nr.flags = s_stash[6 * kExtBlock + tid];
                     if (nr.flags & NEE_PENDING) {
                         if constexpr (SPH) { if (shadow_reached_lamp(nr.flags, h.ref, g.n_tris)) h.ref = PT_MISS; }
-                        if constexpr (LENS) alive = resolve_shadow<true>(c.sc, c.ps, c.fp, kernargs<true, ENV>().nee, slot, r, nr, h.ref == PT_MISS, &lens_args<true, ENV>());
-                        else alive = resolve_shadow(c.sc, c.ps, c.fp, kernargs<true, ENV>().nee, slot, r, nr, h.ref == PT_MISS);
-                    } else alive = shade_one<FUSE, true, ENV, LENS, SPH, TEX>(c.sc, c.ps, c.fp, slot, r, h.t, h.ref, B_LAMBERT, defer, &nr);
-                } else alive = shade_one<FUSE, false, ENV, LENS, false, TEX>(c.sc, c.ps, c.fp, slot, r, h.t, h.ref, B_LAMBERT, defer);
+                        if constexpr (LENS) alive = resolve_shadow<true, WALK>(c.sc, c.ps, c.fp, kernargs<true, ENV>().nee, slot, r, nr, h.ref == PT_MISS, &lens_args<true, ENV>(), &s_stash[kSumRow * kExtBlock + tid]);
+                        else alive = resolve_shadow<false, WALK>(c.sc, c.ps, c.fp, kernargs<true, ENV>().nee, slot, r, nr, h.ref == PT_MISS, nullptr, &s_stash[kSumRow * kExtBlock + tid]);
+                    } else alive = shade_one<FUSE, true, ENV, LENS, SPH, TEX, WALK>(c.sc, c.ps, c.fp, slot, r, h.t, h.ref, B_LAMBERT, defer, &nr, &s_stash[kSumRow * kExtBlock + tid]);
+                } else alive = shade_one<FUSE, false, ENV, LENS, false, TEX, WALK>(c.sc, c.ps, c.fp, slot, r, h.t, h.ref, B_LAMBERT, defer, nullptr, &s_stash[kSumRow * kExtBlock + tid]);
             }
         }
     }
@@ -2055,15 +2126,23 @@
     return hipGetLastError();
 }
 
-hipError_t launch_generate(hipStream_t s, const DeviceScene &sc, const PathState &ps, const FrameParams &fp, GenerateMode mode)
-{
-    hipLaunchKernelGGL(k_generate, shard_grid(blocks_for(ps.shard_cap), ps.shard_count), dim3(kBlock), 0, s, sc, ps, fp, (uint32_t)mode);
+LaneParams lane_params(uint32_t streams, uint32_t lanes)
+{
+    LaneParams lp;
+    lp.lanes = lanes; lp.per_lane = streams / lanes;
+    div_magic(lp.lanes, lp.lanes_magic, lp.lanes_shift); div_magic(lp.per_lane, lp.per_lane_magic, lp.per_lane_shift);
+    return lp;
+}
+
+hipError_t launch_generate(hipStream_t s, const DeviceScene &sc, const PathState &ps, const FrameParams &fp, const LaneParams &lp, GenerateMode mode)
+{
+    hipLaunchKernelGGL(k_generate, shard_grid(blocks_for(ps.shard_cap), ps.shard_count), dim3(kBlock), 0, s, sc, ps, fp, lp, (uint32_t)mode);
     return hipGetLastError();
 }
 
 hipError_t launch_sky_pixels(hipStream_t s, const DeviceScene &sc, const PathState &ps, const FrameParams &fp)
 {
-    hipLaunchKernelGGL(k_sky_pixels, dim3(blocks_for(ps.n_slots)), dim3(kBlock), 0, s, sc, ps, fp);
+    hipLaunchKernelGGL(k_sky_pixels, dim3(blocks_for(fp.slots_per_stream * fp.streams)), dim3(kBlock), 0, s, sc, ps, fp);
     return hipGetLastError();
 }
 
@@ -2083,9 +2162,9 @@
 static void with_value(int v, F &&f) { (void)((v == V && (f(std::integral_constant<int, V>{}), true)) || ...); }
 
 template <int L, bool COUNT, int FUSE, bool NEE, bool ENV, bool LENS, bool SPH, bool TEX>
-static void launch_k_extend(hipStream_t s, dim3 grid, const ExtArgs &a, const NeeArgs *nee, const EnvArgs *env, const LensArgs *lens, const SphArgs *sph, const TexArgs *tex)
-{
-    ExtArgsT<NEE, ENV> t; t.x = a; if constexpr (NEE) t.nee = *nee; if constexpr (ENV) t.env = *env;
+static void launch_k_extend(hipStream_t s, dim3 grid, const ExtArgs &a, const LaneParams &lp, const NeeArgs *nee, const EnvArgs *env, const LensArgs *lens, const SphArgs *sph, const TexArgs *tex)
+{
+    ExtArgsT<NEE, ENV> t; t.x = a; t.lp = lp; if constexpr (NEE) t.nee = *nee; if constexpr (ENV) t.env = *env;
     if constexpr (TEX) hipLaunchKernelGGL((k_extend<L, COUNT, FUSE_TEX, NEE, ENV>), grid, dim3(kExtBlock), 0, s, ExtTexArgsT<NEE, ENV>{ t, *tex });
     else if constexpr (SPH && LENS) hipLaunchKernelGGL((k_extend<L, COUNT, FUSE_SPH_LENS, true, ENV>), grid, dim3(kExtBlock), 0, s, ExtSphArgsT<ENV, true>{ { t, *lens }, *sph });
     else if constexpr (SPH) hipLaunchKernelGGL((k_extend<L, COUNT, FUSE_SPH, true, ENV>), grid, dim3(kExtBlock), 0, s, ExtSphArgsT<ENV, false>{ t, *sph });
@@ -2102,6 +2181,8 @@
     const dim3 grid = shard_grid(x.shard_bound ? (x.shard_bound + per_block - 1) / per_block : 1u, ps.shard_count);
     ExtArgs a;
     a.sc = sc; a.ps = ps; a.fp = fp; a.it = x.it; a.compact = x.compact ? 1u : 0u; a.bounces = x.bounces ? x.bounces : 1u; a.chunk = chunk;
+    const LaneParams lp = x.lanes ? *x.lanes : lane_params(fp.streams, fp.streams);
+    if (lp.lanes != fp.streams && (x.kernel != EXT_SIMPLE || x.fuse == SHADE_NONE || x.count)) return hipErrorInvalidValue;
     const bool known = with_layout(sc.bvh_width, [&](auto lc) { with_value<EXT_SIMPLE, EXT_PACKED, EXT_POOL>(x.kernel, [&](auto kc) {
         with_value<SHADE_NONE, SHADE_QUEUE, SHADE_INLINE>(x.fuse, [&](auto fc) { with_value<0, 1>(x.count, [&](auto cc) {
             with_value<0, 1>(has_nee, [&](auto nc) { with_value<0, 1>(has_env, [&](auto ec) { with_value<0, 1>(has_lens, [&](auto zc) { with_value<0, 1>(has_sph, [&](auto sc_) { with_value<0, 1>(has_tex, [&](auto tc) {
@@ -2110,7 +2191,7 @@
                 if constexpr (!extend_instantiated(K, F, C, N, E, Z, S, T)) return;
                 else if constexpr (K == EXT_POOL) hipLaunchKernelGGL((k_extend_pool<L, C, F>), grid, dim3(64), 0, s, a);
                 else if constexpr (K == EXT_PACKED) hipLaunchKernelGGL((k_extend_packed<L, C, F>), grid, dim3(64), 0, s, a);
-                else launch_k_extend<L, C, F, N, E, Z, S, T>(s, grid, a, x.nee, x.env, x.lens, x.sph, x.tex);
+                else launch_k_extend<L, C, F, N, E, Z, S, T>(s, grid, a, lp, x.nee, x.env, x.lens, x.sph, x.tex);
             }); }); }); }); });
         }); });
     }); });
diff --git a/pathtracing_amd/csrc/pipeline.h b/pathtracing_amd/csrc/pipeline.h
--- a/pathtracing_amd/csrc/pipeline.h
+++ b/pathtracing_amd/csrc/pipeline.h
@@ -34,8 +34,12 @@
     constexpr ShadeMode fuse() const { return split ? SHADE_NONE : shade; }
     constexpr bool full_state() const { return split || forced == (uint32_t)EXT_POOL; }
     constexpr GenerateMode generate_mode(bool dense) const { return full_state() ? GEN_STATE : dense ? GEN_DENSE : GEN_QUEUE; }
-    constexpr bool forces_compact(bool repack_sticky, uint32_t samples_per_stream) const { return bucket || (repack_sticky && samples_per_stream <= 2u); }
+    constexpr bool forces_compact(bool repack_sticky, uint32_t samples_per_slot) const { return bucket || (repack_sticky && samples_per_slot <= 2u); }
     constexpr bool resolves_sky() const { return !full_state() && !count && !env && !lens; }
+    constexpr bool lane_groups(uint32_t choice, uint32_t spp, uint32_t streams) const
+    {
+        return !full_state() && !count && choice == (uint32_t)EXT_SIMPLE && spp >= streams;
+    }
     constexpr bool instrumented() const { return count || profile; }
     constexpr bool single_loop(bool probing) const { return instrumented() || probing; }
     constexpr ExtendKernel kernel_for(uint32_t choice, uint32_t probe_iteration) const
diff --git a/pathtracing_amd/csrc/ptrt_internal.h b/pathtracing_amd/csrc/ptrt_internal.h
--- a/pathtracing_amd/csrc/ptrt_internal.h
+++ b/pathtracing_amd/csrc/ptrt_internal.h
@@ -144,6 +144,10 @@
     uint32_t offset_mod;
     uint32_t scene_x0, scene_x1, scene_y0, scene_y1;
 };
+struct LaneParams {
+    uint32_t lanes, lanes_magic, lanes_shift;
+    uint32_t per_lane, per_lane_magic, per_lane_shift;
+};
 inline __host__ __device__ bool sky_pixel(const FrameParams &fp, uint32_t x, uint32_t y)
 {
     return x < fp.scene_x0 || x >= fp.scene_x1 || y < fp.scene_y0 || y >= fp.scene_y1;
@@ -160,7 +164,8 @@
 }
 
 hipError_t launch_reference_sphere(hipStream_t s, uint32_t w, uint32_t h, float4 *out_f, uint32_t *out_rgba8);
-hipError_t launch_generate(hipStream_t s, const DeviceScene &sc, const PathState &ps, const FrameParams &fp, GenerateMode mode);
+LaneParams lane_params(uint32_t streams, uint32_t lanes);
+hipError_t launch_generate(hipStream_t s, const DeviceScene &sc, const PathState &ps, const FrameParams &fp, const LaneParams &lp, GenerateMode mode);
 hipError_t launch_sky_pixels(hipStream_t s, const DeviceScene &sc, const PathState &ps, const FrameParams &fp);
 struct ExtendLaunch {
     uint32_t it, shard_bound;
@@ -172,6 +177,7 @@
     const LensArgs *lens;
     const SphArgs *sph = nullptr;
     const TexArgs *tex = nullptr;
+    const LaneParams *lanes = nullptr;
 };
 hipError_t launch_extend(hipStream_t s, const DeviceScene &sc, const PathState &ps, const FrameParams &fp, const ExtendLaunch &x);
 hipError_t launch_shade(hipStream_t s, const DeviceScene &sc, const PathState &ps, const FrameParams &fp, uint32_t it, uint32_t shard_bound, ShadeMode mode, bool compact);
```

Measured after the change: 18450. No clear change (-0.3%).
